# Yukayo/MobGT

Measured on AMD Instinct MI355X. Metric: check-ins/sec (train step), higher is better.
Workload: dtype bf16

## Files before the change

### __graft_entry__.py

```python
import os
import subprocess
import sys

ROOT = os.path.dirname(os.path.abspath(__file__))
if ROOT not in sys.path:
    sys.path.insert(0, ROOT)


def build() -> None:
    from mobgt_amd import _native
    for library in _native.LIBRARIES:
        library.build()
        library.lib()
    from mobgt_amd import _pairbins
    _pairbins.LIBRARY.build()
    _pairbins.LIBRARY.lib()
    from mobgt_amd import _universe
    _universe.LIBRARY.build()
    _universe.LIBRARY.lib()
    from mobgt_amd import _checkins
    _checkins.LIBRARY.build()
    _checkins.LIBRARY.lib()
    from mobgt_amd import _prefixes
    _prefixes.LIBRARY.build()
    _prefixes.LIBRARY.lib()
    from mobgt_amd import _baseline
    _baseline.LIBRARY.build()
    _baseline.LIBRARY.lib()
    from mobgt_amd import _prior
    _prior.LIBRARY.build()
    _prior.LIBRARY.lib()
    from mobgt_amd import _geoprior
    _geoprior.LIBRARY.build()
    _geoprior.LIBRARY.lib()
    from mobgt_amd import _priorfit
    _priorfit.LIBRARY.build()
    _priorfit.LIBRARY.lib()
    from mobgt_amd import _ctxprior
    _ctxprior.LIBRARY.build()
    _ctxprior.LIBRARY.lib()
    subprocess.check_call(["make", "-s", "-C", os.path.join(ROOT, "oracle")])
    import mobgt_amd


def smoke() -> None:
    import numpy as np
    import torch
    from mobgt_amd import ops, synth
    from mobgt_amd.model_fqandtoyo import EncoderLayer
    from oracle import algos_oracle as ao
    from oracle import model_oracle as mo
    assert torch.cuda.is_available(), "smoke() needs cuda:0"
    dev = "cuda:0"
    G, H, T, C = 3, 8, 37, 192
    torch.manual_seed(0)
    layer = EncoderLayer(C, 256, 0.1, 0.1, H).eval()
    sd = {"L." + k: v.detach().clone().requires_grad_(True) for k, v in layer.state_dict().items()}
    rng = np.random.RandomState(0)
    x = torch.from_numpy(rng.standard_normal((G, T, C)).astype(np.float32))
    gy = torch.from_numpy(rng.standard_normal((G, T, C)).astype(np.float32))
    bias = torch.from_numpy((rng.standard_normal((G, H, T, T)) * 0.5).astype(np.float32))
    bias[1, :, :, 30:] = float("-inf")
    xr, br = x.clone().requires_grad_(True), bias.clone().requires_grad_(True)
    ref = mo.encoder_layer_fq(sd, "L", xr, br, H)
    ref.backward(gy)
    layer = layer.to(dev)
    xd, bd = x.to(dev).requires_grad_(True), bias.to(dev).requires_grad_(True)
    out = layer(xd, bd)
    out.backward(gy.to(dev))
    torch.cuda.synchronize()

    def close(name, got, want, tol):
        got, want = got.detach().float().cpu().numpy(), want.detach().numpy()
        scale = float(np.sqrt((want ** 2).mean()))
        err = float(np.abs(got - want).max())
        assert err <= tol * scale, f"{name}: max |err| {err:.3e} vs rms {scale:.3e}"
    close("y", out, ref, 1e-3)
    close("dx", xd.grad, xr.grad, 1e-3)
    close("dbias", bd.grad, br.grad, 1e-3)
    for k, p in layer.named_parameters():
        if k.endswith("linear_k.bias"):
            continue
        if sd["L." + k].grad is not None:
            close("d" + k, p.grad, sd["L." + k].grad, 2e-3)
    layer.act_dtype = torch.bfloat16
    for prm in layer.parameters():
        prm.grad = None
    xb, bb = x.to(dev).requires_grad_(True), bias.to(dev).requires_grad_(True)
    out16 = layer(xb, bb)
    out16.backward(gy.to(dev))
    torch.cuda.synchronize()
    close("y (bf16)", out16, ref, 8e-2)
    close("dx (bf16)", xb.grad, xr.grad, 1e-1)
    close("dbias (bf16)", bb.grad, br.grad, 2e-1)
    trajs = synth.make_batch_of_trajectories(seed=4, G=4, P=50, n_user=8, n_nodes=[17, 3, 9, 30])
    n = np.array([len(t["node_name"]) for t in trajs], dtype=np.int32)
    counts = np.zeros((4, 30, 30), dtype=np.int32)
    for g, t in enumerate(trajs):
        counts[g, :n[g], :n[g]] = t["edge_type"]
    sp = ops.spd_batched(torch.from_numpy(counts).to(dev), torch.from_numpy(n).to(dev), 20)
    for g in range(4):
        k = int(n[g])
        M, path = ao.floyd_warshall(counts[g, :k, :k] != 0)
        assert np.array_equal(sp["spd"][g, :k, :k].cpu().numpy().astype(np.int64), M)
        assert np.array_equal(sp["path"][g, :k, :k].cpu().numpy().astype(np.int64), path)
    print("smoke ok: fused fq EncoderLayer fwd+bwd (f32 and bf16 configurations) and batched SPD match the oracle")


if __name__ == "__main__":
    build()
    if len(sys.argv) > 1 and sys.argv[1] == "smoke":
        smoke()
```

### mobgt_amd/csrc/tokbwd.hip

```cpp
#include "common.h"
#include "mobgt_hip.h"

namespace {

typedef __attribute__((ext_vector_type(4))) float f32x4;

constexpr int TNW = 12, TNT = TNW * 64, TBM = 16;

struct TokBwdParams {
    const float* dout;
    const float* real;
    const float* y4;
    const float* y2; int64_t ld2;
    const float *w4, *w2;
    float *d_nf, *d_add;
    float* dx4; int64_t ldx4;
    float* d_pt;
    float* d_token;
    int G, N;
    float slope4, slope2;
    uint32_t thr_pos, thr_in;
    float keep_pos, keep_in;
    uint64_t seed;
    const uint64_t* seed_dev;
    uint32_t salt_nf, salt_tok, salt_in;
    int n_node_blocks;
};

__device__ __forceinline__ float leaky_grad(float y, float slope) { return y > 0.f ? 1.f : slope; }

#ifdef TB_STAMP
__device__ int* g_tb_dbg = nullptr;
#define TSTAMP_DECL int st_[8] = {}
#define TSTAMP(i) st_[i] = (int)wall_clock64()
#define TSTAMP_DUMP() do { if (g_tb_dbg && threadIdx.x == 0) for (int q_ = 0; q_ < 8; ++q_) g_tb_dbg[blockIdx.x * 8 + q_] = st_[q_]; } while (0)
#else
#define TSTAMP_DECL
#define TSTAMP(i)
#define TSTAMP_DUMP()
#endif

template <int N> constexpr int gemm_ks() { return TNW / ((N + 63) / 64); }
template <int K, int N, int LDA, int LDO>
__device__ __forceinline__ void gemm_kn(const float* __restrict__ A, const float* __restrict__ W, float* __restrict__ out) {
    constexpr int NB = (N + 63) / 64, KS = TNW / NB, NT16 = K / 16, TMAX = (NT16 + KS - 1) / KS;
    static_assert(K % 16 == 0 && N % 32 == 0 && KS >= 1, "shape");
    const int lane = threadIdx.x & 63, wave = threadIdx.x >> 6;
    const int j = lane & 15, q = lane >> 4;
    if (wave >= NB * KS) return;
    const int blk = wave / KS, ks = wave % KS;
    const int t_lo = ks * NT16 / KS, t_hi = (ks + 1) * NT16 / KS;
    const int n0 = 64 * blk;
    const bool col_ok = n0 + 4 * j < N;
    const int cl = col_ok ? n0 + 4 * j : 0;
    f32x4 acc[4];
#pragma unroll
    for (int n = 0; n < 4; ++n) acc[n] = f32x4{0.f, 0.f, 0.f, 0.f};
    f32x4 bw[TMAX][4];
#pragma unroll
    for (int tt = 0; tt < TMAX; ++tt) {
        const int t = min(t_lo + tt, t_hi - 1);
#pragma unroll
        for (int i = 0; i < 4; ++i) bw[tt][i] = *reinterpret_cast<const f32x4*>(W + (int64_t)(16 * t + 4 * q + i) * N + cl);
    }
#pragma unroll
    for (int tt = 0; tt < TMAX; ++tt) {
        if (t_lo + tt < t_hi) {
            const f32x4 a = *reinterpret_cast<const f32x4*>(A + j * LDA + 16 * (t_lo + tt) + 4 * q);
#pragma unroll
            for (int i = 0; i < 4; ++i)
#pragma unroll
                for (int n = 0; n < 4; ++n) acc[n] = __builtin_amdgcn_mfma_f32_16x16x4f32(a[i], bw[tt][i][n], acc[n], 0, 0, 0);
        }
    }
    if (col_ok) {
#pragma unroll
        for (int n = 0; n < 4; ++n)
#pragma unroll
            for (int v = 0; v < 4; ++v) out[(ks * TBM + 4 * q + v) * LDO + n0 + 4 * j + n] = acc[n][v];
    }
}

template <int C, int W2>
__global__ __launch_bounds__(TNT) void token_bwd_chain_kernel(const TokBwdParams p) {
    constexpr int LDA = C + 4, LD2 = W2 + 4;
    __shared__ __attribute__((aligned(16))) float a4[TBM * LDA];
    constexpr int KS4 = gemm_ks<C>(), KS2 = gemm_ks<W2>();
    __shared__ __attribute__((aligned(16))) float t4[(KS4 > KS2 ? KS4 : KS2) * TBM * LDA];
    const int lane = threadIdx.x & 63, wave = threadIdx.x >> 6;
    const int T = p.N + 1;
    const uint64_t seed = (p.thr_pos || p.thr_in) ? p.seed + (p.seed_dev ? *p.seed_dev : 0ull) : 0ull;
    if ((int)blockIdx.x >= p.n_node_blocks) {
        const int g = ((int)blockIdx.x - p.n_node_blocks) * TNW + wave;
        if (g >= p.G) return;
        const int64_t row = (int64_t)g * T;
        const uint32_t h1 = p.thr_pos ? dropout_row_hash(seed, (uint32_t)g ^ p.salt_tok) : 0u;
        const uint32_t h2 = p.thr_in ? dropout_row_hash(seed, (uint32_t)row ^ p.salt_in) : 0u;
        for (int c = lane; c < C; c += 64) {
            float scale = 1.f;
            if (p.thr_pos) scale = dropout_bits16(seed, h1, (uint32_t)c) >= p.thr_pos ? p.keep_pos : 0.f;
            if (p.thr_in) scale *= dropout_bits16(seed, h2, (uint32_t)c) >= p.thr_in ? p.keep_in : 0.f;
            const float d = p.dout[row * C + c] * scale;
            if (d != 0.f) atomicAdd(&p.d_token[c], d);
        }
        return;
    }
    const int64_t R = (int64_t)p.G * p.N;
    const int64_t j0 = (int64_t)blockIdx.x * TBM;
    TSTAMP_DECL;
    TSTAMP(0);
    constexpr int EPT = TBM * C / TNT;
    static_assert(TBM * C % TNT == 0, "flat split");
    float dv[EPT], yv[EPT], rl[EPT];
#pragma unroll
    for (int k = 0; k < EPT; ++k) {
        const int e = threadIdx.x + k * TNT, r = e / C, c = e % C;
        const int64_t jc = min(j0 + r, R - 1);
        const int g = (int)(jc / p.N), n = (int)(jc - (int64_t)g * p.N);
        dv[k] = p.dout[((int64_t)g * T + n + 1) * C + c];
        yv[k] = p.y4[jc * C + c];
        rl[k] = p.real[jc];
    }
#pragma unroll
    for (int k = 0; k < EPT; ++k) {
        const int e = threadIdx.x + k * TNT, r = e / C, c = e % C;
        const int64_t jn = j0 + r;
        const bool on = jn < R;
        const int64_t jc = on ? jn : R - 1;
        const int g = (int)(jc / p.N), n = (int)(jc - (int64_t)g * p.N);
        const int64_t row = (int64_t)g * T + n + 1;
        float scale = 1.f;
        if (p.thr_pos) scale = dropout_bits16(seed, dropout_row_hash(seed, (uint32_t)jc ^ p.salt_nf), (uint32_t)c) >= p.thr_pos ? p.keep_pos : 0.f;
        if (p.thr_in) scale *= dropout_bits16(seed, dropout_row_hash(seed, (uint32_t)row ^ p.salt_in), (uint32_t)c) >= p.thr_in ? p.keep_in : 0.f;
        const float d = on ? dv[k] * scale : 0.f;
        const float dnf = d * rl[k];
        a4[r * LDA + c] = dnf * leaky_grad(yv[k], p.slope4);
        if (on) {
            p.d_add[jn * C + c] = d;
            p.d_nf[jn * C + c] = dnf;
        }
    }
    __syncthreads();
    TSTAMP(1);
    gemm_kn<C, C, LDA, LDA>(a4, p.w4, t4);
    __syncthreads();
    TSTAMP(2);
    for (int e = threadIdx.x; e < TBM * C; e += TNT) {
        const int r = e / C, c = e % C;
        const int64_t jn = j0 + r;
        float v = 0.f;
#pragma unroll
        for (int ks = 0; ks < KS4; ++ks) v += t4[(ks * TBM + r) * LDA + c];
        if (jn < R) p.dx4[jn * p.ldx4 + c] = v;
        if (c < W2) a4[r * LD2 + c] = jn < R ? v * leaky_grad(p.y2[jn * p.ld2 + c], p.slope2) : 0.f;
    }
    __syncthreads();
    TSTAMP(3);
    gemm_kn<W2, W2, LD2, LD2>(a4, p.w2, t4);
    __syncthreads();
    TSTAMP(4);
    for (int e = threadIdx.x; e < TBM * W2; e += TNT) {
        const int r = e / W2, c = e % W2;
        const int64_t jn = j0 + r;
        float v = 0.f;
#pragma unroll
        for (int ks = 0; ks < KS2; ++ks) v += t4[(ks * TBM + r) * LD2 + c];
        if (jn < R) p.d_pt[jn * W2 + c] = v;
    }
    TSTAMP(5);
    TSTAMP_DUMP();
}

}

#ifdef TB_STAMP
extern "C" int mobgt_tokbwd_debug_buffer(int* buf) { return (int)hipMemcpyToSymbol(HIP_SYMBOL(g_tb_dbg), &buf, sizeof(buf)); }
#endif

extern "C" int mobgt_token_bwd_chain(const float* dout, const float* real, const float* y4, const float* y2, int64_t ld_y2,
                                     const float* w4, const float* w2, float* d_nf, float* d_add, float* dx4, int64_t ld_dx4,
                                     float* d_pt, float* d_token, int G, int N, int C, int W2, float slope4, float slope2,
                                     float p_pos, float p_in, uint64_t seed, const uint64_t* seed_dev, uint32_t salt_nf,
                                     uint32_t salt_tok, uint32_t salt_in, void* stream) {
    if (G <= 0 || N <= 0) return MOBGT_EBADDIM;
    if (!(C == 192 && W2 == 160)) return MOBGT_EBADDIM;
    if (!dout || !real || !y4 || !y2 || !w4 || !w2 || !d_nf || !d_add || !dx4 || !d_pt || !d_token || ld_y2 < W2 || ld_dx4 < C)
        return MOBGT_EBADDIM;
    if (((uintptr_t)w4 | (uintptr_t)w2) & 15) return MOBGT_EALIGN;
    TokBwdParams p = {};
    p.dout = dout; p.real = real; p.y4 = y4; p.y2 = y2; p.ld2 = ld_y2; p.w4 = w4; p.w2 = w2; p.d_nf = d_nf; p.d_add = d_add;
    p.dx4 = dx4; p.ldx4 = ld_dx4; p.d_pt = d_pt; p.d_token = d_token; p.G = G; p.N = N; p.slope4 = slope4; p.slope2 = slope2;
    p.thr_pos = p_pos > 0.f ? dropout_threshold(p_pos) : 0u;
    p.thr_in = p_in > 0.f ? dropout_threshold(p_in) : 0u;
    p.keep_pos = p.thr_pos ? 1.f / (1.f - (float)p.thr_pos / 65536.f) : 1.f;
    p.keep_in = p.thr_in ? 1.f / (1.f - (float)p.thr_in / 65536.f) : 1.f;
    p.seed = seed; p.seed_dev = seed_dev; p.salt_nf = salt_nf; p.salt_tok = salt_tok; p.salt_in = salt_in;
    p.n_node_blocks = (int)(((int64_t)G * N + TBM - 1) / TBM);
    const dim3 grid(p.n_node_blocks + (G + TNW - 1) / TNW), block(TNT);
    hipLaunchKernelGGL((token_bwd_chain_kernel<192, 160>), grid, block, 0, (hipStream_t)stream, p);
    return (int)hipGetLastError();
}
```

### mobgt_amd/csrc/wgrad_body.h

```cpp
#pragma once
#include "common.h"
#include "mobgt_hip.h"

namespace mobgt_wgrad {

constexpr int TILE = 32;
constexpr int KSTEP = 32;
constexpr int SHORT_R = 1024;
typedef __attribute__((ext_vector_type(4))) float f32x4;

struct WgradParams {
    const uint16_t* g;  int64_t ldg;
    const uint16_t* x;  int64_t ldx;
    float* dw;  int64_t ldw;
    float* db;
    int R, M, N;
    int tiles_n;
    int k_per_wg;
    int in_f32;
    const float* gmask;
    const float* xmask;
    float mpos, mneg, mzero;
    int db_x;
    const float* out_bias;
    float* gm_out;
};

__device__ __forceinline__ void split_pairs(const uint32_t (&d)[8], bf16x8& even, bf16x8& odd) {
    uint32_t e[4], o[4];
#pragma unroll
    for (int j = 0; j < 4; ++j) {
        e[j] = __builtin_amdgcn_perm(d[2 * j + 1], d[2 * j], 0x05040100u);
        o[j] = __builtin_amdgcn_perm(d[2 * j + 1], d[2 * j], 0x07060302u);
    }
    even = __builtin_bit_cast(bf16x8, e);
    odd = __builtin_bit_cast(bf16x8, o);
}

__device__ __forceinline__ uint32_t pack_pair(const float* p) {
    typedef __attribute__((ext_vector_type(2))) __bf16 bf16x2;
    const float2 v = *reinterpret_cast<const float2*>(p);
    bf16x2 o;
    o[0] = (bf16_t)v.x;
    o[1] = (bf16_t)v.y;
    return __builtin_bit_cast(uint32_t, o);
}

__device__ __forceinline__ uint32_t pack_pair_masked(const float* p, const float* m, float pos, float neg, float zer,
                                                     float* keep = nullptr) {
    typedef __attribute__((ext_vector_type(2))) __bf16 bf16x2;
    float2 v = *reinterpret_cast<const float2*>(p);
    const float2 y = *reinterpret_cast<const float2*>(m);
    v.x *= y.x > 0.f ? pos : (y.x < 0.f ? neg : zer);
    v.y *= y.y > 0.f ? pos : (y.y < 0.f ? neg : zer);
    if (keep) *reinterpret_cast<float2*>(keep) = v;
    bf16x2 o;
    o[0] = (bf16_t)v.x;
    o[1] = (bf16_t)v.y;
    return __builtin_bit_cast(uint32_t, o);
}

struct Slab {
    uint32_t g[8], x[8];
    template <bool F32>
    __device__ __forceinline__ void load_masked(const WgradParams& p, const void* gp, const void* xp, const float* gm, const float* xm,
                                                int r0, int k1, bool m_ok, bool n_ok, float* gkeep = nullptr) {
#pragma unroll
        for (int j = 0; j < 8; ++j) {
            const int r = r0 + j;
            const bool ok = r < k1;
            const float* gq = reinterpret_cast<const float*>(gp) + (int64_t)r * p.ldg;
            const float* xq = reinterpret_cast<const float*>(xp) + (int64_t)r * p.ldx;
            g[j] = !(ok && m_ok) ? 0u : (gm ? pack_pair_masked(gq, gm + (int64_t)r * p.ldg, p.mpos, p.mneg, p.mzero,
                                                               gkeep ? gkeep + (int64_t)r * p.ldg : nullptr) : pack_pair(gq));
            x[j] = !(ok && n_ok) ? 0u : (xm ? pack_pair_masked(xq, xm + (int64_t)r * p.ldx, p.mpos, p.mneg, p.mzero) : pack_pair(xq));
        }
    }
    template <bool GF32, bool XF32>
    __device__ __forceinline__ void load(const void* gp, const void* xp, int64_t ldg, int64_t ldx, int r0, int k1,
                                         bool m_ok, bool n_ok) {
#pragma unroll
        for (int j = 0; j < 8; ++j) {
            const int r = r0 + j;
            const bool ok = r < k1;
            if (GF32) g[j] = ok && m_ok ? pack_pair(reinterpret_cast<const float*>(gp) + (int64_t)r * ldg) : 0u;
            else g[j] = ok && m_ok ? *reinterpret_cast<const uint32_t*>(reinterpret_cast<const uint16_t*>(gp) + (int64_t)r * ldg) : 0u;
            if (XF32) x[j] = ok && n_ok ? pack_pair(reinterpret_cast<const float*>(xp) + (int64_t)r * ldx) : 0u;
            else x[j] = ok && n_ok ? *reinterpret_cast<const uint32_t*>(reinterpret_cast<const uint16_t*>(xp) + (int64_t)r * ldx) : 0u;
        }
    }
};

template <int NWAVE> constexpr int wgrad_lds_floats() { return (NWAVE / 2) * TILE * TILE + NWAVE * TILE; }

template <bool F32, int NWAVE, bool XF32 = F32>
__device__ __forceinline__ void wgrad_body(const WgradParams& p, const int tile, const int split, const int nsplit,
                                           float* __restrict__ lds) {
    float (*part)[TILE * TILE] = reinterpret_cast<float (*)[TILE * TILE]>(lds);
    float (*colpart)[TILE] = reinterpret_cast<float (*)[TILE]>(lds + (NWAVE / 2) * TILE * TILE);
    const int lane = threadIdx.x & 63, wave = threadIdx.x >> 6;
    const int i = lane & 15, kq = lane >> 4;
    const int m0 = (tile / p.tiles_n) * TILE, n0 = (tile % p.tiles_n) * TILE;
    const int k0 = split * p.k_per_wg;
    const int k1 = min(p.R, k0 + p.k_per_wg);
    const bool want_db = p.db != nullptr && (p.db_x ? m0 == 0 : n0 == 0);
    const bool m_ok = m0 + 2 * i < p.M, n_ok = n0 + 2 * i < p.N;
    const void* gp = F32 ? (const void*)(reinterpret_cast<const float*>(p.g) + m0 + 2 * i) : (const void*)(p.g + m0 + 2 * i);
    const void* xp = XF32 ? (const void*)(reinterpret_cast<const float*>(p.x) + n0 + 2 * i) : (const void*)(p.x + n0 + 2 * i);

    f32x4 acc[2][2];
#pragma unroll
    for (int a = 0; a < 2; ++a)
#pragma unroll
        for (int b = 0; b < 2; ++b) acc[a][b] = f32x4{0.f, 0.f, 0.f, 0.f};
    float se = 0.f, so = 0.f;

    const bool masked = F32 && (p.gmask || p.xmask);
    const float* gm = masked && p.gmask ? p.gmask + m0 + 2 * i : nullptr;
    const float* xm = masked && p.xmask ? p.xmask + n0 + 2 * i : nullptr;
    float* gkeep = (masked && gm && p.gm_out && n0 == 0) ? p.gm_out + m0 + 2 * i : nullptr;
    auto fetch = [&](Slab& s_, int r0_) {
        if (masked) s_.template load_masked<F32>(p, gp, xp, gm, xm, r0_, k1, m_ok, n_ok, gkeep);
        else s_.template load<F32, XF32>(gp, xp, p.ldg, p.ldx, r0_, k1, m_ok, n_ok);
    };
    int kb = k0 + wave * KSTEP;
    Slab cur, nxt;
    if (kb < k1) fetch(cur, kb + 8 * kq);
    for (; kb < k1; kb += NWAVE * KSTEP) {
        const int kn = kb + NWAVE * KSTEP;
        if (kn < k1) fetch(nxt, kn + 8 * kq);
        bf16x8 ge, go, xe, xo;
        split_pairs(cur.g, ge, go);
        split_pairs(cur.x, xe, xo);
        acc[0][0] = __builtin_amdgcn_mfma_f32_16x16x32_bf16(ge, xe, acc[0][0], 0, 0, 0);
        acc[0][1] = __builtin_amdgcn_mfma_f32_16x16x32_bf16(ge, xo, acc[0][1], 0, 0, 0);
        acc[1][0] = __builtin_amdgcn_mfma_f32_16x16x32_bf16(go, xe, acc[1][0], 0, 0, 0);
        acc[1][1] = __builtin_amdgcn_mfma_f32_16x16x32_bf16(go, xo, acc[1][1], 0, 0, 0);
        if (want_db) {
#pragma unroll
            for (int j = 0; j < 8; ++j) {
                const uint32_t d = p.db_x ? cur.x[j] : cur.g[j];
                se += bf16_lo(d); so += bf16_hi(d);
            }
        }
        if (kn < k1) cur = nxt;
    }

    if (wave >= NWAVE / 2) {
#pragma unroll
        for (int a = 0; a < 2; ++a)
#pragma unroll
            for (int b = 0; b < 2; ++b)
#pragma unroll
                for (int v = 0; v < 4; ++v) part[wave - NWAVE / 2][(2 * (4 * kq + v) + a) * TILE + 2 * i + b] = acc[a][b][v];
    }
    __syncthreads();
    if (wave < NWAVE / 2) {
#pragma unroll
        for (int a = 0; a < 2; ++a)
#pragma unroll
            for (int b = 0; b < 2; ++b)
#pragma unroll
                for (int v = 0; v < 4; ++v) part[wave][(2 * (4 * kq + v) + a) * TILE + 2 * i + b] += acc[a][b][v];
    }
    if (want_db) {
        se += __shfl_xor(se, 16, 64); se += __shfl_xor(se, 32, 64);
        so += __shfl_xor(so, 16, 64); so += __shfl_xor(so, 32, 64);
        if (kq == 0) { colpart[wave][2 * i] = se; colpart[wave][2 * i + 1] = so; }
    }
    __syncthreads();
    for (int e = threadIdx.x; e < TILE * TILE; e += NWAVE * 64) {
        const int r = e >> 5, c = e & 31;
        float s = 0.f;
#pragma unroll
        for (int w = 0; w < NWAVE / 2; ++w) s += part[w][e];
        if (m0 + r < p.M && n0 + c < p.N) {
            float* dst = p.dw + (int64_t)(m0 + r) * p.ldw + n0 + c;
            if (p.out_bias && split == 0) s += p.out_bias[n0 + c];
            atomicAdd(dst, s);
        }
    }
    {
        const int e = threadIdx.x;
        const int c0 = p.db_x ? n0 : m0;
        if (want_db && e < TILE && c0 + e < (p.db_x ? p.N : p.M)) {
            float t = 0.f;
#pragma unroll
            for (int w = 0; w < NWAVE; ++w) t += colpart[w][e];
            atomicAdd(p.db + c0 + e, t);
        }
    }
}

inline int fill_problem(WgradParams& p, const void* g, int64_t ldg, const void* x, int64_t ldx, float* dw, int64_t ldw, float* db,
                 int64_t R, int M, int N, int target_wgs, int* tiles_out, int* splits_out, int in_f32, int nwave) {
    if (R <= 0 || M <= 0 || N <= 0 || (M & 1) || (N & 1) || (ldg & 1) || (ldx & 1) || R > 0x7fffffff) return MOBGT_EBADDIM;
    if (((uintptr_t)g & (in_f32 == 1 ? 7 : 3)) || ((uintptr_t)x & (in_f32 ? 7 : 3))) return MOBGT_EALIGN;
    p.in_f32 = in_f32;
    p.gmask = p.xmask = nullptr; p.mpos = p.mneg = p.mzero = 1.f; p.db_x = 0; p.out_bias = nullptr; p.gm_out = nullptr;
    p.g = reinterpret_cast<const uint16_t*>(g); p.ldg = ldg;
    p.x = reinterpret_cast<const uint16_t*>(x); p.ldx = ldx;
    p.dw = dw; p.ldw = ldw; p.db = db;
    p.R = (int)R; p.M = M; p.N = N;
    const int tiles_m = (M + TILE - 1) / TILE;
    p.tiles_n = (N + TILE - 1) / TILE;
    const int tiles = tiles_m * p.tiles_n;
    const int slab = nwave * KSTEP;
    int splits = target_wgs / tiles;
    const int max_splits = (int)((R + slab - 1) / slab);
    if (splits > max_splits) splits = max_splits;
    if (splits < 1) splits = 1;
    p.k_per_wg = (int)(((R + splits - 1) / splits + slab - 1) / slab) * slab;
    *splits_out = (int)((R + p.k_per_wg - 1) / p.k_per_wg);
    *tiles_out = tiles;
    return 0;
}


}
```

### mobgt_amd/forms.py

```python
import contextlib
import os
from collections import namedtuple

Form = namedtuple("Form", "name env default doc")

_ROWS = (
    Form("safe_forms", "MOBGT_SAFE_FORMS", False, "no launch waits for peer workgroups: one workgroup per row block, the head as "
         "three launches, the GCN layer by layer (what TrainStep.guarded_step switches to before it re-runs a faulted step)"),
    Form("chain", "MOBGT_NO_CHAIN", True, "out-proj -> LN -> FFN -> LN -> the next layer's QKV in one launch (off: separate launches)"),
    Form("chain_big", "MOBGT_NO_CHAIN_BIG", True, "past 4 096 rows: the 64-row forward chain (off: the library's GEMMs)"),
    Form("chain_bwd", None, True, "the same chain backwards, d(out) -> d(attention out)"),
    Form("ln_gemm", None, True, "dropout+residual+LN as the prologue of the GEMM that consumes it (off: the two-launch form)"),
    Form("ln_gemm_bwd", "MOBGT_LN_GEMM_BWD", False, "the LayerNorm-prologue GEMMs in the backward as well"),
    Form("own_gemm", None, True, "the layer's GEMMs on csrc/gemm.hip (off: through torch)"),
    Form("tail", None, True, "a layer's input-gradient GEMM rides in its grouped weight-gradient launch"),
    Form("defer_tail", "MOBGT_NO_DEFER_TAIL", True, "a layer leaves dx and its weight gradients to the chain_bwd launch of the layer "
         "below (off: it finishes its own backward)"),
    Form("wgrad_big", None, True, "past 4 096 rows: the layer's weight gradients as one launch"),
    Form("skinny_all", "MOBGT_SKINNY_ALL", False, "all three classifier products on csrc/skinny.hip (off: dW / db only)"),
    Form("token_fwd_chain", "MOBGT_NO_TOKEN_FWD_CHAIN", True, "the encoder input's forward as one launch (off: four)"),
    Form("token_bwd_chain", "MOBGT_NO_TOKEN_BWD_CHAIN", True, "the encoder input's backward as one launch, csrc/tokbwd.hip (off: three)"),
    Form("pack_passenger", "MOBGT_NO_PACK_PASSENGER", True, "the layers' weight pack, in the next front launch"),
    Form("front_passengers", "MOBGT_NO_FRONT_PASSENGERS", True, "hop table forward and node-feature indices, in the category GCN's forward"),
    Form("bias_bwd_passenger", "MOBGT_NO_BIAS_BWD_PASSENGER", True, "short batches: the bias tables' backward, in the category GCN's backward"),
    Form("bias_bwd_beside", None, True, "long batches: the bias tables' backward on a side stream (off: where autograd reaches it)"),
    Form("l0_ride", "MOBGT_NO_L0_RIDE", True, "the distance GCN's first product, in the bias assembly's launch"),
    Form("psum_defer", "MOBGT_NO_PSUM_DEFER", True, "split-K partial sums, in the step's one reduction launch into the gradient sinks"),
    Form("small_gcn", "MOBGT_NO_SMALL_GCN", True, "the three-layer category GCN as one launch each way (off: layer by layer)"),
    Form("conv_act", "MOBGT_NO_CONV_ACT", True, "bias + LeakyReLU + dropout in the small GEMM's epilogue (off: launch per product)"),
    Form("dist_gcn_fused", "MOBGT_NO_DIST_GCN_FUSED", True, "the distance GCN on the masked-GEMM launches"),
    Form("sp_gather", None, True, "sparse adjacency, transposed product as a gather (off: the atomic scatter)"),
    Form("stock_front", "MOBGT_NO_STOCK_FRONT", True, "hop table, weight pack and encoder input as one front launch"),
    Form("stock_tail", "MOBGT_NO_STOCK_TAIL", True, "the encoder input's and the wide hop table's backward share one grid at the flush"),
    Form("stock_ln_qkv", "MOBGT_NO_STOCK_LN_QKV", True, "the first layer's norm inside its QKV GEMM"),
    Form("attn_one_pass", "MOBGT_ATTN_TWO_PASS", True, "T > 64, bf16: one-pass backward (off: the two deterministic passes)"),
    Form("ddp_overlap", "MOBGT_DDP_OVERLAP", False, "the backward split into graphs, finished gradient slices all-reduced beside the next"),
    Form("ddp_host_exchange", "MOBGT_DDP_HOST_EXCHANGE", False, "all-reduce issued by the host between backward and optimizer graph"),
    Form("force_comm", "MOBGT_FORCE_COMM", False, "a process group of one rank takes the data-parallel path (tests)"),
)
_BY_NAME = {row.name: row for row in _ROWS}
_OVERRIDES = {}


def _env_set(var):
    v = os.environ.get(var, "")
    if v in ("", "0"):
        return False
    if v == "1":
        return True
    raise ValueError(f"{var}={v!r}: expected unset, '', '0' or '1'")


def on(name):
    row = _BY_NAME[name]
    if name in _OVERRIDES:
        return _OVERRIDES[name]
    if row.env is not None and _env_set(row.env):
        return not row.default
    return row.default


def set(name, value):
    _BY_NAME[name]
    if value is None:
        _OVERRIDES.pop(name, None)
    else:
        _OVERRIDES[name] = bool(value)


@contextlib.contextmanager
def using(**names):
    saved = dict(_OVERRIDES)
    try:
        for name, value in names.items():
            set(name, value)
        yield
    finally:
        _OVERRIDES.clear()
        _OVERRIDES.update(saved)


def table():
    return _ROWS
```

### mobgt_amd/fused_layer.py

```python
import ctypes
from collections import namedtuple

import torch

from . import _lib, forms, ops
from .layer_plan import (BACKWARD_FORMS, BIG_R, FORWARD_FORMS, TAIL_MAX_R, Given, Operands, Tail, plan_backward, plan_forward)
from .ops import _p, _stream, _DT
from .step_state import STEP

_M32 = 0xFFFFFFFF
_TAKES_OUT_DTYPE = {}


def _takes_out_dtype(gemm, *operands):
    if gemm not in _TAKES_OUT_DTYPE:
        try:
            gemm(*operands, out_dtype=torch.float32)
            _TAKES_OUT_DTYPE[gemm] = True
        except Exception:
            _TAKES_OUT_DTYPE[gemm] = False
    return _TAKES_OUT_DTYPE[gemm]


def _split_factor(R, tiles):
    want = max(1, (512 + tiles - 1) // tiles)
    best = 1
    for s in range(1, 257):
        if R % s == 0 and R // s >= 32:
            best = s
            if s >= want:
                break
    return best


def _wgrad_hip(dtype, M, N, R):
    return dtype == torch.bfloat16 and M % 2 == 0 and N % 2 == 0 and (M * N <= _WGRAD_HIP_MN or R <= BIG_R)


_WGRAD_HIP_MN = 131072


def _wgrad_arrays(items):
    n = len(items)
    vp, i64, ci = ctypes.c_void_p, ctypes.c_int64, ctypes.c_int
    return (n, (vp * n)(*[t[0].data_ptr() for t in items]), (i64 * n)(*[t[0].stride(0) for t in items]),
            (vp * n)(*[t[1].data_ptr() for t in items]), (i64 * n)(*[t[1].stride(0) for t in items]),
            (vp * n)(*[t[2].data_ptr() for t in items]), (i64 * n)(*[t[2].shape[1] for t in items]),
            (vp * n)(*[(t[3].data_ptr() if t[3] is not None else None) for t in items]),
            (ci * n)(*[t[0].shape[1] for t in items]), (ci * n)(*[t[1].shape[1] for t in items]))


class _WgradBatch:

    def __init__(self):
        self.items = []

    def add(self, g, x, db=None, sink=None):
        if not _wgrad_hip(g.dtype, g.shape[1], x.shape[1], g.shape[0]):
            return _wgrad(g, x, db, sink=sink)
        dw = sink[:] if sink is not None else ops.zeros_f32((g.shape[1], x.shape[1]), g.device)
        self.items.append((g, x, dw, db))
        return dw

    def flush(self, tail=None):
        it = self.items
        if not it:
            return False
        R = it[0][0].shape[0]
        arr = _wgrad_arrays(it)
        group = arr[:8] + (R,) + arr[8:] + (_DT[it[0][0].dtype],)
        self.items = []
        if tail is not None and R <= TAIL_MAX_R:
            a, w, c = tail
            if (a.dtype == torch.bfloat16 and w.dtype == torch.bfloat16 and c.dtype == torch.float32 and a.shape[1] % 32 == 0
                    and w.shape[1] % 8 == 0 and a.is_contiguous() and w.is_contiguous() and c.is_contiguous()):
                _lib.call("mobgt_layer_backward_tail", *group, _p(a), a.stride(0), _p(w), w.stride(0), _p(c), c.stride(0),
                          a.shape[0], w.shape[1], a.shape[1], _stream())
                return True
        _lib.call("mobgt_linear_wgrad_group", *group, _stream())
        return False


def _join_step_wgrads(wb):
    for g, x, dw, db in wb.items:
        STEP.wgrad_items.append((g, x, None, None, (1.0, 1.0, 1.0), dw[:], db[:] if db is not None else None, False))
    wb.items = []


def _wgrad(g, x, db=None, sink=None):
    if _wgrad_hip(g.dtype, g.shape[1], x.shape[1], g.shape[0]):
        return ops.linear_wgrad(g, x, db=db)[0]
    if db is not None:
        _lib.call("mobgt_colsum", _p(g), _p(db), g.shape[0], g.shape[1], _DT[g.dtype], _stream())
    return _mm_tn_f32(g, x, sink=sink)


def _mm_tn_f32(g, x, sink=None):
    R, M = g.shape
    N = x.shape[1]
    tiles = ((M + 63) // 64) * ((N + 63) // 64)
    s = _split_factor(R, tiles) if (tiles <= 12 or (R >= 4096 and tiles < 256)) else 1
    if s > 1:
        ga, xa = g.view(s, R // s, M).transpose(1, 2), x.view(s, R // s, N)
        if g.dtype != torch.float32 and _takes_out_dtype(torch.bmm, ga[:1], xa[:1]):
            part = torch.bmm(ga, xa, out_dtype=torch.float32)
            parked = ops.defer_partial_sum(part, sink) if sink is not None else None
            return parked if parked is not None else part.sum(0)
        part = torch.bmm(ga, xa)
        return part.float().sum(0) if part.dtype != torch.float32 else part.sum(0)
    if g.dtype == torch.float32:
        return g.t() @ x
    if _takes_out_dtype(torch.mm, g.t(), x):
        return torch.mm(g.t(), x, out_dtype=torch.float32)
    return (g.t() @ x).float()




def _addmm_f32(c, a, b, inplace=False):
    if _takes_out_dtype(torch.addmm, c, a, b):
        if inplace:
            return torch.ops.aten.addmm.dtype_out(c, a, b, torch.float32, out=c)
        return torch.addmm(c, a, b, out_dtype=torch.float32)
    return c + (a @ b).float()


def _k1_fwd(x, y, x1, w, b, z, z32, mean, rstd, R, C, p, seed, seed_dev, salt, act):
    _lib.call("mobgt_dropout_add_ln_fwd", _p(x), _p(y), _p(x1), _p(w), _p(b), _p(z), _p(z32), _p(mean), _p(rstd), R, C,
              p, seed, _p(seed_dev), salt, act, _stream())






def _pending_key(t):
    return (ops.graph_task_id(), t.device.index, t.data_ptr())


def _park_tail(dx1, **work):
    STEP.layer_tails[_pending_key(dx1)] = dict(dx1=dx1[:], **work)
    if STEP.tail_check_task != ops.graph_task_id():
        STEP.tail_check_task = ops.graph_task_id()
        torch.autograd.Variable._execution_engine.queue_callback(_pending_check)


def _take_tail(dout):
    if STEP.layer_tails or STEP.tail_check_task is not None:
        STEP.drop_stale_tails(ops.graph_task_id())
    return STEP.layer_tails.pop(_pending_key(dout), None) if STEP.layer_tails else None


def _complete_pending(pend):
    if pend["kind"] == "preln":
        raise RuntimeError("mobgt fused layer (pre-LN): the parked input gradient of a chained layer found no host "
                           "(was the layer's input used by something else as well?); set MOBGT_NO_DEFER_TAIL=1")
    if pend["kind"] == "big":
        _addmm_f32(pend["dx1"], pend["dqkv"], pend["wqkv"], inplace=True)
        return
    wb = _WgradBatch()
    wb.items = pend["items"]
    if not wb.flush(tail=(pend["dqkv"], pend["wqkv"], pend["dx1"])):
        ops.layer_gemm(pend["dqkv"], pend["wqkv"], None, True, ops.GEMM_ADD, aux_in=pend["dx1"])


def _pending_check():
    tid = ops.graph_task_id()
    STEP.tail_check_task = None
    mine = [k for k in STEP.layer_tails if k[0] == tid or tid == -1]
    if mine:
        left = [STEP.layer_tails.pop(k) for k in mine]
        try:
            for pend in left:
                _complete_pending(pend)
        finally:
            STEP.layer_tails.clear()
        raise RuntimeError("mobgt fused layer: a deferred input gradient was not consumed by the layer below "
                           "(was the layer's input used by something else as well?); set MOBGT_NO_DEFER_TAIL=1")


_CHAIN_WS = {}
_CHAIN_NCL = {}


def chain_workspace(dev, C=192, R=None):
    if forms.on("safe_forms"):
        return None
    idx = dev.index if dev.index is not None else torch.cuda.current_device()
    R = 16 if R is None else int(R)
    ncl = _CHAIN_NCL.get((idx, R))
    if ncl is None:
        ncl = _CHAIN_NCL[idx, R] = _lib.lib().mobgt_chain_cluster_size(R)
    key = (idx, int(C), ncl)
    ws = _CHAIN_WS.get(key)
    if ws is None:
        if torch.cuda.is_current_stream_capturing():
            raise RuntimeError("the chain kernels' workspace must be allocated before graph capture: run one eager step first")
        ws = _CHAIN_WS[key] = torch.zeros(int(_lib.lib().mobgt_chain_ws_bytes()), dtype=torch.uint8, device=dev)
    return ws


def _ln_gemm_fwd(x, y, x1, w, b, z, mean, rstd, R, C, p, seed, seed_dev, salt, weight, bias, epilogue):
    N = weight.shape[0]
    out = torch.empty(R, N, dtype=torch.bfloat16, device=x.device)
    aux = torch.empty(R, N, dtype=torch.bfloat16, device=x.device) if epilogue == ops.GEMM_GELU else None
    _lib.call("mobgt_ln_gemm_fwd", _p(x), _p(y), _p(x1), _p(w), _p(b), _p(z), _p(mean), _p(rstd), R, C, p, seed,
              _p(seed_dev), salt, _p(weight), weight.stride(0), _p(bias), _p(out), N, epilogue,
              _p(aux), N, _stream())
    return (out, aux) if aux is not None else out


def _ln_gemm_bwd(dz, dz32, dres, x1, mean, rstd, w, dx1, dy, dgamma, dbeta, dbias, R, C, p, seed, seed_dev, salt, weight_kn,
                 epilogue, aux_in):
    N = weight_kn.shape[1]
    out = torch.empty(R, N, dtype=torch.bfloat16, device=x1.device)
    _lib.call("mobgt_ln_gemm_bwd", _p(dz), _p(dz32), _p(dres), _p(x1), _p(mean), _p(rstd), _p(w), _p(dx1), _p(dy),
              _p(dgamma), _p(dbeta), _p(dbias), R, C, p, seed, _p(seed_dev), salt, _p(weight_kn),
              weight_kn.stride(0), _p(out), N, epilogue, _p(aux_in), N, _stream())
    return out


def _k1_bwd(dz, dz32, dres, x1, mean, rstd, w, dx1, dy, dgamma, dbeta, dbias, R, C, p, seed, seed_dev, salt, act):
    _lib.call("mobgt_dropout_add_ln_bwd", _p(dz), _p(dz32), _p(dres), _p(x1), _p(mean), _p(rstd), _p(w), _p(dx1), _p(dy),
              _p(dgamma), _p(dbeta), _p(dbias), R, C, p, seed, _p(seed_dev), salt, act,
              _stream())


def _chain_fwd(a, x, packed, sh, n1, norm, nq, outs, stats, plan, cfg):
    p_wo, p_w1, p_w2 = packed
    _lib.call("mobgt_layer_chain_fwd", _p(a), _p(x), _p(p_wo), _p(sh.bo), _p(n1[0]), _p(n1[1]), _p(p_w1), _p(sh.b1), _p(p_w2),
              _p(sh.b2), _p(norm[0]), _p(norm[1]), _p(nq[0]), _p(nq[1]), *[_p(t) for t in outs], _p(stats[2]), _p(stats[3]),
              _p(stats[4]), _p(stats[5]), plan.R, plan.C, plan.F, cfg.p, cfg.seed, _p(cfg.seed_dev), (cfg.salt + 1) & _M32,
              (cfg.salt + 2) & _M32, _p(chain_workspace(x.device, plan.C, plan.R)), _stream())


def _chain_bwd(entry, plan, cfg, sv, dout, norm, sm, pend):
    R, C, F = plan.R, plan.C, plan.F
    bf = dict(dtype=cfg.act_dtype, device=dout.device)
    df, dy, da = torch.empty(R, C, **bf), torch.empty(R, C, **bf), torch.empty(R, C, **bf)
    du = torch.empty(R, F, **bf)
    dx1 = torch.empty(R, C, dtype=torch.float32, device=dout.device)
    w2t, w1t, wot = cfg.packed_t[:3]
    st = sv.stats
    ptrs = [_p(t) for t in (dout, sv.x2, sv.x1, sv.u, st[2], st[3], st[4], st[5], sv.n1w, norm[0], w2t, w1t, wot, df, du, dy, da, dx1,
                            norm[1], norm[2], sm.db2, sm.dn1w, sm.dn1b, sm.dbo)]
    dims = (R, C, F, cfg.p, cfg.seed, _p(cfg.seed_dev), (cfg.salt + 1) & _M32, (cfg.salt + 2) & _M32)
    tail = (_p(pend["dqkv"]), _p(pend["wqt"])) if pend is not None else (None, None)
    if entry == "chain64":
        _lib.call("mobgt_layer_chain_bwd_big", *ptrs, _p(None if plan.db1_in_wgrad else sm.db1), *dims, *tail, _stream())
    else:
        extra = _wgrad_arrays(pend["items"]) if pend is not None and pend["items"] else (0,) + (None,) * 9
        _lib.call("mobgt_layer_chain_bwd_preln" if entry == "preln" else "mobgt_layer_chain_bwd", *ptrs, *dims, *tail, *extra,
                  _p(chain_workspace(dout.device, C, R)), _stream())
    return df, du, dy, da, dx1


class LayerConfig:

    def __init__(self, variant, num_heads, scale, p_drop, p_att, seed, seed_dev, salt, pack, act_dtype):
        self.variant, self.H, self.scale = variant, num_heads, scale
        self.p, self.p_att = float(p_drop), float(p_att)
        self.seed, self.seed_dev, self.salt = int(seed), seed_dev, int(salt) & 0xFFFFFFFF
        self.pack = pack
        self.act_dtype = act_dtype
        self.from_layer = False
        self.next_qkv = None
        self.packed = None
        self.packed_t = None
        self.out_act = self.out_qkv = None
        self.next_norm = None
        self.out_preln = False


_Params = namedtuple("_Params", "wq bq wk bk wv bv wo bo n1w n1b nxw nxb w1 b1 w2 b2 nnw nnb", defaults=(None, None))
_Shadows = namedtuple("_Shadows", "wqkv bqkv wo bo w1 b1 w2 b2")
_Saved = namedtuple("_Saved", "x xa qkv a lse x1 z u h x2 stats s_wqkv s_wo s_w1 s_w2 n1w nxw nnw")
_Sinks = namedtuple("_Sinks", "qkv wo w1 w2 small nx nn")
_SmallGrads = namedtuple("_SmallGrads", "dbqkv dbo db1 db2 dn1w dn1b dnxw dnxb")


def _aligned(*ts):
    return all(t is None or (t.is_contiguous() and t.data_ptr() % 16 == 0) for t in ts)


def _forms_on(names):
    return {name: forms.on(name) for name in names}


def _given(cfg, xa_pre, qkv_pre, p, R, C):
    A, nq = cfg.act_dtype, cfg.next_qkv
    return Given(xa_pre=xa_pre is not None and xa_pre.dtype == A and xa_pre.numel() == R * C,
                 qkv_pre=qkv_pre is not None and qkv_pre.dtype == A and qkv_pre.numel() == 3 * R * C,
                 nx=p.nxw is not None, packed=cfg.packed is not None, n_packed_t=len(cfg.packed_t) if cfg.packed_t is not None else 0,
                 next_qkv=nq is not None and nq[0].dtype == A and tuple(nq[0].shape) == (3 * C, C) and _aligned(nq[0]),
                 next_norm=p.nnw is not None and p.nnw.is_contiguous() and p.nnb is not None, from_layer=bool(cfg.from_layer))


def _operands(cfg, x, xa, sh, p):
    if cfg.act_dtype != torch.bfloat16 or xa is None:
        return Operands(False, False, False, False, False, False, False)
    R, C, F = x.shape[0] * x.shape[1], x.shape[2], sh.w1.shape[0]
    stock = cfg.variant == "stock"
    own_norm = () if stock else (p.nxw, p.nxb)
    return Operands(gemm_qkv=ops.layer_gemm_ok(xa, sh.wqkv), gemm_w1=ops.layer_gemm_ok(xa, sh.w1),
                    chain=cfg.packed is not None and _aligned(x, sh.bo, sh.b1, sh.b2, p.n1w, p.n1b, *own_norm, *cfg.packed),
                    ln_qkv=stock and _aligned(x, sh.wqkv, sh.bqkv, p.nxw, p.nxb), ln_ffn=_aligned(x, sh.w1, sh.b1, sh.w2, sh.wo),
                    packed_t=cfg.packed_t is not None and _aligned(*cfg.packed_t), wgrad_hip=_wgrad_hip(cfg.act_dtype, F, C, R))


def _input_act(cfg, x, xa_pre, given, R, C):
    A = cfg.act_dtype
    if cfg.variant == "stock":
        if given.nx:
            return torch.empty(R, C, dtype=A, device=x.device)
        return xa_pre.view(R, C) if given.xa_pre else None
    if A == torch.float32:
        return x.view(R, C)
    return xa_pre.view(R, C) if given.xa_pre else x.view(R, C).to(A)


def _find_sinks(plan, p, C):
    sq, sk, sv = ops.grad_sink(p.wq), ops.grad_sink(p.wk), ops.grad_sink(p.wv)
    s_qkv = None
    if sq is not None and sk is not None and sv is not None and sq.is_contiguous() \
            and sk.data_ptr() == sq.data_ptr() + 4 * sq.numel() and sv.data_ptr() == sk.data_ptr() + 4 * sk.numel():
        s_qkv = torch.as_strided(sq, (3 * C, C), (C, 1))
    weights = (s_qkv, ops.grad_sink(p.wo), ops.grad_sink(p.w1), ops.grad_sink(p.w2))
    preln = plan.body == "preln_chain"
    chain = [ops.grad_sink(t) for t in (p.bq, p.bk, p.bv, p.bo, p.b1, p.b2, p.n1w, p.n1b) + (() if preln else (p.nxw, p.nxb))]
    small = None
    if all(t is not None and t.is_contiguous() for t in chain) and \
            all(chain[j + 1].data_ptr() == chain[j].data_ptr() + 4 * chain[j].numel() for j in range(len(chain) - 1)):
        small = torch.as_strided(chain[0], (sum(t.numel() for t in chain),), (1,))
    nx = (ops.grad_sink(p.nxw), ops.grad_sink(p.nxb)) if preln and p.nxw is not None else (None, None)
    nn = (ops.grad_sink(p.nnw), ops.grad_sink(p.nnb)) if preln and plan.chain_next else (None, None)
    return _Sinks(*weights, small, nx, nn)


def _small_grads(sinks, C, F, n, dev):
    sizes = [3 * C, C, F, C, C, C, C, C][:n]
    block = sinks.small if sinks.small is not None else ops.zeros_f32((sum(sizes),), dev)
    views, o = [], 0
    for size in sizes:
        views.append(block[o:o + size])
        o += size
    return views


def _norm_grads(pair, have, C, dev):
    if not have:
        return None, None
    return tuple(s[:] if s is not None else ops.zeros_f32((C,), dev) for s in pair)


def _forward_chain(plan, cfg, x, a, stats, sh, p):
    R, C, F = plan.R, plan.C, plan.F
    stock, nxt = plan.body == "preln_chain", plan.chain_next
    f32, bf = dict(dtype=torch.float32, device=x.device), dict(dtype=cfg.act_dtype, device=x.device)
    x1, x2 = torch.empty(R, C, **f32), torch.empty(R, C, **f32)
    z, u, h = torch.empty(R, C, **bf), torch.empty(R, F, **bf), torch.empty(R, F, **bf)
    out = None if stock else torch.empty(R, C, **f32)
    out_a = torch.empty(R, C, **bf) if nxt or not stock else None
    qkv_next = torch.empty(R, 3 * C, **bf) if nxt else None
    norm = (p.nxw, p.nxb) if not stock else (p.nnw, p.nnb) if nxt else (None, None)
    _chain_fwd(a, x, cfg.packed, sh, (p.n1w, p.n1b), norm, cfg.next_qkv if nxt else (None, None),
               (x1, z, u, h, x2, out, out_a, qkv_next), stats, plan, cfg)
    if not stock:
        cfg.out_act, cfg.out_qkv = out_a, qkv_next
    elif nxt:
        cfg.out_act, cfg.out_qkv, cfg.out_preln = out_a, qkv_next, True
    return (x2 if stock else out), x1, z, u, h, x2


def _forward_launches(plan, cfg, x, a, stats, sh, p):
    R, C, A, own = plan.R, plan.C, cfg.act_dtype, plan.own
    act = _DT[A]
    seed, sd, salt = cfg.seed, cfg.seed_dev, cfg.salt
    f32 = dict(dtype=torch.float32, device=x.device)
    y = ops.layer_gemm(a.view(R, C), sh.wo, sh.bo) if own else torch.addmm(sh.bo, a.view(R, C), sh.wo.t())
    x1 = torch.empty(R, C, **f32)
    z = torch.empty(R, C, dtype=A, device=x.device)
    if plan.ln_gemm:
        u, h = _ln_gemm_fwd(x, y, x1, p.n1w, p.n1b, z, stats[2], stats[3], R, C, cfg.p, seed, sd, salt + 1, sh.w1, sh.b1,
                            ops.GEMM_GELU)
        f = ops.layer_gemm(h, sh.w2, sh.b2)
    elif own:
        _k1_fwd(x, y, x1, p.n1w, p.n1b, z, None, stats[2], stats[3], R, C, cfg.p, seed, sd, salt + 1, act)
        u, h = ops.layer_gemm(z, sh.w1, sh.b1, epilogue=ops.GEMM_GELU)
        f = ops.layer_gemm(h, sh.w2, sh.b2)
    else:
        _k1_fwd(x, y, x1, p.n1w, p.n1b, z, None, stats[2], stats[3], R, C, cfg.p, seed, sd, salt + 1, act)
        u = torch.addmm(sh.b1, z, sh.w1.t())
        h = torch.empty_like(u)
        _lib.call("mobgt_gelu_fwd", _p(u), _p(h), u.numel(), act, _stream())
        f = torch.addmm(sh.b2, h, sh.w2.t())
    x2 = torch.empty(R, C, **f32)
    if plan.variant == "stock":
        _k1_fwd(x1, f, x2, None, None, None, None, None, None, R, C, cfg.p, seed, sd, salt + 2, act)
        out = x2
    else:
        out = torch.empty(R, C, **f32)
        out_a = torch.empty(R, C, dtype=A, device=x.device) if A != torch.float32 else None
        _k1_fwd(x1, f, x2, p.nxw, p.nxb, out_a, out, stats[4], stats[5], R, C, cfg.p, seed, sd, salt + 2, act)
        cfg.out_act = out_a
    return out, x1, z, u, h, x2


def _backward_launches(plan, bp, cfg, wb, dout, sv, sm, sinks):
    R, C, F, A, own = plan.R, plan.C, plan.F, cfg.act_dtype, plan.own
    act, dev, st = _DT[A], dout.device, sv.stats
    seed, sd, salt = cfg.seed, cfg.seed_dev, cfg.salt
    db1_in_wgrad = plan.db1_in_wgrad
    df = torch.empty(R, C, dtype=A, device=dev)
    du = None
    if plan.variant == "stock":
        dx2 = dout
        _k1_bwd(None, None, dout, sv.x2, None, None, None, None, df, None, None, sm.db2, R, C, cfg.p, seed, sd, salt + 2, act)
    else:
        dx2 = torch.empty(R, C, dtype=torch.float32, device=dev)
        if bp.ln_gemm_bwd and db1_in_wgrad:
            du = _ln_gemm_bwd(None, dout, None, sv.x2, st[4], st[5], sv.nxw, dx2, df, sm.dnxw, sm.dnxb, sm.db2, R, C, cfg.p,
                              seed, sd, salt + 2, sv.s_w2, ops.GEMM_GELU_BWD, sv.u)
        else:
            _k1_bwd(None, dout, None, sv.x2, st[4], st[5], sv.nxw, dx2, df, sm.dnxw, sm.dnxb, sm.db2, R, C, cfg.p, seed, sd,
                    salt + 2, act)
    dw2 = wb.add(df, sv.h, sink=sinks.w2)
    if du is not None:
        pass
    elif own and db1_in_wgrad:
        du = ops.layer_gemm(df, sv.s_w2, None, True, ops.GEMM_GELU_BWD, aux_in=sv.u)
    else:
        dh = df @ sv.s_w2
        du = torch.empty_like(sv.u)
        _lib.call("mobgt_gelu_bwd_colsum", _p(dh), _p(sv.u), _p(du), _p(None if db1_in_wgrad else sm.db1), R, F, act,
                  _stream())
    dz = ops.layer_gemm(du, sv.s_w1, None, True) if own else du @ sv.s_w1
    dw1 = wb.add(du, sv.z, db=sm.db1 if db1_in_wgrad else None, sink=sinks.w1)
    dx1 = torch.empty(R, C, dtype=torch.float32, device=dev)
    dy = torch.empty(R, C, dtype=A, device=dev)
    if bp.ln_gemm_bwd:
        da = _ln_gemm_bwd(dz, None, dx2, sv.x1, st[2], st[3], sv.n1w, dx1, dy, sm.dn1w, sm.dn1b, sm.dbo, R, C, cfg.p, seed, sd,
                          salt + 1, sv.s_wo, ops.GEMM_BIAS, None)
    else:
        _k1_bwd(dz, None, dx2, sv.x1, st[2], st[3], sv.n1w, dx1, dy, sm.dn1w, sm.dn1b, sm.dbo, R, C, cfg.p, seed, sd, salt + 1, act)
        da = ops.layer_gemm(dy, sv.s_wo, None, True) if own else dy @ sv.s_wo
    dwo = wb.add(dy, sv.a.view(R, C), sink=sinks.wo)
    return da, dx1, dw2, dw1, dwo


def _finish_dx(plan, bp, cfg, sv, sm, dqkv2, dx1, items):
    R, C = plan.R, plan.C
    if bp.dx == "below":
        kind = "preln" if bp.entry == "preln" else "layer" if bp.wgrads == "below" else "big"
        _park_tail(dx1, dqkv=dqkv2, wqkv=sv.s_wqkv, wqt=cfg.packed_t[3], items=items, R=R, kind=kind)
    elif bp.dx == "norm":
        dz0 = ops.layer_gemm(dqkv2, sv.s_wqkv, None, True) if plan.own else dqkv2 @ sv.s_wqkv
        dx = torch.empty(R, C, dtype=torch.float32, device=dx1.device)
        _k1_bwd(dz0, None, dx1, sv.x.view(R, C), sv.stats[0], sv.stats[1], sv.nxw, dx, None, sm.dnxw, sm.dnxb, None, R, C, 0.0,
                cfg.seed, cfg.seed_dev, cfg.salt, _DT[cfg.act_dtype])
        return dx
    elif bp.dx == "addmm_out":
        torch.addmm(dx1, dqkv2, sv.s_wqkv, out=dx1)
    elif bp.dx == "own_gemm":
        ops.layer_gemm(dqkv2, sv.s_wqkv, None, True, ops.GEMM_ADD, aux_in=dx1)
    elif bp.dx == "addmm_f32":
        _addmm_f32(dx1, dqkv2, sv.s_wqkv, inplace=True)
    return dx1


class _FusedLayerFn(torch.autograd.Function):

    @staticmethod
    def forward(ctx, x, token, cfg, shadows, xa_pre, qkv_pre, *params):
        p, sh = _Params(*params), _Shadows(*shadows)
        G, T, C = x.shape
        R, F, A = G * T, sh.w1.shape[0], cfg.act_dtype
        x = x.contiguous()
        given = _given(cfg, xa_pre, qkv_pre, p, R, C)
        xa = _input_act(cfg, x, xa_pre, given, R, C)
        plan = plan_forward(cfg.variant, A == torch.bfloat16, R, C, F, any(ctx.needs_input_grad), given, _operands(cfg, x, xa, sh, p),
                            _forms_on(FORWARD_FORMS))
        stats = torch.empty(6, R, dtype=torch.float32, device=x.device)
        seed, sd, salt = cfg.seed, cfg.seed_dev, cfg.salt
        if plan.norm_launch:
            _k1_fwd(x, None, None, p.nxw, p.nxb, xa, None, stats[0], stats[1], R, C, 0.0, seed, sd, salt, _DT[A])
        if plan.qkv == "pre":
            qkv = qkv_pre.view(G, T, 3 * C)
        elif plan.qkv == "ln_gemm":
            qkv = _ln_gemm_fwd(x, None, None, p.nxw, p.nxb, xa, stats[0], stats[1], R, C, 0.0, seed, sd, salt, sh.wqkv, sh.bqkv,
                               ops.GEMM_BIAS).view(G, T, 3 * C)
        elif plan.qkv == "own":
            qkv = ops.layer_gemm(xa, sh.wqkv, sh.bqkv).view(G, T, 3 * C)
        else:
            qkv = torch.addmm(sh.bqkv, xa, sh.wqkv.t()).view(G, T, 3 * C)
        q, k, v = qkv[..., :C], qkv[..., C:2 * C], qkv[..., 2 * C:]
        a, lse = ops._attn_fwd(q, k, v, cfg.pack, cfg.scale, cfg.p_att, seed ^ (salt * 0x9E3779B1), sd)
        cfg.out_qkv = None
        body = _forward_launches if plan.body == "launches" else _forward_chain
        out, x1, z, u, h, x2 = body(plan, cfg, x, a, stats, sh, p)
        ctx.plan, ctx.cfg, ctx.shapes = plan, cfg, (G, T, C)
        ctx.chain_bwd, ctx.stock_chain = plan.chain_bwd, plan.body == "preln_chain"
        ctx.sinks = _find_sinks(plan, p, C)
        ctx.save_for_backward(x, xa, qkv, a, lse, x1, z, u, h, x2, stats, sh.wqkv, sh.wo, sh.w1, sh.w2, p.n1w, p.nxw,
                              p.nnw if plan.chain_next else None)
        return out.view(G, T, C)

    @staticmethod
    def backward(ctx, dout):
        cfg, plan, sinks = ctx.cfg, ctx.plan, ctx.sinks
        G, T, C = ctx.shapes
        R, F, A, dev = plan.R, plan.F, cfg.act_dtype, dout.device
        sv = _Saved(*ctx.saved_tensors)
        busy = getattr(ctx, "_mobgt_pending", None)
        if busy is not None:
            busy.done()
        preln = plan.body == "preln_chain"
        dout = dout.contiguous().view(R, C).float()
        if preln:
            sm = _SmallGrads(*_small_grads(sinks, C, F, 6, dev), *_norm_grads(sinks.nx, sv.nxw is not None, C, dev))
            dnn = _norm_grads(sinks.nn, sv.nnw is not None, C, dev)
        else:
            sm, dnn = _SmallGrads(*_small_grads(sinks, C, F, 8, dev)), (None, None)
        pend = _take_tail(dout)
        bp = plan_backward(plan, _forms_on(BACKWARD_FORMS), STEP.wgrad_on,
                           Tail(pend["kind"], pend["R"], bool(pend["items"])) if pend is not None else None,
                           sum(_wgrad_hip(A, m, n, R) for m, n in ((C, F), (F, C), (C, C), (3 * C, C))),
                           all(k is not None for k in sinks[:4]), sinks.small is not None, R * max(3 * C, F) * 2 < (1 << 31))
        if pend is not None and not bp.host:
            _complete_pending(pend)
            pend = None
        wb = _WgradBatch()
        if bp.entry is None:
            da, dx1, dw2, dw1, dwo = _backward_launches(plan, bp, cfg, wb, dout, sv, sm, sinks)
        else:
            norm = (sv.nnw,) + dnn if preln else (sv.nxw, sm.dnxw, sm.dnxb)
            df, du, dy, da, dx1 = _chain_bwd(bp.entry, plan, cfg, sv, dout, norm, sm, pend)
            if bp.db1_colsum:
                _lib.call("mobgt_colsum", _p(du), _p(sm.db1), R, F, _DT[A], _stream())
            three = [(df, sv.h, None, sinks.w2), (du, sv.z, sm.db1 if plan.db1_in_wgrad else None, sinks.w1),
                     (dy, sv.a.view(R, C), None, sinks.wo)]
            if bp.wgrads != "big":
                dw2, dw1, dwo = [wb.add(g_, x_, db=db_, sink=k_) for g_, x_, db_, k_ in three]
        dqkv = torch.empty(G, T, 3 * C, dtype=A, device=dev)
        q, k, v = sv.qkv[..., :C], sv.qkv[..., C:2 * C], sv.qkv[..., 2 * C:]
        ops._attn_bwd(q, k, v, sv.a, sv.lse, da.view(G, T, C), dqkv[..., :C], dqkv[..., C:2 * C], dqkv[..., 2 * C:], cfg.pack,
                      cfg.scale, cfg.p_att, cfg.seed ^ (cfg.salt * 0x9E3779B1), cfg.seed_dev)
        dqkv2 = dqkv.view(R, 3 * C)
        items = []
        if bp.wgrads == "big":
            four = three + [(dqkv2, sv.xa.view(R, C), sm.dbqkv, sinks.qkv)]
            assert ops.layer_wgrad_big_ok(four)
            dw2, dw1, dwo, dwqkv = ops.layer_wgrad_big(four, R)
        else:
            dwqkv = wb.add(dqkv2, sv.xa, db=sm.dbqkv, sink=sinks.qkv)
        if bp.wgrads == "below":
            items = [(g_, x_, dw_[:], db_[:] if db_ is not None else None) for g_, x_, dw_, db_ in wb.items]
            wb.items = []
        elif bp.wgrads == "step":
            _join_step_wgrads(wb)
        else:
            rode = wb.flush(tail=(dqkv2, sv.s_wqkv, dx1) if bp.dx == "tail" else None)
            assert rode == (bp.dx == "tail")
        dx = _finish_dx(plan, bp, cfg, sv, sm, dqkv2, dx1, items)
        return (dx.view(G, T, C), None, None, None, None, None, dwqkv[:C], sm.dbqkv[:C], dwqkv[C:2 * C], sm.dbqkv[C:2 * C],
                dwqkv[2 * C:], sm.dbqkv[2 * C:], dwo, sm.dbo, sm.dn1w, sm.dn1b, sm.dnxw, sm.dnxb, dw1, sm.db1, dw2, sm.db2) \
            + (dnn if plan.variant == "stock" else ())


def fused_encoder_layer(x, pack, cfg, shadows, params, xa_pre=None, qkv_pre=None):
    cfg.out_act = cfg.out_qkv = None
    cfg.out_preln = False
    out = _FusedLayerFn.apply(x, pack.token, cfg, shadows, xa_pre, qkv_pre, *params)
    if cfg.out_preln:
        out._mobgt_preln = True
    if cfg.out_act is not None:
        out._mobgt_act = cfg.out_act
    if cfg.out_qkv is not None:
        out._mobgt_qkv = cfg.out_qkv
        out._mobgt_from_layer = True
    return out
```

### mobgt_amd/layer_plan.py

```python
from collections import namedtuple

from . import _lib

CHAIN_SHAPES = ((128, 1024), (192, 1024), (256, 1024))
BIG_R = _lib.CONSTANTS["MOBGT_CHAIN_BIG_ROWS"]
TAIL_MAX_R = 1024
DEFER_MAX_R = 4096

FORWARD_FORMS = ("own_gemm", "ln_gemm", "stock_ln_qkv", "chain", "chain_big", "chain_bwd")
BACKWARD_FORMS = ("ln_gemm_bwd", "wgrad_big", "defer_tail", "tail")

Given = namedtuple("Given", "xa_pre qkv_pre nx packed n_packed_t next_qkv next_norm from_layer")
Operands = namedtuple("Operands", "gemm_qkv gemm_w1 chain ln_qkv ln_ffn packed_t wgrad_hip")

LayerPlan = namedtuple("LayerPlan", "variant bf16 R C F qkv norm_launch own body ln_gemm chain_next chain_bwd below_hosts chained_in "
                                    "db1_in_wgrad")
Tail = namedtuple("Tail", "kind R items")
BackwardPlan = namedtuple("BackwardPlan", "entry host host_items db1_colsum ln_gemm_bwd wgrads dx")


def plan_forward(variant, bf16, R, C, F, need_bwd, given, ok, on):
    stock = variant == "stock"
    chained_in = stock and not given.nx
    if chained_in and not (given.xa_pre and given.qkv_pre):
        raise RuntimeError("mobgt fused layer (pre-LN): a chained input without its normed copy / qkv")
    own = bool(on["own_gemm"] and ok.gemm_qkv and ok.gemm_w1 and C % 32 == 0 and F % 32 == 0)
    ln_fits = on["ln_gemm"] and C % 32 == 0 and C <= 256
    if given.qkv_pre and (not stock or chained_in):
        qkv = "pre"
    elif (stock and bf16 and not given.qkv_pre and on["own_gemm"] and ok.gemm_qkv and ln_fits and ok.ln_qkv and on["stock_ln_qkv"]):
        qkv = "ln_gemm"
    else:
        qkv = "own" if own else "torch"
    chain_fits = bool(bf16 and given.packed and on["chain"] and (C, F) in CHAIN_SHAPES and ok.chain)
    if stock:
        bwd_ok = on["chain_bwd"] and given.n_packed_t > 3 and ok.packed_t
        body = "preln_chain" if (own and chain_fits and (bwd_ok or not need_bwd) and ok.wgrad_hip) else "launches"
        chain_bwd = False
    else:
        body = "chain" if ((own or (R > BIG_R and on["chain_big"])) and chain_fits) else "launches"
        chain_bwd = bool(body == "chain" and on["chain_bwd"] and given.n_packed_t >= 3 and ok.packed_t and (R <= BIG_R or on["chain_big"]))
    if chained_in and body != "preln_chain":
        raise RuntimeError("mobgt fused layer (pre-LN): the layer below chained into this one, which cannot run its chain kernels")
    return LayerPlan(
        variant=variant, bf16=bool(bf16), R=R, C=C, F=F, qkv=qkv, norm_launch=stock and not chained_in and qkv != "ln_gemm", own=own,
        body=body, ln_gemm=bool(body == "launches" and own and bf16 and ln_fits and ok.ln_ffn),
        chain_next=bool(given.next_qkv and (body == "chain" or (body == "preln_chain" and given.next_norm))), chain_bwd=chain_bwd,
        below_hosts=bool(given.from_layer and given.qkv_pre and chain_bwd and given.n_packed_t > 3),
        chained_in=chained_in, db1_in_wgrad=bool(ok.wgrad_hip))


def plan_backward(plan, on, wgrad_on, tail, n_hip, sinks, small_sink, big_fits):
    R, stock = plan.R, plan.variant == "stock"
    step = bool(stock and wgrad_on and R <= DEFER_MAX_R and sinks)
    if plan.body == "preln_chain":
        host = bool(tail is not None and tail.kind == "preln" and plan.chain_next and tail.R == R)
        return BackwardPlan("preln", host, False, False, False, "step" if step and n_hip else "own", "below" if plan.chained_in else "norm")
    chain = plan.chain_bwd and (plan.db1_in_wgrad or R > BIG_R)
    host = bool(chain and tail is not None and tail.kind != "preln" and tail.R == R)
    host_items = bool(host and tail.items)
    entry = None if not chain else "chain64" if (R > BIG_R and not host_items) else "chain16"
    big = bool(chain and R > BIG_R and on["wgrad_big"] and plan.bf16 and not plan.db1_in_wgrad and big_fits)
    n_batch = 0 if big else n_hip
    may_defer = on["defer_tail"] and plan.below_hosts and not stock and on["tail"]
    defer = bool(may_defer and plan.own and n_batch == 4 and R <= DEFER_MAX_R and small_sink and sinks)
    big_defer = bool(not defer and may_defer and R > BIG_R)
    wgrads = "big" if big else "below" if defer else "step" if step and n_batch else "own"
    if defer or big_defer:
        dx = "below"
    elif wgrads == "own" and plan.own and not stock and on["tail"] and n_batch and R <= TAIL_MAX_R:
        dx = "tail"
    else:
        dx = "norm" if stock else "addmm_out" if not plan.bf16 else "own_gemm" if plan.own else "addmm_f32"
    return BackwardPlan(entry, host, host_items, entry == "chain16" and not plan.db1_in_wgrad,
                        bool(entry is None and on["ln_gemm_bwd"] and (plan.ln_gemm if plan.body == "launches" else plan.own)), wgrads, dx)
```

### mobgt_amd/model.py

```python
import math
import weakref

import torch
import torch.nn as nn
import torch.nn.functional as F

from . import forms, layer_plan, ops
from .step_state import STEP


def init_bert_params(module, n_layers):
    if isinstance(module, nn.Linear):
        module.weight.data.normal_(mean=0.0, std=0.02 / math.sqrt(n_layers))
        if module.bias is not None:
            module.bias.data.zero_()
    if isinstance(module, nn.Embedding):
        module.weight.data.normal_(mean=0.0, std=0.02)


def no_grad_row0(weight):
    return torch.cat([weight[:1].detach(), weight[1:]], dim=0)


def hop_table_from(edge_weight, edge_dis_weight, H, D, fp16_roundtrip=False):
    if edge_weight.is_cuda and edge_weight.dtype == torch.float32 and edge_dis_weight.dtype == torch.float32:
        from . import ops
        return ops.hop_table(edge_weight, edge_dis_weight, H, D, fp16_roundtrip)
    W = edge_dis_weight.reshape(-1, H, H)[:D]
    enc = no_grad_row0(edge_weight)
    if fp16_roundtrip:
        return torch.matmul(enc.half().float().unsqueeze(0), W.half().float()).half().float()
    return torch.matmul(enc.unsqueeze(0), W)


class FeedForwardNetwork(nn.Module):

    def __init__(self, hidden_size, ffn_size, dropout_rate):
        super().__init__()
        self.layer1 = nn.Linear(hidden_size, ffn_size)
        self.gelu = nn.GELU()
        self.layer2 = nn.Linear(ffn_size, hidden_size)

    def forward(self, x):
        return self.layer2(self.gelu(self.layer1(x)))


_layer_counter = [0]


class MultiHeadAttention(nn.Module):

    def __init__(self, hidden_size, attention_dropout_rate, num_heads):
        super().__init__()
        self.num_heads = num_heads
        self.att_size = att_size = hidden_size // num_heads
        self.scale = att_size ** -0.5
        self.linear_q = nn.Linear(hidden_size, num_heads * att_size)
        self.linear_k = nn.Linear(hidden_size, num_heads * att_size)
        self.linear_v = nn.Linear(hidden_size, num_heads * att_size)
        self.att_dropout = nn.Dropout(attention_dropout_rate)
        self.output_layer = nn.Linear(num_heads * att_size, hidden_size)
        _layer_counter[0] += 1
        self.set_layer_index(_layer_counter[0])
        self._pack_cache = None
        self.seed_dev = None

    def set_layer_index(self, index):
        self._layer_index = int(index)
        self._seed_salt = (self._layer_index * 0x9E3779B97F4A7C15) & 0x7FFFFFFFFFFFFFFF

    def fuse_qkv_storage(self):
        ws = [self.linear_q.weight, self.linear_k.weight, self.linear_v.weight]
        bs = [self.linear_q.bias, self.linear_k.bias, self.linear_v.bias]
        C = ws[0].shape[0]
        fw = getattr(self, "_wqkv", None)
        ok = fw is not None and fw.device == ws[0].device and all(
            w.data_ptr() == fw.data_ptr() + i * C * w.shape[1] * 4 for i, w in enumerate(ws)) and all(
            b.data_ptr() == self._bqkv.data_ptr() + i * C * 4 for i, b in enumerate(bs))
        if not ok:
            with torch.no_grad():
                fw = torch.cat([w.detach().float() for w in ws], dim=0).contiguous()
                fb = torch.cat([b.detach().float() for b in bs], dim=0).contiguous()
                for i, (w, b) in enumerate(zip(ws, bs)):
                    w.data = fw[i * C:(i + 1) * C]
                    b.data = fb[i * C:(i + 1) * C]
            self._wqkv, self._bqkv = fw, fb
        return self._wqkv, self._bqkv

    def _packed(self, attn_bias, G, T, ref):
        if isinstance(attn_bias, ops.PackedBias):
            return attn_bias
        if attn_bias is None:
            attn_bias = torch.zeros(1, 1, T, T, device=ref.device)
        cache = MultiHeadAttention._shared_cache
        src = cache.get("src")
        grad_mode = attn_bias.requires_grad and torch.is_grad_enabled()
        if (src is None or src() is not attn_bias or cache.get("key") != (attn_bias._version, G, T, self.num_heads, grad_mode)
                or cache["pack"].spent):
            cache["pack"] = ops.pack_bias(attn_bias, G, self.num_heads, T)
            cache["src"] = weakref.ref(attn_bias)
            cache["key"] = (attn_bias._version, G, T, self.num_heads, grad_mode)
        return cache["pack"]

    _shared_cache = {}

    def _masked_forward(self, q, k, v, attn_bias, mask):
        G, Tq = q.shape[0], q.shape[1]
        H, d = self.num_heads, self.att_size
        qh = self.linear_q(q).float().view(G, -1, H, d).transpose(1, 2) * self.scale
        kh = self.linear_k(k).float().view(G, -1, H, d).transpose(1, 2).transpose(2, 3)
        vh = self.linear_v(v).float().view(G, -1, H, d).transpose(1, 2)
        s = torch.matmul(qh, kh)
        if attn_bias is not None:
            if isinstance(attn_bias, ops.PackedBias):
                attn_bias = attn_bias.dense()
            s = s + attn_bias.float()
        s = s.masked_fill(mask.unsqueeze(1), 0)
        p = self.att_dropout(torch.softmax(s, dim=3))
        x = torch.matmul(p, vh).transpose(1, 2).contiguous().view(G, Tq, H * d)
        return self.output_layer(x.to(self.output_layer.weight.dtype))

    def forward(self, q, k, v, attn_bias=None, mask=None):
        if mask is not None:
            x = self._masked_forward(q, k, v, attn_bias, mask)
            assert x.size() == q.size()
            return x
        orig_q_size = q.size()
        G, T = q.shape[0], q.shape[1]
        pack = self._packed(attn_bias, G, T, q)
        p_drop = self.att_dropout.p if self.training else 0.0
        seed = self._seed_salt
        if p_drop > 0 and self.seed_dev is None:
            seed = (seed + int(torch.randint(0, 2 ** 31 - 1, (1,)).item())) & 0x7FFFFFFFFFFFFFFF
        if q is k and k is v:
            w = torch.cat([self.linear_q.weight, self.linear_k.weight, self.linear_v.weight], dim=0)
            b = torch.cat([self.linear_q.bias, self.linear_k.bias, self.linear_v.bias], dim=0)
            x = ops.attention_qkv(F.linear(q, w, b), pack, self.scale, p_drop, seed, self.seed_dev)
        else:
            x = ops.attention(self.linear_q(q), self.linear_k(k), self.linear_v(v), pack, self.scale, p_drop, seed,
                              self.seed_dev)
        x = self.output_layer(x)
        assert x.size() == orig_q_size
        return x


def fused_layer_forward(layer, variant, x, attn_bias, n1, nx, next_layer=None):
    from .fused_layer import LayerConfig, fused_encoder_layer
    mha = layer.self_attention
    G, T, C = x.shape
    pack = mha._packed(attn_bias, G, T, x)
    wqkv, bqkv = mha.fuse_qkv_storage()
    act = getattr(layer, "act_dtype", torch.float32)
    amp = x.is_cuda and torch.is_autocast_enabled("cuda")
    if amp:
        act = torch.bfloat16
    masters = (wqkv, bqkv, mha.output_layer.weight, mha.output_layer.bias, layer.ffn.layer1.weight, layer.ffn.layer1.bias,
               layer.ffn.layer2.weight, layer.ffn.layer2.bias)
    if act == torch.float32:
        shadows = tuple(m.detach() for m in masters)
    else:
        sh = getattr(layer, "_shadows", None)
        if sh is None or sh[0].device != x.device or sh[0].dtype != act:
            sh = tuple(torch.empty_like(m, dtype=act) for m in masters)
            layer._shadows = sh
            layer._shadow_fresh = False
            layer._shadow_ver = None
        if not getattr(layer, "_shadow_fresh", False) or act != getattr(layer, "act_dtype", torch.float32):
            ver = _weights_version(layer)
            if ((getattr(layer, "_shadow_ver", None) != ver or not _may_skip_shadow_copy(layer))
                    and not getattr(layer, "_shadow_external", False)):
                torch._foreach_copy_(list(sh), [m.detach() for m in masters])
                layer._shadow_ver = ver
                layer._packed_ver = None
        layer._shadow_fresh = False
        shadows = sh
    training = layer.training
    p = layer.self_attention_dropout.p if training else 0.0
    p_att = mha.att_dropout.p if training else 0.0
    seed = mha._seed_salt
    if (p > 0 or p_att > 0) and mha.seed_dev is None:
        seed = (seed + int(torch.randint(0, 2 ** 31 - 1, (1,)).item())) & 0x7FFFFFFFFFFFFFFF
    cfg = LayerConfig(variant, mha.num_heads, mha.scale, p, p_att, seed, mha.seed_dev, mha._layer_index * 8, pack, act)
    cfg.from_layer = bool(getattr(x, "_mobgt_from_layer", False)) and not getattr(layer, "_mobgt_cut", False)
    nxt = next_layer
    stock = variant == "stock"
    if (nxt is not None and act != torch.float32 and not amp and getattr(nxt, "fused", False)
            and getattr(nxt, "act_dtype", None) == act and getattr(nxt, "_packed_fresh", False)
            and nxt._packed[0].device == x.device):
        if not stock:
            cfg.next_qkv = (nxt._packed[0], nxt._shadows[1])
        else:
            bwd_ok = (not torch.is_grad_enabled()) or (getattr(nxt, "_packed_t_fresh", False) and getattr(layer, "_packed_t_fresh", False))
            if forms.on("defer_tail") and not getattr(nxt, "_mobgt_cut", False) and getattr(layer, "_packed_fresh", False) and bwd_ok:
                cfg.next_qkv = (nxt._packed[0], nxt._shadows[1])
                cfg.next_norm = (nxt.self_attention_norm.weight, nxt.self_attention_norm.bias)
    if getattr(layer, "_packed_fresh", False) is True and act != torch.float32 and not amp:
        cfg.packed = layer._packed[1:]
        if getattr(layer, "_packed_t_fresh", False):
            cfg.packed_t = layer._packed_t
    layer._packed_fresh = layer._packed_t_fresh = False
    chained_in = (stock and not amp and getattr(x, "_mobgt_preln", False) and getattr(x, "_mobgt_qkv", None) is not None
                  and getattr(x, "_mobgt_act", None) is not None and not getattr(layer, "_mobgt_cut", False))
    params = (mha.linear_q.weight, mha.linear_q.bias, mha.linear_k.weight, mha.linear_k.bias, mha.linear_v.weight,
              mha.linear_v.bias, mha.output_layer.weight, mha.output_layer.bias, n1.weight, n1.bias,
              None if chained_in else nx.weight, None if chained_in else nx.bias,
              layer.ffn.layer1.weight, layer.ffn.layer1.bias, layer.ffn.layer2.weight, layer.ffn.layer2.bias)
    if stock:
        nn_ = getattr(cfg, "next_norm", None)
        params = params + ((nn_[0], nn_[1]) if nn_ is not None else (None, None))
    if amp:
        with torch.autocast("cuda", enabled=False):
            out = fused_encoder_layer(x.float(), pack, cfg, shadows, params, xa_pre=getattr(x, "_mobgt_act", None))
    else:
        out = fused_encoder_layer(x.float(), pack, cfg, shadows, params, xa_pre=getattr(x, "_mobgt_act", None),
                                  qkv_pre=getattr(x, "_mobgt_qkv", None))
    if act != torch.float32 and out.requires_grad:
        note_pending_backward(layer, out)
    return out


def take_pending_pack():
    jobs, STEP.weight_pack = STEP.weight_pack, []
    return jobs


def flush_pending_pack():
    jobs = take_pending_pack()
    if jobs:
        _launch_pack(jobs)


def _launch_pack(jobs):
    import ctypes
    from . import _lib
    from .ops import _stream
    for o in range(0, len(jobs), 96):
        part = jobs[o:o + 96]
        n = len(part)
        vp, ci = ctypes.c_void_p, ctypes.c_int
        _lib.call("mobgt_pack_mfma_b", n, (vp * n)(*[j[0].data_ptr() for j in part]), (vp * n)(*[j[1].data_ptr() for j in part]),
                  (ci * n)(*[j[2] for j in part]), (ci * n)(*[j[3] for j in part]),
                  (ci * n)(*[j[4] for j in part]), _stream())


class _PendingBackward:
    __slots__ = ("pending", "__weakref__")

    def __init__(self, pending):
        self.pending = pending
        pending.add(id(self))
        weakref.finalize(self, pending.discard, id(self))

    def done(self):
        self.pending.discard(id(self))


def note_pending_backward(layer, out):
    fn = getattr(out, "grad_fn", None)
    if fn is None:
        return
    pend = layer.__dict__.setdefault("_pending_bwd", set())
    try:
        fn._mobgt_pending = _PendingBackward(pend)
    except Exception:
        pass


def _may_skip_shadow_copy(layer):
    return bool(getattr(layer, "_pending_bwd", None)) or bool(getattr(layer, "_weights_frozen", False))


def _weights_version(layer):
    mha = layer.self_attention
    ps = (mha.linear_q.weight, mha.linear_k.weight, mha.linear_v.weight, mha.linear_q.bias, mha.linear_k.bias, mha.linear_v.bias,
          mha.output_layer.weight, mha.output_layer.bias, layer.ffn.layer1.weight, layer.ffn.layer1.bias, layer.ffn.layer2.weight,
          layer.ffn.layer2.bias)
    return tuple((p._version, p.data_ptr()) for p in ps)


def refresh_shadows(layers, defer_pack=False, rows=None):
    dst, src = [], []
    for layer in layers:
        if getattr(layer, "act_dtype", torch.float32) == torch.float32 or not layer.fused:
            continue
        if getattr(layer, "_shadow_external", False):
            layer._shadow_fresh = True
            continue
        mha = layer.self_attention
        wqkv, bqkv = mha.fuse_qkv_storage()
        masters = (wqkv, bqkv, mha.output_layer.weight, mha.output_layer.bias, layer.ffn.layer1.weight, layer.ffn.layer1.bias,
                   layer.ffn.layer2.weight, layer.ffn.layer2.bias)
        sh = getattr(layer, "_shadows", None)
        ver = _weights_version(layer)
        if sh is None or sh[0].device != wqkv.device or sh[0].dtype != layer.act_dtype:
            sh = tuple(torch.empty_like(m, dtype=layer.act_dtype) for m in masters)
            layer._shadows = sh
            layer._shadow_ver = None
        if getattr(layer, "_shadow_ver", None) != ver or not _may_skip_shadow_copy(layer):
            dst += list(sh)
            src += [m.detach() for m in masters]
            layer._shadow_ver = ver
            layer._packed_ver = None
        layer._shadow_fresh = True
    if dst:
        torch._foreach_copy_(dst, src)
    pack_layer_weights(layers, defer=defer_pack, rows=rows)


def pack_layer_weights(layers, defer=False, rows=None):
    flush_pending_pack()
    if not forms.on("chain"):
        return
    want_t = torch.is_grad_enabled() and forms.on("chain_bwd")
    big = rows is not None and rows > layer_plan.BIG_R
    qkv0_only = big and not forms.on("chain_big")
    if big and not forms.on("chain_big"):
        want_t = False
    jobs = []
    for li, layer in enumerate(layers):
        layer._packed_fresh = layer._packed_t_fresh = False
        sh = getattr(layer, "_shadows", None)
        if (sh is None or not getattr(layer, "fused", False) or not getattr(layer, "_shadow_fresh", False)
                or not (hasattr(layer, "ffn_norm2") or hasattr(layer, "self_attention_norm")) or sh[0].dtype != torch.bfloat16
                or not sh[0].is_cuda):
            continue
        C, F = sh[2].shape[0], sh[4].shape[0]
        if (C, F) not in layer_plan.CHAIN_SHAPES or not all(sh[i].is_contiguous() for i in (0, 2, 4, 6)):
            continue
        pk = getattr(layer, "_packed", None)
        if pk is None or pk[0].device != sh[0].device:
            pk = tuple(torch.empty_like(sh[i]) for i in (0, 2, 4, 6))
            layer._packed = pk
            layer._packed_ver = None
        want_t_l = bool(want_t and any(p.requires_grad for p in layer.parameters()))
        pt = getattr(layer, "_packed_t", None)
        if want_t_l and (pt is None or pt[0].device != sh[0].device):
            pt = tuple(torch.empty_like(sh[i]) for i in (6, 4, 2, 0))
            layer._packed_t = pt
            layer._packed_ver = None
        ver = None if getattr(layer, "_shadow_external", False) else getattr(layer, "_shadow_ver", None)
        have = getattr(layer, "_packed_ver", None)
        what = "qkv" if qkv0_only else "all"
        reuse = ver is not None and have is not None and have[0] == ver and have[1] == what and (have[2] or not want_t_l)
        if qkv0_only:
            if li == 0:
                if not reuse:
                    jobs.append((sh[0], pk[0], sh[0].shape[0], sh[0].shape[1], 0))
                    layer._packed_ver = (ver, what, False)
                layer._packed_fresh = "qkv"
            continue
        if not reuse:
            for d, i in zip(pk, (0, 2, 4, 6)):
                jobs.append((sh[i], d, sh[i].shape[0], sh[i].shape[1], 0))
            if want_t_l:
                for d, i in zip(pt, (6, 4, 2, 0)):
                    jobs.append((sh[i], d, sh[i].shape[1], sh[i].shape[0], 1))
            layer._packed_ver = (ver, what, want_t_l)
        layer._packed_fresh = True
        layer._packed_t_fresh = want_t_l
    small = sum(j[2] * j[3] for j in jobs) <= (8 << 20)
    if defer and jobs and len(jobs) <= 96 and small and forms.on("pack_passenger"):
        STEP.weight_pack.extend(jobs)
    else:
        _launch_pack(jobs)


def sync_external_shadows(model):
    for layer in getattr(model, "layers", []):
        layer._shadow_ver = layer._packed_ver = None
    ref = model.__dict__.get("_shadow_sync")
    fn = ref() if ref is not None else None
    if fn is not None:
        fn()


class EncoderLayer(nn.Module):
    fused = True
    act_dtype = torch.float32

    def __init__(self, hidden_size, ffn_size, dropout_rate, attention_dropout_rate, num_heads):
        super().__init__()
        self.self_attention_norm = nn.LayerNorm(hidden_size)
        self.self_attention = MultiHeadAttention(hidden_size, attention_dropout_rate, num_heads)
        self.self_attention_dropout = nn.Dropout(dropout_rate)
        self.ffn_norm = nn.LayerNorm(hidden_size)
        self.ffn = FeedForwardNetwork(hidden_size, ffn_size, dropout_rate)
        self.ffn_dropout = nn.Dropout(dropout_rate)

    def forward(self, x, attn_bias=None, mask=None, next_layer=None):
        if self.fused and x.is_cuda and mask is None:
            return fused_layer_forward(self, "stock", x, attn_bias, self.ffn_norm, self.self_attention_norm, next_layer=next_layer)
        y = self.self_attention_norm(x)
        y = self.self_attention(y, y, y, attn_bias, mask=mask)
        y = self.self_attention_dropout(y)
        x = x + y.to(x.dtype)
        y = self.ffn_norm(x)
        y = self.ffn(y)
        y = self.ffn_dropout(y)
        return x + y.to(x.dtype)


class Graphormer(nn.Module):

    def __init__(self, n_layers, num_heads, hidden_dim, dropout_rate, intput_dropout_rate, weight_decay, ffn_dim,
                 dataset_name, warmup_updates, tot_updates, peak_lr, end_lr, edge_type, multi_hop_max_dist,
                 attention_dropout_rate, num_class=1, bias_dtype=torch.float32, act_dtype=torch.float32, fused_layers=True,
                 num_atoms=512 * 9 + 1, **_unused):
        super().__init__()
        self.num_heads = num_heads
        self.atom_encoder = nn.Embedding(num_atoms, hidden_dim, padding_idx=0)
        self.edge_encoder = nn.Embedding(512 * 3 + 1, num_heads, padding_idx=0)
        self.edge_type = edge_type
        if self.edge_type == "multi_hop":
            self.edge_dis_encoder = nn.Embedding(128 * num_heads * num_heads, 1)
        self.rel_pos_encoder = nn.Embedding(512, num_heads, padding_idx=0)
        self.in_degree_encoder = nn.Embedding(512, hidden_dim, padding_idx=0)
        self.out_degree_encoder = nn.Embedding(512, hidden_dim, padding_idx=0)
        self.input_dropout = nn.Dropout(intput_dropout_rate)
        self.layers = nn.ModuleList([EncoderLayer(hidden_dim, ffn_dim, dropout_rate, attention_dropout_rate, num_heads)
                                     for _ in range(n_layers)])
        for li, layer in enumerate(self.layers):
            layer.act_dtype, layer.fused = act_dtype, fused_layers
            layer.self_attention.set_layer_index(li + 1)
        self.final_ln = nn.LayerNorm(hidden_dim)
        self.downstream_out_proj = nn.Linear(hidden_dim, num_class)
        self.graph_token = nn.Embedding(1, hidden_dim)
        self.graph_token_virtual_distance = nn.Embedding(1, num_heads)
        self.dataset_name = dataset_name
        self.warmup_updates, self.tot_updates = warmup_updates, tot_updates
        self.peak_lr, self.end_lr, self.weight_decay = peak_lr, end_lr, weight_decay
        self.multi_hop_max_dist = multi_hop_max_dist
        self.hidden_dim = hidden_dim
        self.bias_dtype = bias_dtype
        self.apply(lambda module: init_bert_params(module, n_layers=n_layers))

    def _hop_depth(self, batched_data):
        D = batched_data.edge_input.shape[3]
        if self.multi_hop_max_dist > 0:
            D = min(D, self.multi_hop_max_dist)
        if self.edge_type != "multi_hop":
            raise NotImplementedError("only edge_type='multi_hop' is used by MobGT (README.md:62)")
        return D

    def assemble_bias(self, batched_data, hop=None):
        H = self.num_heads
        edge_input = batched_data.edge_input
        D = self._hop_depth(batched_data)
        if hop is None:
            hop = hop_table_from(self.edge_encoder.weight, self.edge_dis_encoder.weight, H, D)
        rel = self.rel_pos_encoder.weight
        return ops.build_bias(batched_data.attn_bias, batched_data.rel_pos, None, edge_input, rel, None, hop,
                              self.graph_token_virtual_distance.weight, D, dtype=self.bias_dtype)

    def validate_batch(self, batched_data):
        if getattr(batched_data, "_mobgt_validated", None) is self or not batched_data.x.is_cuda:
            return
        if torch.cuda.is_current_stream_capturing():
            return
        lim = [("x", batched_data.x, self.atom_encoder.num_embeddings), ("in_degree", batched_data.in_degree, self.in_degree_encoder.num_embeddings),
               ("rel_pos", batched_data.rel_pos, self.rel_pos_encoder.num_embeddings),
               ("edge_input", batched_data.edge_input, self.edge_encoder.num_embeddings),
               ("y", batched_data.y, self.downstream_out_proj.out_features)]
        mx = torch.stack([t.max().long() if t.numel() else torch.zeros((), dtype=torch.long, device=t.device) for _, t, _ in lim]).tolist()
        mn = int(batched_data.y.min()) if batched_data.y.numel() else 0
        for (name, _, n), m in zip(lim, mx):
            if m >= n:
                raise IndexError(f"batch.{name} has index {m}, out of range for a table of {n} rows")
        if mn < 0:
            raise IndexError(f"batch.y has the negative class {mn}")
        try:
            batched_data._mobgt_validated = self
        except AttributeError:
            pass

    def index_limits(self):
        return dict(x=self.atom_encoder.num_embeddings - 1, y=self.downstream_out_proj.out_features - 1,
                    edge=self.edge_encoder.num_embeddings, deg=self.in_degree_encoder.num_embeddings)

    def forward(self, batched_data, perturb=None):
        self.validate_batch(batched_data)
        x = batched_data.x
        in_degree = out_degree = batched_data.in_degree
        n_graph = x.size(0)
        if x.shape[2] != 1:
            raise NotImplementedError("MobGT items have one feature column (wrapper.py:37)")
        xi = x.reshape(x.shape[0], x.shape[1])
# ... 60 lines not shown
```

### mobgt_amd/ops.py

```python
import contextlib
import ctypes
import math

import torch

from . import _lib, forms
from ._lib import F32, BF16, I64, I32, I16, U8, check
from .step_state import STEP

_DT = {torch.float32: F32, torch.bfloat16: BF16}
BIAS_LONG_PAIRS, HOP_DMAX, TOPK_MAX = _lib.LIBRARY.constants("BIAS_LONG_PAIRS", "HOP_DMAX", "TOPK_MAX_K")
SKINNY_MAX_G, SKINNY_MAX_K, SKINNY_MFMA_MAX_K, SKINNY_MFMA_K_STEP = _lib.LIBRARY.constants(
    "SKINNY_MAX_G", "SKINNY_MAX_K", "SKINNY_MFMA_MAX_K", "SKINNY_MFMA_K_STEP")
_IT = {torch.int64: I64, torch.int32: I32, torch.int16: I16, torch.uint8: U8}


def _stream():
    return ctypes.c_void_p(torch.cuda.current_stream().cuda_stream)


def _p(t):
    return ctypes.c_void_p(t.data_ptr()) if t is not None else ctypes.c_void_p(0)


def _require_cuda(*ts):
    for t in ts:
        if t is not None and not t.is_cuda:
            raise RuntimeError("mobgt_amd ops run on the GPU only (there is no CPU fallback); got a CPU tensor")




def _ws_word(ws, off):
    return ws.view(torch.int32)[off // 4:off // 4 + 1]


def _scrub_exchange_area(ws, fault_off):
    ws[fault_off + 4:].zero_()
    torch.cuda.synchronize()


def peer_wait_faults(reset=True):
    from . import fused_layer
    lib = _lib.lib()
    dev = torch.cuda.current_device()
    torch.cuda.synchronize(dev)
    out = {}
    for key, ws in fused_layer._CHAIN_WS.items():
        if key[0] != dev:
            continue
        off = int(lib.mobgt_chain_ws_fault_offset())
        w = _ws_word(ws, off)
        n = int(w.item())
        if n:
            out["chain"] = out.get("chain", 0) + n
            if reset:
                w.zero_()
                _scrub_exchange_area(ws, off)
    ws = _HEAD_WS.get(dev)
    if ws is not None:
        off = int(lib.mobgt_head_chain_ws_fault_offset())
        w = _ws_word(ws, off)
        n = int(w.item())
        if n:
            out["head"] = n
            if reset:
                w.zero_()
                _scrub_exchange_area(ws, off)
    c = ctypes.c_uint32(0)
    _lib.call("mobgt_small_gcn_faults", 1 if reset else 0, ctypes.byref(c))
    if c.value:
        out["small_gcn"] = int(c.value)
    return out


def set_peer_wait_limit(rounds=0, gcn_ticks=0):
    from . import fused_layer
    lib = _lib.lib()
    dev = torch.cuda.current_device()
    rounds = int(rounds) & 0xFFFFFFFF
    rounds = rounds - (1 << 32) if rounds >= (1 << 31) else rounds
    for key, ws in fused_layer._CHAIN_WS.items():
        if key[0] == dev:
            _ws_word(ws, int(lib.mobgt_chain_ws_limit_offset())).fill_(int(rounds))
    ws = _HEAD_WS.get(dev)
    if ws is not None:
        _ws_word(ws, int(lib.mobgt_head_chain_ws_limit_offset())).fill_(int(rounds))
    _lib.call("mobgt_small_gcn_set_wait_limit", int(gcn_ticks))
    torch.cuda.synchronize()


class ZeroArena:

    def __init__(self, device, n=1 << 20):
        self.buf = torch.zeros(n, dtype=torch.float32, device=device)
        self.off = 0

    def reset(self):
        self.buf.zero_()
        self.off = 0

    def take(self, n):
        n4 = (n + 3) // 4 * 4
        if self.off + n4 > self.buf.numel():
            return None
        t = self.buf[self.off:self.off + n]
        self.off += n4
        return t


def set_zero_arena(arena):
    STEP.zero_arena = arena


def zeros_f32(shape, device):
    n = 1
    for d in (shape if isinstance(shape, (tuple, list, torch.Size)) else (shape,)):
        n *= int(d)
    a = STEP.zero_arena
    if a is not None and a.buf.device == torch.device(device):
        t = a.take(n)
        if t is not None:
            return t.view(shape)
    return torch.zeros(shape, dtype=torch.float32, device=device)


def set_grad_sinks(params, views):
    import weakref
    STEP.grad_sinks = {p.data_ptr(): (weakref.ref(p), v) for p, v in zip(params, views)} if params is not None else {}


def sink_census_begin():
    STEP.sink_census.update(on=True, cur={}, max={})


def sink_census_pass():
    c = STEP.sink_census
    for k, n in c["cur"].items():
        if n > c["max"].get(k, 0):
            c["max"][k] = n
    c["cur"] = {}


def sink_census_end():
    sink_census_pass()
    c = STEP.sink_census
    out, c["on"], c["max"] = c["max"], False, {}
    return out


def grad_sink(param):
    c = STEP.sink_census
    if c["on"]:
        c["cur"][id(param)] = c["cur"].get(id(param), 0) + 1
    e = STEP.grad_sinks.get(param.data_ptr())
    if e is not None and e[0]() is param and e[1].shape == param.shape:
        return e[1]
    return None


def round_up(x, m):
    return (x + m - 1) // m * m


class PackedBias:

    def __init__(self, G, H, T, dtype, device):
        self.G, self.H, self.T = G, H, T
        self.ld = round_up(T, 64)
        self.dtype = dtype
        self.bias = torch.empty(G, H, T, self.ld, dtype=dtype, device=device)
        self.bias_t = torch.empty(G, H, T, self.ld, dtype=dtype, device=device)
        self.dbias = None
        self.n_use = 0
        self.n_bwd = 0
        self.needs_grad = False
        self.token = None
        self.spent = False

    def dense(self):
        return self.bias[..., : self.T].float()

    @property
    def sliced(self):
        return self.dtype == torch.bfloat16

    def grad_buffer(self):
        if self.dbias is None:
            shape = (self.G, self.H, self.T, self.ld)
            if self.sliced:
                self.dbias = torch.empty((max(self.n_use, 1),) + shape, dtype=torch.bfloat16, device=self.bias.device)
            else:
                self.dbias = torch.zeros(shape, dtype=torch.float32, device=self.bias.device)
        return self.dbias

    def next_grad_slice(self):
        buf = self.grad_buffer()
        i = self.n_bwd
        self.n_bwd += 1
        if not self.sliced:
            return buf, 1 if i > 0 else 0
        if i >= buf.shape[0]:
            raise RuntimeError("PackedBias: more attention backward passes than forward uses of this bias")
        return buf[i], 0

    def grad_total(self):
        if self.dbias is None:
            return None
        if self.sliced:
            return self.dbias[: max(self.n_bwd, 1), ..., : self.T].float().sum(0)
        return self.dbias[..., : self.T]


class _PackFn(torch.autograd.Function):
    @staticmethod
    def forward(ctx, src, pack):
        G, H, T = pack.G, pack.H, pack.T
        s = src.expand(G, H, T, T)
        st = s.stride()
        _lib.call("mobgt_bias_pack", _p(s), _DT[s.dtype], st[0], st[1], st[2], st[3], _p(pack.bias), _p(pack.bias_t),
                  _DT[pack.dtype], G, H, T, pack.ld, _stream())
        ctx.pack = pack
        ctx.src_shape = src.shape
        ctx.src_dtype = src.dtype
        ctx.set_materialize_grads(False)
        return zeros_f32((1,), src.device)

    @staticmethod
    def backward(ctx, _g):
        pack = ctx.pack
        pack.spent = True
        if pack.dbias is None:
            return torch.zeros(ctx.src_shape, dtype=ctx.src_dtype, device=pack.bias.device), None
        g = pack.grad_total()
        if tuple(ctx.src_shape) != tuple(g.shape):
            g = g.sum_to_size(ctx.src_shape)
        return g.to(ctx.src_dtype), None


def pack_bias(attn_bias, G, H, T, dtype=None):
    _require_cuda(attn_bias)
    if attn_bias.dtype not in _DT:
        attn_bias = attn_bias.float()
    if attn_bias.dim() == 3:
        attn_bias = attn_bias.unsqueeze(1)
    pack = PackedBias(G, H, T, dtype or attn_bias.dtype, attn_bias.device)
    pack.needs_grad = attn_bias.requires_grad and torch.is_grad_enabled()
    pack.token = _PackFn.apply(attn_bias, pack)
    return pack




def front_deferral(on):
    STEP.front_on = bool(on) and forms.on("front_passengers")


def take_front_jobs():
    hop, ni = STEP.front_hop, STEP.front_ni
    STEP.front_hop = STEP.front_ni = None
    return hop, ni


def flush_front():
    hop, ni = take_front_jobs()
    if hop is not None:
        _lib.call("mobgt_hop_table_fwd", *hop[0], _stream())
    if ni is not None:
        _lib.call("mobgt_node_index", *ni[0], _stream())


def _bias_bwd_alloc(shapes, dev, sinks=(None, None, None, None)):
    return tuple(None if sh is None else (k[:] if (k is not None and tuple(k.shape) == tuple(sh)) else zeros_f32(sh, dev))
                 for sh, k in zip(shapes, sinks))


def take_bias_bwd_job():
    job, STEP.bias_bwd_job = STEP.bias_bwd_job, None
    if job is None or not forms.on("bias_bwd_passenger"):
        return None
    pack = job["pack"]()
    if pack is None or pack.dbias is None or not pack.sliced or pack.n_use < 1 or pack.n_bwd < pack.n_use:
        return None
    G, N, H, D_in, D, F, n_rel, n_poi, n_edge, ld, idx_dt, edge_dt = job["args"]
    if not (idx_dt == I16 and edge_dt == U8 and H == 8 and 0 < D <= HOP_DMAX and F == 1 and G * (N + 1) * (N + 1) < BIAS_LONG_PAIRS
            and job["idx"][3] is not None):
        return None
    return job


def bias_bwd_job_args(job):
    pack = job["pack"]()
    outs = _bias_bwd_alloc(job["shapes"], pack.bias.device, job.get("sinks", (None,) * 4))
    attn_bias, rel_pos, poi_pos, edge_input = job["idx"]
    n_sl = max(pack.n_bwd, 1) if pack.sliced else 1
    stride = pack.dbias.stride(0) if pack.sliced else 0
    args = [_p(pack.dbias), _DT[pack.dbias.dtype], n_sl, stride, _p(attn_bias), _p(rel_pos), _p(poi_pos), _p(edge_input),
            _p(outs[0]), _p(outs[1]), _p(outs[2]), _p(outs[3]), *job["args"]]
    return outs, args


class _BuildBiasFn(torch.autograd.Function):
    @staticmethod
    def forward(ctx, rel_table, poi_table, hop_table, vdist, pack, attn_bias, rel_pos, poi_pos, edge_input, D, sinks=(None,) * 4):
        G, N = rel_pos.shape[:2]
        H = rel_table.shape[1]
        has_edge = edge_input is not None and D > 0
        D_in = edge_input.shape[3] if has_edge else 0
        F = edge_input.shape[4] if has_edge else 1
# ... 901 lines not shown
    STEP.token_fwd_on = bool(on) and forms.on("token_fwd_chain") and not _NAN_TRACE["on"]


def flush_token_fwd():
    for k in ("gather", "f2", "f4"):
        rec = STEP.token_fwd.pop(k, None)
        if rec is not None:
            rec["launch"]()


class _GatherMultiFn(torch.autograd.Function):

    @staticmethod
    def forward(ctx, spec, out_widths, n, *args):
        tables, idx = args[:n], args[n:]
        R = idx[0].numel()
        dev = tables[0].device
        outs = [torch.empty(R, w, dtype=torch.float32, device=dev) for w in out_widths]
        ci, i64, vp = ctypes.c_int, ctypes.c_int64, ctypes.c_void_p

        def launch():
            _lib.call("mobgt_embed_gather_multi",
                n, _ptr_array(tables), None, _ptr_array(idx), (i64 * n)(*[sp[3] for sp in spec]),
                (ci * n)(*[t.shape[1] for t in tables]), (ci * n)(*[sp[1] for sp in spec]), (ci * n)(*[int(sp[2]) for sp in spec]),
                (vp * n)(*[outs[sp[0]].data_ptr() for sp in spec]), (i64 * n)(*[outs[sp[0]].stride(0) for sp in spec]), R,
                _IT[idx[0].dtype], 0, None, 0, _stream())
        if STEP.token_fwd_on and "gather" not in STEP.token_fwd and len(outs) == 3 and all(i_.dtype == idx[0].dtype for i_ in idx):
            STEP.token_fwd["gather"] = dict(launch=launch, tables=tables, idx=idx, spec=spec, outs=outs, R=R)
        else:
            launch()
        ctx.idx, ctx.spec, ctx.n = idx, spec, n
        ctx.ptrs = [t.data_ptr() for t in tables]
        ctx.shapes = [t.shape for t in tables]
        ctx.sinks = [grad_sink(t) for t in tables]
        return tuple(outs)

    @staticmethod
    def backward(ctx, *douts):
        n, spec = ctx.n, ctx.spec
        dev = ctx.idx[0].device
        R = ctx.idx[0].numel()
        gbuf = []
        for g in douts:
            if g is not None and (g.stride(1) != 1 or g.stride(0) % 4 or g.data_ptr() % 16 or g.dtype != torch.float32):
                g = g.float().contiguous()
            gbuf.append(g)
        grads = [(ctx.sinks[t][:] if ctx.sinks[t] is not None else zeros_f32(tuple(sh), dev))
                 if (ctx.needs_input_grad[3 + t] and gbuf[spec[t][0]] is not None) else None for t, sh in enumerate(ctx.shapes)]
        jobs = [t for t in range(n) if grads[t] is not None]
        if jobs:
            m = len(jobs)
            ci, i64, vp = ctypes.c_int, ctypes.c_int64, ctypes.c_void_p
            extra, extra_job = None, 0
            for k, t in enumerate(jobs):
                pend = _ROW0_PENDING.pop(ctx.ptrs[t], None)
                if pend is not None:
                    extra, extra_job = pend, k
            _lib.call("mobgt_embed_gather_multi",
                m, None, (vp * m)(*[grads[t].data_ptr() for t in jobs]), (vp * m)(*[ctx.idx[t].data_ptr() for t in jobs]),
                (i64 * m)(*[spec[t][3] for t in jobs]), (ci * m)(*[ctx.shapes[t][1] for t in jobs]),
                (ci * m)(*[spec[t][1] for t in jobs]), None, (vp * m)(*[gbuf[spec[t][0]].data_ptr() for t in jobs]),
                (i64 * m)(*[gbuf[spec[t][0]].stride(0) for t in jobs]), R, _IT[ctx.idx[0].dtype], 1, _p(extra), extra_job,
                _stream())
        return (None, None, None, *grads, *([None] * n))


def embed_gather_multi(jobs, out_widths):
    n = len(jobs)
    tabs = [j[0].float().contiguous() for j in jobs]
    idx = [j[1].contiguous().reshape(-1) for j in jobs]
    _require_cuda(*tabs, *idx)
    spec = tuple((int(j[2]), int(j[3]), int(j[4]), -1 if j[5] is None else int(j[5])) for j in jobs)
    for k, sp in enumerate(spec):
        assert sp[2] != 2 or (k > 0 and tabs[k].shape[1] == tabs[k - 1].shape[1] and not tabs[k].requires_grad
                              and (k < 4 or any(s_[2] != 2 for s_ in spec[k - 3:k]))), "fold job (at most three per gather)"
    return list(_GatherMultiFn.apply(spec, tuple(out_widths), n, *tabs, *idx))


class _JoinColsFn(torch.autograd.Function):

    @staticmethod
    def forward(ctx, whole, part):
        ctx.w = part.shape[1]
        return whole.detach().view_as(whole)

    @staticmethod
    def backward(ctx, g):
        return g, g[:, :ctx.w]


def join_cols(whole, part):
    return _JoinColsFn.apply(whole, part)


class _GradientTailLossFn(torch.autograd.Function):
    @staticmethod
    def forward(ctx, logits, targets, alpha, target_offset):
        logits = logits.float().contiguous()
        G, V = logits.shape
        dlogits = torch.empty_like(logits)
        loss = torch.empty((), dtype=torch.float32, device=logits.device)
        _lib.call("mobgt_gradient_tail_loss", _p(logits), _p(targets.long().contiguous()), int(target_offset), _p(dlogits),
                  _p(loss), G, V, float(alpha), _stream())
        ctx.save_for_backward(dlogits)
        return loss

    @staticmethod
    def backward(ctx, g):
        (dlogits,) = ctx.saved_tensors
        if g.data_ptr() == unit_grad(g.device).data_ptr():
            return dlogits, None, None, None
        return dlogits * g, None, None, None


class _StockTokensFn(torch.autograd.Function):
    @staticmethod
    def forward(ctx, x, din, dout, atom, indeg, outdeg, gtok, p, seed, seed_dev, salt, padding_idx):
        G, N = x.shape
        C = atom.shape[1]
        y = torch.empty(G, N + 1, C, dtype=torch.float32, device=atom.device)
        tok = (_p(x), _p(din), _p(dout), _IT[x.dtype], _IT[din.dtype], _p(atom), _p(indeg), _p(outdeg), _p(gtok), _p(y),
               G, N, C, atom.shape[0], indeg.shape[0], outdeg.shape[0], p, seed, _p(seed_dev), salt)
        hop, ni = take_front_jobs() if STEP.front_on else (None, None)
        if ni is not None:
            _lib.call("mobgt_node_index", *ni[0], _stream())
        jobs = []
        if STEP.front_on:
            from .model import take_pending_pack
            jobs = take_pending_pack()
        if hop is not None or jobs:
            import ctypes
            vp, ci = ctypes.c_void_p, ctypes.c_int
            for o in range(96, len(jobs), 96):
                from .model import _launch_pack
                _launch_pack(jobs[o:o + 96])
            part = jobs[:96]
            nj = len(part)
            pack = ((vp * nj)(*[j[0].data_ptr() for j in part]), (vp * nj)(*[j[1].data_ptr() for j in part]), (ci * nj)(*[j[2] for j in part]),
                    (ci * nj)(*[j[3] for j in part]), (ci * nj)(*[j[4] for j in part])) if nj else (None, None, None, None, None)
            hargs = [1] + hop[0] if hop is not None else [0, None, None, None, 0, 0, 0, 0]
            _lib.call("mobgt_stock_front_fwd", *tok, nj, *pack, *hargs, _stream())
        else:
            _lib.call("mobgt_stock_tokens_fwd", *tok, _stream())
        ctx.idx = (x, din, dout)
        ctx.misc = (p, seed, seed_dev, salt, padding_idx, [t.shape for t in (atom, indeg, outdeg, gtok)])
        ptrs = [t.data_ptr() for t in (atom, indeg, outdeg, gtok)]
        ctx.sinks = [grad_sink(t) if ptrs.count(t.data_ptr()) == 1 else None for t in (atom, indeg, outdeg, gtok)]
        return y

    @staticmethod
    def backward(ctx, dy):
        x, din, dout = ctx.idx
        p, seed, seed_dev, salt, padding_idx, shapes = ctx.misc
        G, N = x.shape
        dy = dy.contiguous()
        C = dy.shape[2]
        grads = [None if not need else (k[:] if (k is not None and tuple(k.shape) == tuple(sh)) else zeros_f32(tuple(sh), dy.device))
                 for need, k, sh in zip(ctx.needs_input_grad[3:7], ctx.sinks, shapes)]
        args = [_p(dy), _p(x), _p(din), _p(dout), _IT[x.dtype], _IT[din.dtype], _p(grads[0]), _p(grads[1]), _p(grads[2]),
                _p(grads[3]), G, N, C, shapes[0][0], shapes[1][0], shapes[2][0], int(padding_idx), p, seed, _p(seed_dev), salt]
        in_sinks = all((not need) or (k is not None and tuple(k.shape) == tuple(sh))
                       for need, k, sh in zip(ctx.needs_input_grad[3:7], ctx.sinks, shapes))
        if STEP.wgrad_on and in_sinks and STEP.wgrad_stock_tok is None and forms.on("stock_tail"):
            STEP.wgrad_stock_tok = (args, (dy, x, din, dout, seed_dev, grads))
            return (None, None, None, *[g_[:] if g_ is not None else None for g_ in grads], None, None, None, None, None)
        _lib.call("mobgt_stock_tokens_bwd", *args, _stream())
        return (None, None, None, *grads, None, None, None, None, None)


def stock_tokens_ok(x, atom, indeg, outdeg, gtok):
    return (x.is_cuda and x.dim() == 2 and x.dtype in _IT and atom.shape[1] % 4 == 0
            and all(t.dtype == torch.float32 and t.is_contiguous() and t.data_ptr() % 16 == 0 for t in (atom, indeg, outdeg, gtok)))


def stock_tokens(x, in_degree, out_degree, atom, indeg, outdeg, graph_token, p, training, salt, padding_idx=0):
    _require_cuda(x, atom)
    assert in_degree.dtype == out_degree.dtype and in_degree.dtype in _IT and in_degree.dtype != torch.uint8 and x.dtype != torch.uint8
    if not training:
        p = 0.0
    seed, seed_dev = _DROPOUT_STATE["seed"], _DROPOUT_STATE["seed_dev"]
    if seed_dev is None and p > 0:
        seed = (seed + int(torch.randint(0, 2 ** 31 - 1, (1,)).item())) & 0x7FFFFFFFFFFFFFFF
    return _StockTokensFn.apply(x.contiguous(), in_degree.contiguous(), out_degree.contiguous(), atom, indeg, outdeg, graph_token,
                                float(p), int(seed), seed_dev, int(salt) & 0xFFFFFFFF, int(padding_idx))


class _TokenLayerNormFn(torch.autograd.Function):
    @staticmethod
    def forward(ctx, enc, weight, bias, eps):
        enc = enc.contiguous()
        G, T, C = enc.shape
        y = torch.empty(G, C, dtype=torch.float32, device=enc.device)
        stat = torch.empty(2, G, dtype=torch.float32, device=enc.device)
        _lib.call("mobgt_token_ln_fwd", _p(enc), _p(weight), _p(bias), _p(y), _p(stat[0]), _p(stat[1]), G, T, C, float(eps),
                  _stream())
        ctx.save_for_backward(enc, weight, stat)
        ctx.sinks = (grad_sink(weight), grad_sink(bias))
        return y

    @staticmethod
    def backward(ctx, dy):
        enc, weight, stat = ctx.saved_tensors
        G, T, C = enc.shape
        denc = torch.empty_like(enc)
        dg, db = (k[:] if k is not None else zeros_f32((C,), enc.device) for k in ctx.sinks)
        _lib.call("mobgt_token_ln_bwd", _p(dy.contiguous()), _p(enc), _p(stat[0]), _p(stat[1]), _p(weight), _p(denc), _p(dg), _p(db),
                  G, T, C, _stream())
        return denc, dg, db, None


def token_layer_norm_ok(enc, weight):
    return (enc.is_cuda and enc.dim() == 3 and enc.dtype == torch.float32 and weight.dtype == torch.float32
            and enc.shape[2] <= 1024)


def token_layer_norm(enc, weight, bias, eps=1e-5):
    _require_cuda(enc, weight, bias)
    return _TokenLayerNormFn.apply(enc, weight.contiguous(), bias.contiguous(), eps)


class _CrossEntropyFn(torch.autograd.Function):
    @staticmethod
    def forward(ctx, logits, targets, ignore_index):
        logits = logits.float().contiguous()
        G, V = logits.shape
        dlogits = torch.empty_like(logits)
        loss = torch.empty((), dtype=torch.float32, device=logits.device)
        _lib.call("mobgt_cross_entropy", _p(logits), _p(targets.long().contiguous()), int(ignore_index), _p(dlogits), _p(loss), G, V,
                  _stream())
        ctx.save_for_backward(dlogits)
        return loss

    @staticmethod
    def backward(ctx, g):
        (dlogits,) = ctx.saved_tensors
        if g.data_ptr() == unit_grad(g.device).data_ptr():
            return dlogits, None, None
        return dlogits * g, None, None


def cross_entropy_ok(logits, targets):
    return (logits.is_cuda and logits.dim() == 2 and 0 < logits.shape[0] <= 4095 and logits.shape[1] <= 10240
            and targets.numel() == logits.shape[0])


def cross_entropy(logits, targets, ignore_index=-100):
    _require_cuda(logits, targets)
    return _CrossEntropyFn.apply(logits, targets.reshape(-1), ignore_index)


_UNIT = {}


def unit_grad(device):
    device = torch.device(device)
    key = (device.type, device.index if device.index is not None else (torch.cuda.current_device() if device.type == "cuda" else 0))
    t = _UNIT.get(key)
    if t is None:
        t = torch.ones((), dtype=torch.float32, device=device)
        _UNIT[key] = t
    return t


def gradient_tail_loss(logits, targets, alpha=0.25, target_offset=0):
    _require_cuda(logits, targets)
    return _GradientTailLossFn.apply(logits, targets[: logits.shape[0]].reshape(-1), alpha, target_offset)


class OutRef:

    def __init__(self, t):
        self.t = t.detach()


def register_token_chain(nf, x4, w2_width, w4, slope4, w2, slope2):
    STEP.token_chain = None
    if not forms.on("token_bwd_chain"):
        return
    if (nf.is_cuda and nf.dtype == torch.float32 and x4.dtype == torch.float32 and nf.dim() == 2 and nf.is_contiguous()
            and x4.is_contiguous() and tuple(nf.shape) == tuple(x4.shape) and nf.shape[1] == 192 and w2_width == 160
            and tuple(w4.shape) == (192, 192) and tuple(w2.shape) == (160, 160) and w4.is_contiguous() and w2.is_contiguous()
            and w4.dtype == torch.float32 and w2.dtype == torch.float32):
        STEP.token_chain = dict(nf_ptr=nf.data_ptr(), nf=nf.detach(), x4=x4.detach(), w4=w4.detach(), slope4=float(slope4),
                                w2=w2.detach(), slope2=float(slope2))


def _token_park_linear(g, w, y):
    pend = STEP.token_pending.get(g.data_ptr())
    if pend is None:
        return None
    ent = pend["ent"]
    if pend["stage"] == 1 and w.data_ptr() == ent["w4"].data_ptr() and y is not None and y.data_ptr() == ent["nf_ptr"]:
        del STEP.token_pending[g.data_ptr()]
        dx4 = torch.empty_like(ent["x4"])
        pend.update(stage=2, dx4=dx4)
        STEP.token_pending[dx4.data_ptr()] = pend
        return dx4
    if pend["stage"] == 2 and w.data_ptr() == ent["w2"].data_ptr() and y is not None and y.data_ptr() == ent["x4"].data_ptr():
        del STEP.token_pending[g.data_ptr()]
        G, N, C, p_pos, p_in, seed, seed_dev, salts = pend["misc"]
        W2 = ent["w2"].shape[0]
        d_pt = torch.empty(G * N, W2, dtype=torch.float32, device=g.device)
        dx4 = pend["dx4"]
        _lib.call("mobgt_token_bwd_chain", _p(pend["dout"]), _p(pend["real"]), _p(ent["nf"]), _p(ent["x4"]), ent["x4"].stride(0),
                  _p(ent["w4"]), _p(ent["w2"]), _p(pend["d_nf"]), _p(pend["d_add"]), _p(dx4), dx4.stride(0),
                  _p(d_pt), _p(pend["d_tok"]), G, N, C, W2, ent["slope4"], ent["slope2"], p_pos, p_in, seed,
                  _p(seed_dev), salts[0], salts[1], salts[2], _stream())
        return d_pt
    return None


class _LinearSplitKFn(torch.autograd.Function):

    @staticmethod
    def forward(ctx, x, w, b, bf16_wgrad, slope, out=None):
        ctx.bf16_wgrad = bf16_wgrad
        ctx.slope = slope
        if _small_linear(x, w) & 1:
            rec, gat = STEP.token_fwd, STEP.token_fwd.get("gather") if STEP.token_fwd_on else None
            stage = None
            if gat is not None and slope is not None and b is not None and x.dtype == torch.float32 and w.dtype == torch.float32:
                if ("f2" not in rec and out is not None and x.data_ptr() == gat["outs"][0].data_ptr()
                        and out.t.data_ptr() == gat["outs"][1].data_ptr()):
                    stage = "f2"
                elif ("f2" in rec and "f4" not in rec and out is None
                        and x.data_ptr() == gat["outs"][1].data_ptr() and x.is_contiguous()):
                    stage = "f4"
            if stage is not None:
                y = out.t if out is not None else torch.empty(x.shape[0], w.shape[0], dtype=torch.float32, device=x.device)
                rec[stage] = dict(launch=lambda: small_gemm(x, w, b, True, leaky=slope, out=y), x=x, w=w, b=b, slope=slope, y=y)
            else:
                y = small_gemm(x, w, b, True, leaky=slope, out=out.t if out is not None else None)
            if out is not None:
                y = y.view_as(y)
        else:
            y = torch.addmm(b, x, w.t())
            if slope is not None:
                y = torch.nn.functional.leaky_relu(y, slope)
        ctx.save_for_backward(x, w, y if slope is not None else None)
        ctx.sinks = (grad_sink(w), grad_sink(b) if b is not None else None)
        return y

    @staticmethod
    def backward(ctx, g):
        x, w, y = ctx.saved_tensors
        k_w, k_b = ctx.sinks

        def dst(sink, shape):
            return sink[:] if sink is not None else zeros_f32(shape, g.device)
        if y is None or y.is_contiguous():
            g = g.contiguous()
        R = x.shape[0]
        hip_wgrad = (ctx.bf16_wgrad and g.dtype == torch.float32 and x.dtype == torch.float32 and g.shape[1] % 2 == 0
                     and x.shape[1] % 2 == 0 and R <= 4096 and g.data_ptr() % 8 == 0 and x.data_ptr() % 8 == 0)
        if y is not None:
            mv = act_mask_values(ctx.slope, 0.0)
            if (hip_wgrad and R <= 64 and small_gemm_ok(g, w) and y.is_contiguous() and y.data_ptr() % 8 == 0
                    and max(w.shape) <= 512):
                db = dst(k_b, (g.shape[1],))
                dw = linear_wgrad_masked(g, x, g_mask=y, mask_vals=mv, db=db, leaf=True, dw=dst(k_w, tuple(w.shape)))
                dx = _token_park_linear(g, w, y) if STEP.wgrad_on else None
                return (dx if dx is not None else small_gemm(g, w, a_mask=(y, *mv))), dw, (db[:] if STEP.wgrad_on else db), None, None, None
            if (STEP.wgrad_on and hip_wgrad and g.stride(1) == 1 and y.stride() == g.stride() and g.data_ptr() % 8 == 0
                    and y.data_ptr() % 8 == 0 and g.stride(0) % 2 == 0 and small_gemm_ok(g, w) and R <= _SMALL_ROWS
                    and max(w.shape) <= 512):
                db = dst(k_b, (g.shape[1],))
                dw = linear_wgrad_masked(g, x, g_mask=y, mask_vals=mv, db=db, leaf=True, dw=dst(k_w, tuple(w.shape)))
                dx = _token_park_linear(g, w, y)
                return (dx if dx is not None else small_gemm(g, w, a_mask=(y, *mv))), dw, db[:], None, None, None
            if (hip_wgrad and g.stride(1) == 1 and y.stride() == g.stride() and g.data_ptr() % 8 == 0 and y.data_ptr() % 8 == 0
                    and g.stride(0) % 2 == 0):
                gm = torch.empty_strided(g.shape, g.stride(), dtype=torch.float32, device=g.device)
                db = zeros_f32((g.shape[1],), g.device)
                dw = linear_wgrad_masked(g, x, g_mask=y, mask_vals=mv, db=db, g_out=gm)
                dx = small_gemm(gm, w) if (small_gemm_ok(gm, w) and R <= _SMALL_ROWS and max(w.shape) <= 512) else gm @ w
                return dx, dw, db, None, None, None
            g = torch.ops.aten.leaky_relu_backward(g, y, ctx.slope, True).contiguous()
        if hip_wgrad:
            dw, db = linear_wgrad(g, x, with_bias=True, leaf=True, dw=dst(k_w, tuple(w.shape)), db=dst(k_b, (g.shape[1],)))
            return (small_gemm(g, w) if _small_linear(g, w) & 2 else g @ w), dw, db, None, None, None
        s = max((c for c in (16, 8, 4, 2) if R % c == 0 and R // c >= 16), default=1)
        if s > 1:
            dw = torch.bmm(g.view(s, R // s, -1).transpose(1, 2), x.view(s, R // s, -1)).sum(0)
        else:
            dw = g.t() @ x
        return g @ w, dw, colsum(g), None, None, None


_SMALL_LINEAR = 1
_SMALL_ROWS = 4096


def _small_linear(x, w):
    ok = (x.is_cuda and x.dtype == torch.float32 and w.dtype == torch.float32 and x.dim() == 2 and x.shape[0] <= _SMALL_ROWS
          and max(w.shape) <= 512 and x.stride(1) == 1 and w.is_contiguous())
    if not ok:
        return 0
    return _SMALL_LINEAR if x.shape[0] <= 64 else (_SMALL_LINEAR & 1)


def linear_splitk(x, weight, bias, bf16_wgrad=False, slope=None, out=None):
    shape = x.shape
    x2 = x.reshape(-1, shape[-1]).contiguous()
    if out is not None and not (_small_linear(x2, weight) & 1 and out.shape == (x2.shape[0], weight.shape[0])):
        out = None
    y = _LinearSplitKFn.apply(x2, weight, bias, bf16_wgrad, slope, OutRef(out) if out is not None else None)
    return y if out is not None else y.view(*shape[:-1], weight.shape[0])


_DROPOUT_STATE = {"seed_dev": None, "seed": 0x5DEECE66D}


def set_dropout_state(seed_dev=None, seed=None):
    _DROPOUT_STATE["seed_dev"] = seed_dev
    if seed is not None:
        _DROPOUT_STATE["seed"] = int(seed)


class _DropoutFn(torch.autograd.Function):
    @staticmethod
    def forward(ctx, x, p, seed, seed_dev, salt):
        x = x.contiguous()
        y = torch.empty_like(x)
        row = x.shape[-1] if x.dim() > 1 else x.numel()
        _lib.call("mobgt_dropout", _p(x), _p(y), x.numel(), row, p, seed, _p(seed_dev), salt, _stream())
        ctx.misc = (p, seed, seed_dev, salt, row)
        return y

    @staticmethod
    def backward(ctx, g):
        p, seed, seed_dev, salt, row = ctx.misc
        g = g.contiguous()
        dx = torch.empty_like(g)
        _lib.call("mobgt_dropout", _p(g), _p(dx), g.numel(), row, p, seed, _p(seed_dev), salt, _stream())
        return dx, None, None, None, None


def dropout(x, p, training, salt):
    if not training or p <= 0.0:
        return x
    _require_cuda(x)
    seed, seed_dev = _DROPOUT_STATE["seed"], _DROPOUT_STATE["seed_dev"]
    if seed_dev is None:
        seed = (seed + int(torch.randint(0, 2 ** 31 - 1, (1,)).item())) & 0x7FFFFFFFFFFFFFFF
    return _DropoutFn.apply(x.float(), float(p), int(seed), seed_dev, int(salt) & 0xFFFFFFFF)


class _BiasActFn(torch.autograd.Function):
    @staticmethod
    def forward(ctx, x, bias, slope, p_drop, seed, seed_dev, salt, yt=None):
        x = x.contiguous()
        R, C = x.shape
        y = torch.empty_like(x)
        _lib.call("mobgt_bias_act_fwd_t", _p(x), _p(bias), _p(y), _p(yt.t if yt is not None else None),
                  yt.t.stride(0) if yt is not None else 0, R, C, slope, p_drop, seed, _p(seed_dev), salt,
                  _stream())
        ctx.save_for_backward(y)
        ctx.misc = (slope, p_drop, seed, seed_dev, salt, bias is not None)
        return y

    @staticmethod
    def backward(ctx, dy):
        (y,) = ctx.saved_tensors
        slope, p_drop, seed, seed_dev, salt, has_bias = ctx.misc
        R, C = y.shape
        dx = torch.empty_like(y)
        db = zeros_f32((C,), y.device) if has_bias else None
        _lib.call("mobgt_bias_act_bwd", _p(dy.contiguous()), _p(y), _p(dx), _p(db), R, C, slope, p_drop, seed, _p(seed_dev),
                  salt, _stream())
        return dx, db, None, None, None, None, None, None


def dropout_seed(p_drop):
    seed, seed_dev = _DROPOUT_STATE["seed"], _DROPOUT_STATE["seed_dev"]
    if seed_dev is None and p_drop > 0:
        seed = (seed + int(torch.randint(0, 2 ** 31 - 1, (1,)).item())) & 0x7FFFFFFFFFFFFFFF
    return int(seed), seed_dev


def bias_act(x, bias, slope, p_drop, training, salt, yt=None):
    _require_cuda(x)
    if not training:
        p_drop = 0.0
    seed, seed_dev = _DROPOUT_STATE["seed"], _DROPOUT_STATE["seed_dev"]
    if seed_dev is None and p_drop > 0:
        seed = (seed + int(torch.randint(0, 2 ** 31 - 1, (1,)).item())) & 0x7FFFFFFFFFFFFFFF
    return _BiasActFn.apply(x.float(), bias, float(slope), float(p_drop), int(seed), seed_dev, int(salt) & 0xFFFFFFFF,
                            OutRef(yt) if yt is not None else None)


class _HeadActFn(torch.autograd.Function):
    @staticmethod
    def forward(ctx, u, w, b, eps, slope, p_drop, seed, seed_dev, salt):
        u, w, b = u.contiguous(), w.contiguous(), b.contiguous()
        R, C = u.shape
        out = torch.empty_like(u)
        stats = torch.empty(2, R, dtype=torch.float32, device=u.device)
        _lib.call("mobgt_head_act_fwd", _p(u), _p(w), _p(b), _p(out), _p(stats[0]), _p(stats[1]), R, C, eps, slope, p_drop,
                  seed, _p(seed_dev), salt, _stream())
        ctx.save_for_backward(u, w, b, stats)
        ctx.misc = (eps, slope, p_drop, seed, seed_dev, salt)
        return out

    @staticmethod
    def backward(ctx, dout):
        u, w, b, stats = ctx.saved_tensors
        eps, slope, p_drop, seed, seed_dev, salt = ctx.misc
        R, C = u.shape
        du = torch.empty_like(u)
        dg, db = zeros_f32((C,), u.device), zeros_f32((C,), u.device)
        _lib.call("mobgt_head_act_bwd", _p(dout.contiguous()), _p(u), _p(w), _p(b), _p(stats[0]), _p(stats[1]), _p(du),
                  _p(dg), _p(db), R, C, eps, slope, p_drop, seed, _p(seed_dev), salt, _stream())
        return du, dg, db, None, None, None, None, None, None


def head_act(u, ln_weight, ln_bias, eps, slope, p_drop, training, salt):
    _require_cuda(u, ln_weight, ln_bias)
    if not training:
        p_drop = 0.0
    seed, seed_dev = _DROPOUT_STATE["seed"], _DROPOUT_STATE["seed_dev"]
    if seed_dev is None and p_drop > 0:
        seed = (seed + int(torch.randint(0, 2 ** 31 - 1, (1,)).item())) & 0x7FFFFFFFFFFFFFFF
    return _HeadActFn.apply(u.float(), ln_weight, ln_bias, float(eps), float(slope), float(p_drop), int(seed), seed_dev,
                            int(salt) & 0xFFFFFFFF)


class _HeadChainFn(torch.autograd.Function):

    @staticmethod
    def forward(ctx, enc, table, user, offset, w3, b3, ln_w, ln_b, eps, slope, p_drop, seed, seed_dev, salt, bf16_wgrad):
        G, T, C = enc.shape
        U = table.shape[1]
        W = C + U
        dev = enc.device
        x3, u3, out = (torch.empty(G, W, dtype=torch.float32, device=dev) for _ in range(3))
        stats = torch.empty(2, G, dtype=torch.float32, device=dev)
        _lib.call("mobgt_head_chain_fwd", _p(enc), _p(user), _IT[user.dtype], offset, _p(table), table.shape[0], _p(w3), _p(b3),
                  _p(ln_w), _p(ln_b), _p(x3), _p(u3), _p(out), _p(stats[0]), _p(stats[1]), G, T, C, U,
                  eps, slope, p_drop, seed, _p(seed_dev), salt, _p(_head_chain_ws(dev)), _stream())
        ctx.save_for_backward(x3, u3, stats, w3, ln_w, ln_b)
        ctx.user = user
        ctx.misc = (G, T, C, U, offset, tuple(table.shape), eps, slope, p_drop, seed, seed_dev, salt, bf16_wgrad)
        ctx.sink = grad_sink(table)
        ctx.psinks = (grad_sink(w3), grad_sink(b3), grad_sink(ln_w), grad_sink(ln_b))
        return out

    @staticmethod
    def backward(ctx, dout):
        x3, u3, stats, w3, ln_w, ln_b = ctx.saved_tensors
        G, T, C, U, offset, tshape, eps, slope, p_drop, seed, seed_dev, salt, bf16_wgrad = ctx.misc
        dev = dout.device
        dout = dout.contiguous()
        du3 = torch.empty_like(u3)
        denc = torch.empty(G, T, C, dtype=torch.float32, device=dev)
        dtable = ctx.sink[:] if ctx.sink is not None else zeros_f32(tshape, dev)
        k_w3, k_b3, k_g, k_beta = ctx.psinks
        dg = k_g[:] if k_g is not None else zeros_f32((C + U,), dev)
        dbeta = k_beta[:] if k_beta is not None else zeros_f32((C + U,), dev)
        _lib.call("mobgt_head_chain_bwd", _p(dout), _p(u3), _p(stats[0]), _p(stats[1]), _p(ctx.user), _IT[ctx.user.dtype], offset,
                  tshape[0], _p(w3), _p(ln_w), _p(ln_b), _p(du3), _p(denc), _p(dtable), _p(dg), _p(dbeta),
                  G, T, C, U, eps, slope, p_drop, seed, _p(seed_dev), salt, _stream())
        if bf16_wgrad:
            dw, db = linear_wgrad(du3, x3, with_bias=True, leaf=True, dw=k_w3[:] if k_w3 is not None else None,
                                  db=k_b3[:] if k_b3 is not None else None)
        else:
            dw, db = du3.t() @ x3, colsum(du3)
        return denc, dtable, None, None, dw, db, dg, dbeta, None, None, None, None, None, None, None


_HEAD_WS = {}


def _head_chain_ws(dev):
    key = dev.index if dev.index is not None else torch.cuda.current_device()
    ws = _HEAD_WS.get(key)
    if ws is None:
        if torch.cuda.is_current_stream_capturing():
            raise RuntimeError("the head kernel's workspace must be allocated before graph capture: run one eager step first")
        ws = _HEAD_WS[key] = torch.zeros(int(_lib.lib().mobgt_head_chain_ws_bytes()), dtype=torch.uint8, device=dev)
    return ws


def head_chain_ok(enc, table, user, w3):
    W = enc.shape[-1] + table.shape[1]
    return (enc.is_cuda and enc.dim() == 3 and enc.dtype == torch.float32 and table.dtype == torch.float32 and table.is_contiguous()
            and W in (320, 384) and tuple(w3.shape) == (W, W) and w3.dtype == torch.float32 and w3.is_contiguous()
            and user.dtype in (torch.int64, torch.int32) and user.numel() == enc.shape[0] and enc.shape[0] <= 160
            and enc.shape[-1] % 16 == 0 and table.shape[1] % 16 == 0 and not forms.on("safe_forms"))


def head_chain(enc, user_table, user, user_offset, w3, b3, ln_weight, ln_bias, eps, slope, p_drop, training, salt, bf16_wgrad=False):
    _require_cuda(enc, user_table, user, w3)
    if not training:
        p_drop = 0.0
    seed, seed_dev = _DROPOUT_STATE["seed"], _DROPOUT_STATE["seed_dev"]
    if seed_dev is None and p_drop > 0:
        seed = (seed + int(torch.randint(0, 2 ** 31 - 1, (1,)).item())) & 0x7FFFFFFFFFFFFFFF
    return _HeadChainFn.apply(enc.contiguous(), user_table, user.reshape(-1).contiguous(), int(user_offset), w3, b3.contiguous(),
                              ln_weight.contiguous(), ln_bias.contiguous(), float(eps), float(slope), float(p_drop), int(seed),
                              seed_dev, int(salt) & 0xFFFFFFFF, bool(bf16_wgrad))


class _HeadInputFn(torch.autograd.Function):
    @staticmethod
    def forward(ctx, enc, table, user, offset):
        G, T, C = enc.shape
        U = table.shape[1]
        x3 = torch.empty(G, C + U, dtype=torch.float32, device=enc.device)
        _lib.call("mobgt_head_input_fwd", _p(enc), _p(user), _IT[user.dtype], offset, _p(table), table.shape[0], _p(x3),
                  G, T, C, U, _stream())
        ctx.user, ctx.misc = user, (G, T, C, U, offset, table.shape)
        ctx.sink = grad_sink(table)
        return x3

    @staticmethod
    def backward(ctx, dx3):
        G, T, C, U, offset, tshape = ctx.misc
        dx3 = dx3.contiguous()
        denc = torch.empty(G, T, C, dtype=torch.float32, device=dx3.device)
        dtable = ctx.sink[:] if ctx.sink is not None else zeros_f32(tuple(tshape), dx3.device)
        _lib.call("mobgt_head_input_bwd", _p(dx3), _p(ctx.user), _IT[ctx.user.dtype], offset, _p(denc), _p(dtable),
                  tshape[0], G, T, C, U, _stream())
        return denc, dtable, None, None


def head_input(enc, user_table, user, user_offset=0):
    _require_cuda(enc, user_table, user)
    assert enc.dtype == torch.float32 and user_table.dtype == torch.float32 and user.dtype in (torch.int64, torch.int32)
    assert user_table.is_contiguous()
    return _HeadInputFn.apply(enc.contiguous(), user_table, user.reshape(-1).contiguous(), int(user_offset))


def _token_fwd_fused(nf, real, add, token, pe0, out, out16, qkv_w, qkv, G, N, C, p_pos, p_in, seed, seed_dev, salts):
    gat, f2, f4 = (STEP.token_fwd.get(k) for k in ("gather", "f2", "f4"))
    ok = (gat is not None and f2 is not None and f4 is not None and C == 192 and gat["R"] == G * N and len(gat["outs"]) == 3
          and nf.data_ptr() == f4["y"].data_ptr() and add.data_ptr() == gat["outs"][2].data_ptr()
          and tuple(f2["w"].shape) == (160, 160) and tuple(f4["w"].shape) == (192, 192)
          and gat["outs"][0].shape[1] == 160 and gat["outs"][1].shape[1] == 192 and gat["outs"][2].shape[1] == 192
          and all(t.is_contiguous() for t in (f2["w"], f2["b"], f4["w"], f4["b"], *gat["outs"]))
          and (pe0.dim() == 1 or pe0.shape[0] >= 1))
    if not ok:
        flush_token_fwd()
        return False
    tables, idx, spec = gat["tables"], gat["idx"], gat["spec"]
    n = len(tables)
    ci = ctypes.c_int
    rc = (_lib.lib().mobgt_token_fwd_chain(
        n, _ptr_array(tables), _ptr_array(idx), (ci * n)(*[t.shape[1] for t in tables]), (ci * n)(*[sp[1] for sp in spec]),
        (ci * n)(*[int(sp[2]) for sp in spec]), (ci * n)(*[sp[0] for sp in spec]), _IT[idx[0].dtype],
        _p(gat["outs"][0]), _p(gat["outs"][1]), _p(gat["outs"][2]), _p(f4["y"]), 160,
        _p(f2["w"]), _p(f2["b"]), float(f2["slope"]), _p(f4["w"]), _p(f4["b"]), float(f4["slope"]),
        _p(real), _p(token), _p(pe0), _p(out), _p(out16), _p(qkv_w[0].t), _p(qkv_w[1].t), _p(qkv), G, N, C, p_pos, p_in, seed,
        _p(seed_dev), salts[0], salts[1], salts[2], _stream()))
    if rc == _lib.CONSTANTS["MOBGT_EBADDIM"]:
        flush_token_fwd()
        return False
    check(rc, "mobgt_token_fwd_chain")
    STEP.token_fwd = {}
    STEP.token_fwd_fused_calls += 1
    return True


class _AssembleTokensFn(torch.autograd.Function):
    @staticmethod
    def forward(ctx, nf, real, add, token, pe0, p_pos, p_in, seed, seed_dev, salts, side, row0_via_gather=False, qkv_w=None, tok_sink=None):
        ctx.tok_sink = tok_sink
        ctx.pe_ptr = pe0.data_ptr() if (row0_via_gather and pe0.dim() == 2 and pe0.shape[0] > 1) else None
        ctx.nf_ptr = nf.data_ptr()
        G, N, C = nf.shape
        nf, add, real = nf.contiguous(), add.contiguous(), real.contiguous()
        shapes = (token.shape, pe0.shape)
        token = token.reshape(-1).contiguous()
        pe0 = pe0.contiguous() if pe0.dim() == 2 and pe0.shape[0] > 1 else pe0.reshape(-1).contiguous()
        out = torch.empty(G, N + 1, C, dtype=torch.float32, device=nf.device)
        out16 = torch.empty(G, N + 1, C, dtype=torch.bfloat16, device=nf.device) if side is not None else None
        if qkv_w is not None and out16 is not None and C in (192, 256):
            qkv = torch.empty(G * (N + 1), 3 * C, dtype=torch.bfloat16, device=nf.device)
            if not _token_fwd_fused(nf, real, add, token, pe0, out, out16, qkv_w, qkv, G, N, C, p_pos, p_in, seed, seed_dev, salts):
                _lib.call("mobgt_assemble_tokens_qkv", _p(nf), _p(real), _p(add), _p(token), _p(pe0), _p(out), _p(out16),
                          _p(qkv_w[0].t), _p(qkv_w[1].t), _p(qkv), G, N, C, p_pos, p_in, seed,
                          _p(seed_dev), salts[0], salts[1], salts[2], _stream())
            side.append(out16)
            side.append(qkv)
        else:
            flush_token_fwd()
            _lib.call("mobgt_assemble_tokens_fwd", _p(nf), _p(real), _p(add), _p(token), _p(pe0), _p(out), _p(out16), G, N, C,
                      p_pos, p_in, seed, _p(seed_dev), salts[0], salts[1], salts[2], _stream())
            if side is not None:
                side.append(out16)
        ctx.save_for_backward(real)
        ctx.misc = (G, N, C, p_pos, p_in, seed, seed_dev, salts, shapes)
        return out

    @staticmethod
    def backward(ctx, dout):
        (real,) = ctx.saved_tensors
        G, N, C, p_pos, p_in, seed, seed_dev, salts, (tshape, pshape) = ctx.misc
        dout = dout.contiguous()
        d_nf = torch.empty(G, N, C, dtype=torch.float32, device=dout.device)
        d_add = torch.empty(G, N, C, dtype=torch.float32, device=dout.device)
        k_tok = ctx.tok_sink
        if ctx.pe_ptr is not None:
            d_tok = k_tok.view(-1)[:] if (k_tok is not None and k_tok.numel() == C) else zeros_f32((C,), dout.device)
            d_pe = None
        elif len(pshape) == 2 and pshape[0] > 1:
            d_pe = zeros_f32(tuple(pshape), dout.device)
            d_tok = d_pe[0]
        else:
            d_tok = zeros_f32((C,), dout.device)
            d_pe = d_tok.view(pshape)
        ent = STEP.token_chain
        if (ent is not None and ent["nf_ptr"] == ctx.nf_ptr and STEP.wgrad_on and C == ent["nf"].shape[1]
                and G * N == ent["nf"].shape[0] and forms.on("token_bwd_chain")):
            STEP.token_pending[d_nf.data_ptr()] = dict(stage=1, ent=ent, dout=dout, real=real, d_nf=d_nf, d_add=d_add, d_tok=d_tok,
                                                       misc=(G, N, C, p_pos, p_in, seed, seed_dev, salts))
        else:
            _lib.call("mobgt_assemble_tokens_bwd", _p(dout), _p(real), _p(d_nf), _p(d_add), _p(d_tok), G, N, C, p_pos, p_in, seed,
                      _p(seed_dev), salts[0], salts[1], salts[2], _stream())
        if ctx.pe_ptr is not None:
            _ROW0_PENDING[ctx.pe_ptr] = d_tok
            return d_nf, None, d_add, d_tok.view(tshape), None, None, None, None, None, None, None, None, None, None
        return d_nf, None, d_add, d_tok.view(tshape), d_pe, None, None, None, None, None, None, None, None, None


def assemble_tokens(nf, real, add, token, pe0, p_pos, p_in, training, salts=(0x1001, 0x1002, 0x1003), bf16_copy=False,
                    pe_row0_via_gather=False, first_qkv=None):
    _require_cuda(nf, add, token, pe0)
    if not training:
        p_pos = p_in = 0.0
    seed, seed_dev = _DROPOUT_STATE["seed"], _DROPOUT_STATE["seed_dev"]
    if seed_dev is None and (p_pos > 0 or p_in > 0):
        seed = (seed + int(torch.randint(0, 2 ** 31 - 1, (1,)).item())) & 0x7FFFFFFFFFFFFFFF
    side = [] if bf16_copy else None
    out = _AssembleTokensFn.apply(nf.float(), real.float(), add.float(), token.float(), pe0.float(), float(p_pos),
                                  float(p_in), int(seed), seed_dev, tuple(int(s) & 0xFFFFFFFF for s in salts), side,
                                  bool(pe_row0_via_gather and pe0.requires_grad and torch.is_grad_enabled()),
                                  (OutRef(first_qkv[0]), OutRef(first_qkv[1])) if (first_qkv is not None and bf16_copy) else None,
                                  grad_sink(token) if token.is_contiguous() else None)
    if side:
        out._mobgt_act = side[0]
        if len(side) > 1:
            out._mobgt_qkv = side[1]
    return out


def small_gemm(a, b, bias=None, b_is_nk=False, out=None, out_dtype=torch.float32, leaky=None, drop=None, a_mask=None, ct=None,
               k_b=None):
    _require_cuda(a, b)
    assert a.dtype == torch.float32 and b.dtype == torch.float32 and a.dim() == 2 and b.dim() == 2
    assert a.stride(1) == 1 and b.stride(1) == 1
    pre = STEP.front_sgemm.get("done")
    if pre is not None:
        if (pre["key"] == (a.data_ptr(), b.data_ptr(), bias.data_ptr() if bias is not None else 0, leaky, k_b,
                           ct[0].data_ptr() if ct else 0) and drop is None and a_mask is None and out is None and not b_is_nk):
            del STEP.front_sgemm["done"]
            return pre["c"]
    M, K = a.shape
    N = b.shape[0] if b_is_nk else b.shape[1]
    assert (b.shape[1] if b_is_nk else b.shape[0]) == (K if k_b is None else k_b) and (k_b is None or (not b_is_nk and k_b <= K))
    if bias is not None:
        assert bias.dtype == torch.float32 and bias.numel() == N and bias.is_contiguous()
    only_t = ct is not None and ct[2]
    c = None if only_t else (out if out is not None else torch.empty(M, N, dtype=out_dtype, device=a.device))
    if leaky is None and a_mask is None and ct is None and k_b is None:
        _lib.call("mobgt_small_gemm_f32", _p(a), a.stride(0), _p(b), b.stride(0), int(b_is_nk), _p(bias), _p(c), c.stride(0),
                  _DT[c.dtype], M, N, K, _stream())
        return c
    y, pos, neg, zer = a_mask if a_mask is not None else (None, 1.0, 1.0, 1.0)
    if y is not None:
        assert y.dtype == torch.float32 and y.shape == a.shape and y.stride(1) == 1 and y.stride(0) == a.stride(0)
    p_drop, seed, seed_dev, salt = drop if drop is not None else (0.0, 0, None, 0)
    _lib.call("mobgt_small_gemm_f32_act", _p(a), a.stride(0), _p(y), float(pos), float(neg), float(zer), _p(b), b.stride(0),
              int(b_is_nk), _p(bias), int(leaky is not None), float(leaky or 0.0), float(p_drop),
              int(seed), _p(seed_dev), int(salt) & 0xFFFFFFFF, _p(c), c.stride(0) if c is not None else N,
              _DT[c.dtype] if c is not None else F32, _p(ct[0] if ct else None),
              ct[0].stride(0) if ct else 0, _p(ct[1] if ct else None), M, N, K, int(k_b or 0),
              _stream())
    return c


def front_small_gemm(a, b, bias, leaky, k_b, ct):
    STEP.front_sgemm = {}
    if (not forms.on("l0_ride") or not (a.is_cuda and a.dtype == torch.float32 and b.dtype == torch.float32
            and a.is_contiguous() and b.is_contiguous() and bias is not None and bias.is_contiguous())):
        return False
    M, K = a.shape
    N = b.shape[1]
    c = torch.empty(M, N, dtype=torch.float32, device=a.device)
    rc = _lib.lib().mobgt_front_sgemm_job(_p(a), a.stride(0), _p(b), b.stride(0), _p(bias), 1, float(leaky), _p(c), c.stride(0),
                                          _p(ct), ct.stride(0) if ct is not None else 0, M, N, K, int(k_b))
    if rc != 0:
        return False
    STEP.front_sgemm["job"] = dict(key=(a.data_ptr(), b.data_ptr(), bias.data_ptr(), leaky, k_b, ct.data_ptr() if ct is not None else 0),
                                   c=c, args=(a, b, bias, leaky, k_b, ct))
    return True


def front_small_gemm_flush():
    job = STEP.front_sgemm.pop("job", None)
    if job is None:
        return
    if _lib.lib().mobgt_front_sgemm_pending():
        _lib.call("mobgt_front_sgemm_job", None, 0, None, 0, None, 0, 0.0, None, 0, None, 0, 0, 0, 0, 0)
        a, b, bias, leaky, k_b, ct = job["args"]
        job["c"] = small_gemm(a, b, bias, leaky=leaky, k_b=k_b, ct=(ct, None, False) if ct is not None else None)
    STEP.front_sgemm["done"] = job


def graph_task_id():
    fn = getattr(torch._C, "_current_graph_task_id", None)
    return int(fn()) if fn is not None else -1


def drop_parked():
    if "job" in STEP.front_sgemm:
        _lib.call("mobgt_front_sgemm_job", None, 0, None, 0, None, 0, 0.0, None, 0, None, 0, 0, 0, 0, 0)
    STEP.drop_parked(graph_task_id())


def act_mask_values(slope, p_drop):
    if p_drop and p_drop > 0.0:
        thr = int(p_drop * 65536.0 + 0.5)
        ik = 1.0 / (1.0 - thr / 65536.0)
        return ik, slope * ik, 0.0
    return 1.0, slope, slope


@contextlib.contextmanager
def recording_wgrads(on=True):
    STEP.wgrad_on = bool(on)
    try:
        yield
        flush_deferred_wgrads()
    except BaseException:
        drop_parked()
        raise
    finally:
        STEP.wgrad_on = False


def defer_partial_sum(part, dst):
    if not (STEP.wgrad_on and dst is not None and part.dtype == torch.float32 and dst.dtype == torch.float32
            and part.is_contiguous() and dst.is_contiguous() and part.dim() == 3 and dst.numel() == part[0].numel()
            and dst.numel() % 4 == 0 and part.data_ptr() % 16 == 0 and dst.data_ptr() % 16 == 0
            and forms.on("psum_defer")):
        return None
    STEP.wgrad_psum.append((part, dst))
    return dst[:]


def layer_wgrad_big(items, R):
    lib = _lib.lib()
    n = len(items)
    vp, i64, ci = ctypes.c_void_p, ctypes.c_int64, ctypes.c_int
    tiles = sum(lib.mobgt_layer_wgrad_big_tiles(g.shape[1], x.shape[1]) for g, x, _, _ in items)
    S = lib.mobgt_layer_wgrad_big_splits(R, tiles)
    dev = items[0][0].device
    parts = [torch.empty(S, g.shape[1], x.shape[1], dtype=torch.float32, device=dev) for g, x, _, _ in items]
    _lib.call("mobgt_layer_wgrad_big", n, (vp * n)(*[t[0].data_ptr() for t in items]), (i64 * n)(*[t[0].stride(0) for t in items]),
              (vp * n)(*[t[1].data_ptr() for t in items]), (i64 * n)(*[t[1].stride(0) for t in items]),
              (vp * n)(*[q.data_ptr() for q in parts]),
              (vp * n)(*[(t[2].data_ptr() if t[2] is not None else None) for t in items]),
              (ci * n)(*[t[0].shape[1] for t in items]), (ci * n)(*[t[1].shape[1] for t in items]), R, S,
              _stream())
    outs = []
    for part, (_, _, _, sink) in zip(parts, items):
        parked = defer_partial_sum(part, sink) if sink is not None else None
        outs.append(parked if parked is not None else part.sum(0))
    return outs


def layer_wgrad_big_ok(items):
    return (1 <= len(items) <= 4 and all(
        g.dtype == torch.bfloat16 and x.dtype == torch.bfloat16 and g.dim() == 2 and x.dim() == 2 and g.shape[0] == x.shape[0]
        and g.stride(1) == 1 and x.stride(1) == 1 and g.shape[1] % 8 == 0 and x.shape[1] % 8 == 0 and g.stride(0) % 8 == 0
        and x.stride(0) % 8 == 0 and g.data_ptr() % 16 == 0 and x.data_ptr() % 16 == 0
        and g.shape[0] * g.stride(0) * 2 < (1 << 31) and x.shape[0] * x.stride(0) * 2 < (1 << 31) for g, x, _, _ in items))


def _wgrad_defer(g, x, g_mask, x_mask, mask_vals, dw, db, db_of_x):
    STEP.wgrad_items.append((g, x, g_mask, x_mask, tuple(float(v) for v in mask_vals), dw, db, bool(db_of_x)))
    return dw[:]


def step_state_leftovers():
    return STEP.leftovers()


def flush_deferred_wgrads():
    if STEP.token_pending:
        stages = [p_["stage"] for p_ in STEP.token_pending.values()]
        raise RuntimeError(f"a parked encoder-input backward chain was never completed (stages {stages}): gradients of this "
                           "step are invalid -- set MOBGT_NO_TOKEN_BWD_CHAIN=1 and report")
    items, hop, psum, tok, wide = STEP.wgrad_items, STEP.wgrad_hop, STEP.wgrad_psum, STEP.wgrad_stock_tok, STEP.wgrad_hop_wide
    STEP.wgrad_items, STEP.wgrad_hop, STEP.wgrad_psum, STEP.wgrad_stock_tok, STEP.wgrad_hop_wide = [], None, [], None, None
    for o in range(0, len(psum), 48):
        part = psum[o:o + 48]
        n = len(part)
        _lib.call("mobgt_partial_sum_multi", n, (ctypes.c_void_p * n)(*[p_[0].data_ptr() for p_ in part]),
                  (ctypes.c_void_p * n)(*[p_[1].data_ptr() for p_ in part]),
                  (ctypes.c_int * n)(*[p_[0].shape[0] for p_ in part]),
                  (ctypes.c_int64 * n)(*[p_[1].numel() for p_ in part]), _stream())
    if tok is not None and wide is not None:
        dtab, ew, dw_, d_ew, d_dw, D, E, rt = wide
        _lib.call("mobgt_stock_tail_bwd", *tok[0], _p(dtab), _p(ew), _p(dw_), _p(d_ew), _p(d_dw), D, E, 8, rt, _stream())
    elif tok is not None:
        _lib.call("mobgt_stock_tokens_bwd", *tok[0], _stream())
    elif wide is not None:
        _hop_table_bwd(wide)
    vp, i64, ci, cf = ctypes.c_void_p, ctypes.c_int64, ctypes.c_int, ctypes.c_float
    if hop is not None and not items:
        _hop_table_bwd(hop)
        hop = None
    for o in range(0, len(items), 32):
        part = items[o:o + 32]
        n = len(part)
        if hop is not None:
            dtab, ew, dw_, d_ew, d_dw, D, E, rt = hop
            hop_args = [1, _p(dtab), _p(ew), _p(dw_), _p(d_ew), _p(d_dw), D, E, rt]
            hop = None
        else:
            hop_args = [0, None, None, None, None, None, 0, 0, 0]
        ptr = lambda t: t.data_ptr() if t is not None else None
        mv = []
        for it in part:
            mv += list(it[4])
        _lib.call("mobgt_linear_wgrad_multi_hop",
            n, (vp * n)(*[ptr(it[0]) for it in part]), (i64 * n)(*[it[0].stride(0) for it in part]),
            (vp * n)(*[ptr(it[1]) for it in part]), (i64 * n)(*[it[1].stride(0) for it in part]),
            (vp * n)(*[ptr(it[2]) for it in part]), (vp * n)(*[ptr(it[3]) for it in part]), (cf * (3 * n))(*mv),
            (vp * n)(*[ptr(it[5]) for it in part]), (i64 * n)(*[it[5].stride(0) for it in part]),
            (vp * n)(*[ptr(it[6]) for it in part]), (ci * n)(*[int(it[7]) for it in part]),
            (i64 * n)(*[it[0].shape[0] for it in part]), (ci * n)(*[it[0].shape[1] for it in part]),
            (ci * n)(*[it[1].shape[1] for it in part]), (ci * n)(*[1 if it[0].dtype == torch.float32 else 0 for it in part]),
            *hop_args, _stream())


def linear_wgrad_masked(g, x, g_mask=None, x_mask=None, mask_vals=(1.0, 1.0, 1.0), db=None, db_of_x=False, dw=None, g_out=None,
                        leaf=False):
    _require_cuda(g, x)
    R, M = g.shape
    N = x.shape[1]
    assert g.dtype == torch.float32 and x.dtype == torch.float32 and g.stride(1) == 1 and x.stride(1) == 1
    for m, t in ((g_mask, g), (x_mask, x)):
        assert m is None or (m.dtype == torch.float32 and m.shape == t.shape and m.stride() == t.stride())
    if dw is None:
        dw = zeros_f32((M, N), g.device)
    assert dw.dim() == 2 and dw.stride(1) == 1
    assert g_out is None or (g_mask is not None and g_out.shape == g.shape and g_out.stride() == g.stride())
    if leaf and STEP.wgrad_on and g_out is None and M % 2 == 0 and N % 2 == 0:
        return _wgrad_defer(g, x, g_mask, x_mask, mask_vals, dw, db, db_of_x)
    _lib.call("mobgt_linear_wgrad_masked", _p(g), g.stride(0), _p(x), x.stride(0), _p(g_mask), _p(x_mask), float(mask_vals[0]),
              float(mask_vals[1]), float(mask_vals[2]), _p(g_out), _p(dw), dw.stride(0), _p(db), int(db_of_x),
              R, M, N, _stream())
    return dw


def small_gemm_ok(a, b):
    return (a.is_cuda and a.dtype == torch.float32 and b.dtype == torch.float32 and a.dim() == 2 and b.dim() == 2
            and a.stride(1) == 1 and b.stride(1) == 1)


GEMM_BIAS, GEMM_GELU, GEMM_GELU_BWD, GEMM_ADD = (_lib.CONSTANTS["MOBGT_GEMM_" + n] for n in ("BIAS", "GELU", "GELU_BWD", "ADD"))


def layer_gemm_ok(a, b, b_is_kn=False):
    if a.dtype != torch.bfloat16 or b.dtype != torch.bfloat16 or a.dim() != 2 or b.dim() != 2:
        return False
    M, K = a.shape
    N = b.shape[1] if b_is_kn else b.shape[0]
    if (b.shape[0] if b_is_kn else b.shape[1]) != K:
        return False
    return (K % 32 == 0 and N % 8 == 0 and a.stride(1) == 1 and b.stride(1) == 1 and a.stride(0) % 8 == 0
            and b.stride(0) % (2 if b_is_kn else 8) == 0 and a.data_ptr() % 16 == 0 and b.data_ptr() % 16 == 0
            and M <= 4096)


def layer_gemm(a, b, bias=None, b_is_kn=False, epilogue=GEMM_BIAS, aux_in=None):
    _require_cuda(a, b)
    M, K = a.shape
    N = b.shape[1] if b_is_kn else b.shape[0]
    dev = a.device
    aux_out = None
    if epilogue == GEMM_ADD:
        assert aux_in.dtype == torch.float32 and aux_in.shape == (M, N) and aux_in.is_contiguous()
        c = aux_in
    else:
        c = torch.empty(M, N, dtype=torch.bfloat16, device=dev)
        if epilogue == GEMM_GELU:
            aux_out = torch.empty(M, N, dtype=torch.bfloat16, device=dev)
        elif epilogue == GEMM_GELU_BWD:
            assert aux_in.dtype == torch.bfloat16 and aux_in.shape == (M, N) and aux_in.is_contiguous()
    if bias is not None:
        assert bias.dtype == torch.bfloat16 and bias.numel() == N and bias.is_contiguous()
    _lib.call("mobgt_layer_gemm", _p(a), a.stride(0), _p(b), b.stride(0), int(b_is_kn), _p(bias), _p(c), N, epilogue,
              _p(aux_in), _p(aux_out), M, N, K, _stream())
    return (c, aux_out) if epilogue == GEMM_GELU else c


_NAN_TRACE = {"flags": None, "names": [], "on": False}


def nan_trace_enable(device, slots=256):
    _NAN_TRACE.update(flags=torch.zeros(slots, dtype=torch.float32, device=device), names=[], on=True)


def trace_nan(name, t, grad=True):
    if not _NAN_TRACE["on"] or t is None:
        return t
    names, flags = _NAN_TRACE["names"], _NAN_TRACE["flags"]
    if name not in names:
        names.append(name)
        if grad:
            names.append("d/" + name)
    i = names.index(name)
    flags[i:i + 1].copy_(torch.isnan(t.detach()).any().float().reshape(1))
    if grad and t.requires_grad:
        j = names.index("d/" + name)
        def _hook(g, j=j):
            flags[j:j + 1].copy_(torch.isnan(g).any().float().reshape(1))
            return None
        t.register_hook(_hook)
    return t


def nan_trace_report():
    f = _NAN_TRACE["flags"].cpu().tolist()
    return [(n, bool(f[i])) for i, n in enumerate(_NAN_TRACE["names"])]


def linear_wgrad(g, x, with_bias=False, db=None, out_bias=None, leaf=False, dw=None):
    _require_cuda(g)
    R, M = g.shape
    N = x.shape[1]
    assert g.dtype == x.dtype and g.dtype in (torch.bfloat16, torch.float32) and g.stride(1) == 1 and x.stride(1) == 1
    if dw is None:
        dw = zeros_f32((M, N), g.device)
    assert dw.dim() == 2 and dw.stride(1) == 1
    if out_bias is not None:
        assert db is None and not with_bias and out_bias.dtype == torch.float32 and out_bias.numel() == N
        _lib.call("mobgt_linear_wgrad_bias", _p(g), g.stride(0), _p(x), x.stride(0), _p(out_bias.contiguous()), _p(dw), dw.stride(0), R, M, N,
                  _DT[g.dtype], _stream())
        return dw, None
    if db is None and with_bias:
        db = zeros_f32((M,), g.device)
# ... 15 lines not shown
```

### mobgt_amd/step_state.py

```python
import contextlib
from collections import namedtuple

PARKED, CARRIED, SWITCH = "parked", "carried", "switch"
Field = namedtuple("Field", "name scope new doc")
_none = type(None)

FIELDS = (
    Field("zero_arena", SWITCH, _none, "TrainStep._prologue sets the step's ZeroArena; ops.zeros_f32 carves from it"),
    Field("grad_sinks", CARRIED, dict, "TrainStep (ops.set_grad_sinks): parameter address -> (weak parameter, gradient view); ops.grad_sink reads"),
    Field("sink_census", SWITCH, lambda: {"on": False, "cur": {}, "max": {}}, "train.used_parameters' dry run counts ops.grad_sink requests per forward"),
    Field("bias_bwd_job", PARKED, _none, "_BuildBiasFn.forward parks; the category GCN's backward launch, the side stream or its own backward takes"),
    Field("front_on", SWITCH, bool, "the model's forward (ops.front_deferral) around the hop table and the node indices"),
    Field("front_hop", PARKED, _none, "_HopTableFn.forward parks; the category GCN's / stock front's forward launch or ops.flush_front takes"),
    Field("front_ni", PARKED, _none, "ops.node_index parks; the same launches take"),
    Field("token_fwd_on", SWITCH, bool, "model_fqandtoyo.node_features (ops.token_fwd_deferral)"),
    Field("token_fwd", PARKED, dict, "'gather' / 'f2' / 'f4': _GatherMultiFn / _LinearSplitKFn.forward record; _AssembleTokensFn launches them as one"),
    Field("token_fwd_fused_calls", CARRIED, int, "how often mobgt_token_fwd_chain took the three records (a counter for tests)"),
    Field("token_chain", CARRIED, _none, "ops.register_token_chain: the encoder-input chain of the forward that just ran; its backward reads it"),
    Field("token_pending", PARKED, dict, "_AssembleTokensFn.backward parks under a gradient's address; FuseEmbeddings-4 / -2's backward re-park / launch"),
    Field("front_sgemm", PARKED, dict, "'job': ops.front_small_gemm parks, the bias assembly's launch takes; 'done': its result until ops.small_gemm asks"),
    Field("wgrad_on", SWITCH, bool, "ops.recording_wgrads around the trainer's backward"),
    Field("wgrad_items", PARKED, list, "leaf weight gradients (ops.linear_wgrad*, fused layers) for ops.flush_deferred_wgrads' grouped launch"),
    Field("wgrad_hop", PARKED, _none, "_HopTableFn.backward parks; rides in the flush's first grouped launch"),
    Field("wgrad_hop_wide", PARKED, _none, "_HopTableFn.backward past 256 edge ids; shares the flush's stock tail launch"),
    Field("wgrad_stock_tok", PARKED, _none, "_StockTokensFn.backward parks; the flush's stock tail launch takes"),
    Field("wgrad_psum", PARKED, list, "ops.defer_partial_sum: split-K partial sums for the flush's one reduction launch"),
    Field("layer_tails", PARKED, dict, "(graph task, device, address of dx1) -> a fused layer's tail; the chain launch of the layer below takes"),
    Field("tail_check_task", PARKED, _none, "graph task whose end-of-backward check (fused_layer._pending_check) is queued"),
    Field("weight_pack", PARKED, list, "model.pack_layer_weights(defer=True) parks; the category GCN's / stock front's forward launch takes"),
    Field("gcn_prelaunched", PARKED, dict, "modelGNN.prelaunch_small_gcn: id(module) -> (key, result); that module's forward adopts it"),
)


class StepState:
    def __init__(self):
        for f in FIELDS:
            setattr(self, f.name, f.new())

    def leftovers(self):
        held = {f.name: getattr(self, f.name) for f in FIELDS if f.scope == PARKED}
        return {k: sorted(map(str, v)) if isinstance(v, dict) else len(v) if isinstance(v, list) else type(v).__name__
                for k, v in held.items() if v is not None and v != [] and v != {}}

    def drop_stale_tails(self, task_id):
        if self.tail_check_task != task_id:
            self.tail_check_task = None
        for k in [k for k in self.layer_tails if k[0] != task_id]:
            del self.layer_tails[k]

    def drop_parked(self, task_id=-1):
        self.drop_stale_tails(task_id)
        for f in FIELDS:
            if f.scope == PARKED and f.name not in ("layer_tails", "tail_check_task"):
                setattr(self, f.name, f.new())

    @contextlib.contextmanager
    def keeping_carried(self):
        saved = {f.name: getattr(self, f.name) for f in FIELDS if f.scope == CARRIED}
        try:
            yield
        finally:
            for k, v in saved.items():
                setattr(self, k, v)


STEP = StepState()
```

Baseline: 26950.

## Fuse first encoder layer's backward tail into token backward chain kernel

Adds a new native library whose kernel runs the first encoder layer's deferred tail (the dqkv x Wqkv^T bf16 MFMA that feeds dx1, plus up to four weight-gradient items) inside the token backward chain launch. Previously the tail ran as a separate launch before the token chain. The aim is fewer kernel launches and less round-tripping of dx1 through memory in the backward pass. It adds eligibility checks and a new code path that is only taken under graph capture, or when an eager flag is set, for small row counts.

```diff
diff --git a/__graft_entry__.py b/__graft_entry__.py
--- a/__graft_entry__.py
+++ b/__graft_entry__.py
@@ -39,6 +39,9 @@
     from mobgt_amd import _ctxprior
     _ctxprior.LIBRARY.build()
     _ctxprior.LIBRARY.lib()
+    from mobgt_amd import _tokhost
+    _tokhost.LIBRARY.build()
+    _tokhost.LIBRARY.lib()
     subprocess.check_call(["make", "-s", "-C", os.path.join(ROOT, "oracle")])
     import mobgt_amd
 
diff --git a/include/mobgt_tokhost.h b/include/mobgt_tokhost.h
--- /dev/null
+++ b/include/mobgt_tokhost.h
@@ -0,0 +1,30 @@
+#ifndef MOBGT_TOKHOST_H
+#define MOBGT_TOKHOST_H
+#include <stdint.h>
+
+#ifdef __cplusplus
+extern "C" {
+#endif
+
+#define MOBGT_TOKHOST_EBADDIM (-1)
+#define MOBGT_TOKHOST_EALIGN (-2)
+
+#define MOBGT_TOKHOST_ABI_VERSION 1
+int mobgt_tokhost_abi_version(void);
+
+#define MOBGT_TOKHOST_MAX_WG 4
+#define MOBGT_TOKHOST_MAX_ROWS 1024
+
+int mobgt_tokhost_token_bwd_chain(const float* dout, const float* real, const float* y4, const float* y2, int64_t ld_y2,
+                                  const float* w4, const float* w2, float* d_nf, float* d_add, float* dx4, int64_t ld_dx4,
+                                  float* d_pt, float* d_token, int G, int N, int C, int W2, float slope4, float slope2, float p_pos,
+                                  float p_in, uint64_t seed, const uint64_t* seed_dev, uint32_t salt_nf, uint32_t salt_tok,
+                                  uint32_t salt_in, const void* tail_dqkv, const void* tail_wqkv_t, float* dx1, int n_wg,
+                                  const void* const* wg_g, const int64_t* wg_ldg, const void* const* wg_x, const int64_t* wg_ldx,
+                                  float* const* wg_dw, const int64_t* wg_ldw, float* const* wg_db, const int* wg_M, const int* wg_N,
+                                  void* stream);
+
+#ifdef __cplusplus
+}
+#endif
+#endif
diff --git a/mobgt_amd/_tokhost.py b/mobgt_amd/_tokhost.py
--- /dev/null
+++ b/mobgt_amd/_tokhost.py
@@ -0,0 +1,15 @@
+from ._native import Library, NativeError
+
+
+class MobgtTokhostError(NativeError):
+    pass
+
+
+LIBRARY = Library("mobgt_tokhost.h", "csrc_tokhost", "libmobgt_tokhost.so", "MOBGT_TOKHOST_", error=MobgtTokhostError,
+                  missing="the first encoder layer's tail is hosted on the device only (MOBGT_NO_L0_TOKEN_HOST=1 does without).",
+                  errors={"EBADDIM": "size outside the supported limits, null buffer or inconsistent tail",
+                          "EALIGN": "pointer violates the documented alignment"})
+lib, launch = LIBRARY.lib, LIBRARY.launch
+SIGNATURES, CONSTANTS, ABI_VERSION = LIBRARY.SIGNATURES, LIBRARY.CONSTANTS, LIBRARY.ABI_VERSION
+MAX_WG, MAX_ROWS = LIBRARY.constants("MAX_WG", "MAX_ROWS")
+EBADDIM, EALIGN = LIBRARY.constants("EBADDIM", "EALIGN")
diff --git a/mobgt_amd/csrc/tokbwd.hip b/mobgt_amd/csrc/tokbwd.hip
--- a/mobgt_amd/csrc/tokbwd.hip
+++ b/mobgt_amd/csrc/tokbwd.hip
@@ -1,177 +1,6 @@
-#include "common.h"
-#include "mobgt_hip.h"
+#include "tokbwd_body.h"
 
-namespace {
-
-typedef __attribute__((ext_vector_type(4))) float f32x4;
-
-constexpr int TNW = 12, TNT = TNW * 64, TBM = 16;
-
-struct TokBwdParams {
-    const float* dout;
-    const float* real;
-    const float* y4;
-    const float* y2; int64_t ld2;
-    const float *w4, *w2;
-    float *d_nf, *d_add;
-    float* dx4; int64_t ldx4;
-    float* d_pt;
-    float* d_token;
-    int G, N;
-    float slope4, slope2;
-    uint32_t thr_pos, thr_in;
-    float keep_pos, keep_in;
-    uint64_t seed;
-    const uint64_t* seed_dev;
-    uint32_t salt_nf, salt_tok, salt_in;
-    int n_node_blocks;
-};
-
-__device__ __forceinline__ float leaky_grad(float y, float slope) { return y > 0.f ? 1.f : slope; }
-
-#ifdef TB_STAMP
-__device__ int* g_tb_dbg = nullptr;
-#define TSTAMP_DECL int st_[8] = {}
-#define TSTAMP(i) st_[i] = (int)wall_clock64()
-#define TSTAMP_DUMP() do { if (g_tb_dbg && threadIdx.x == 0) for (int q_ = 0; q_ < 8; ++q_) g_tb_dbg[blockIdx.x * 8 + q_] = st_[q_]; } while (0)
-#else
-#define TSTAMP_DECL
-#define TSTAMP(i)
-#define TSTAMP_DUMP()
-#endif
-
-template <int N> constexpr int gemm_ks() { return TNW / ((N + 63) / 64); }
-template <int K, int N, int LDA, int LDO>
-__device__ __forceinline__ void gemm_kn(const float* __restrict__ A, const float* __restrict__ W, float* __restrict__ out) {
-    constexpr int NB = (N + 63) / 64, KS = TNW / NB, NT16 = K / 16, TMAX = (NT16 + KS - 1) / KS;
-    static_assert(K % 16 == 0 && N % 32 == 0 && KS >= 1, "shape");
-    const int lane = threadIdx.x & 63, wave = threadIdx.x >> 6;
-    const int j = lane & 15, q = lane >> 4;
-    if (wave >= NB * KS) return;
-    const int blk = wave / KS, ks = wave % KS;
-    const int t_lo = ks * NT16 / KS, t_hi = (ks + 1) * NT16 / KS;
-    const int n0 = 64 * blk;
-    const bool col_ok = n0 + 4 * j < N;
-    const int cl = col_ok ? n0 + 4 * j : 0;
-    f32x4 acc[4];
-#pragma unroll
-    for (int n = 0; n < 4; ++n) acc[n] = f32x4{0.f, 0.f, 0.f, 0.f};
-    f32x4 bw[TMAX][4];
-#pragma unroll
-    for (int tt = 0; tt < TMAX; ++tt) {
-        const int t = min(t_lo + tt, t_hi - 1);
-#pragma unroll
-        for (int i = 0; i < 4; ++i) bw[tt][i] = *reinterpret_cast<const f32x4*>(W + (int64_t)(16 * t + 4 * q + i) * N + cl);
-    }
-#pragma unroll
-    for (int tt = 0; tt < TMAX; ++tt) {
-        if (t_lo + tt < t_hi) {
-            const f32x4 a = *reinterpret_cast<const f32x4*>(A + j * LDA + 16 * (t_lo + tt) + 4 * q);
-#pragma unroll
-            for (int i = 0; i < 4; ++i)
-#pragma unroll
-                for (int n = 0; n < 4; ++n) acc[n] = __builtin_amdgcn_mfma_f32_16x16x4f32(a[i], bw[tt][i][n], acc[n], 0, 0, 0);
-        }
-    }
-    if (col_ok) {
-#pragma unroll
-        for (int n = 0; n < 4; ++n)
-#pragma unroll
-            for (int v = 0; v < 4; ++v) out[(ks * TBM + 4 * q + v) * LDO + n0 + 4 * j + n] = acc[n][v];
-    }
-}
-
-template <int C, int W2>
-__global__ __launch_bounds__(TNT) void token_bwd_chain_kernel(const TokBwdParams p) {
-    constexpr int LDA = C + 4, LD2 = W2 + 4;
-    __shared__ __attribute__((aligned(16))) float a4[TBM * LDA];
-    constexpr int KS4 = gemm_ks<C>(), KS2 = gemm_ks<W2>();
-    __shared__ __attribute__((aligned(16))) float t4[(KS4 > KS2 ? KS4 : KS2) * TBM * LDA];
-    const int lane = threadIdx.x & 63, wave = threadIdx.x >> 6;
-    const int T = p.N + 1;
-    const uint64_t seed = (p.thr_pos || p.thr_in) ? p.seed + (p.seed_dev ? *p.seed_dev : 0ull) : 0ull;
-    if ((int)blockIdx.x >= p.n_node_blocks) {
-        const int g = ((int)blockIdx.x - p.n_node_blocks) * TNW + wave;
-        if (g >= p.G) return;
-        const int64_t row = (int64_t)g * T;
-        const uint32_t h1 = p.thr_pos ? dropout_row_hash(seed, (uint32_t)g ^ p.salt_tok) : 0u;
-        const uint32_t h2 = p.thr_in ? dropout_row_hash(seed, (uint32_t)row ^ p.salt_in) : 0u;
-        for (int c = lane; c < C; c += 64) {
-            float scale = 1.f;
-            if (p.thr_pos) scale = dropout_bits16(seed, h1, (uint32_t)c) >= p.thr_pos ? p.keep_pos : 0.f;
-            if (p.thr_in) scale *= dropout_bits16(seed, h2, (uint32_t)c) >= p.thr_in ? p.keep_in : 0.f;
-            const float d = p.dout[row * C + c] * scale;
-            if (d != 0.f) atomicAdd(&p.d_token[c], d);
-        }
-        return;
-    }
-    const int64_t R = (int64_t)p.G * p.N;
-    const int64_t j0 = (int64_t)blockIdx.x * TBM;
-    TSTAMP_DECL;
-    TSTAMP(0);
-    constexpr int EPT = TBM * C / TNT;
-    static_assert(TBM * C % TNT == 0, "flat split");
-    float dv[EPT], yv[EPT], rl[EPT];
-#pragma unroll
-    for (int k = 0; k < EPT; ++k) {
-        const int e = threadIdx.x + k * TNT, r = e / C, c = e % C;
-        const int64_t jc = min(j0 + r, R - 1);
-        const int g = (int)(jc / p.N), n = (int)(jc - (int64_t)g * p.N);
-        dv[k] = p.dout[((int64_t)g * T + n + 1) * C + c];
-        yv[k] = p.y4[jc * C + c];
-        rl[k] = p.real[jc];
-    }
-#pragma unroll
-    for (int k = 0; k < EPT; ++k) {
-        const int e = threadIdx.x + k * TNT, r = e / C, c = e % C;
-        const int64_t jn = j0 + r;
-        const bool on = jn < R;
-        const int64_t jc = on ? jn : R - 1;
-        const int g = (int)(jc / p.N), n = (int)(jc - (int64_t)g * p.N);
-        const int64_t row = (int64_t)g * T + n + 1;
-        float scale = 1.f;
-        if (p.thr_pos) scale = dropout_bits16(seed, dropout_row_hash(seed, (uint32_t)jc ^ p.salt_nf), (uint32_t)c) >= p.thr_pos ? p.keep_pos : 0.f;
-        if (p.thr_in) scale *= dropout_bits16(seed, dropout_row_hash(seed, (uint32_t)row ^ p.salt_in), (uint32_t)c) >= p.thr_in ? p.keep_in : 0.f;
-        const float d = on ? dv[k] * scale : 0.f;
-        const float dnf = d * rl[k];
-        a4[r * LDA + c] = dnf * leaky_grad(yv[k], p.slope4);
-        if (on) {
-            p.d_add[jn * C + c] = d;
-            p.d_nf[jn * C + c] = dnf;
-        }
-    }
-    __syncthreads();
-    TSTAMP(1);
-    gemm_kn<C, C, LDA, LDA>(a4, p.w4, t4);
-    __syncthreads();
-    TSTAMP(2);
-    for (int e = threadIdx.x; e < TBM * C; e += TNT) {
-        const int r = e / C, c = e % C;
-        const int64_t jn = j0 + r;
-        float v = 0.f;
-#pragma unroll
-        for (int ks = 0; ks < KS4; ++ks) v += t4[(ks * TBM + r) * LDA + c];
-        if (jn < R) p.dx4[jn * p.ldx4 + c] = v;
-        if (c < W2) a4[r * LD2 + c] = jn < R ? v * leaky_grad(p.y2[jn * p.ld2 + c], p.slope2) : 0.f;
-    }
-    __syncthreads();
-    TSTAMP(3);
-    gemm_kn<W2, W2, LD2, LD2>(a4, p.w2, t4);
-    __syncthreads();
-    TSTAMP(4);
-    for (int e = threadIdx.x; e < TBM * W2; e += TNT) {
-        const int r = e / W2, c = e % W2;
-        const int64_t jn = j0 + r;
-        float v = 0.f;
-#pragma unroll
-        for (int ks = 0; ks < KS2; ++ks) v += t4[(ks * TBM + r) * LD2 + c];
-        if (jn < R) p.d_pt[jn * W2 + c] = v;
-    }
-    TSTAMP(5);
-    TSTAMP_DUMP();
-}
-
-}
+using namespace mobgt_tokbwd;
 
 #ifdef TB_STAMP
 extern "C" int mobgt_tokbwd_debug_buffer(int* buf) { return (int)hipMemcpyToSymbol(HIP_SYMBOL(g_tb_dbg), &buf, sizeof(buf)); }
@@ -182,21 +11,8 @@
                                      float* d_pt, float* d_token, int G, int N, int C, int W2, float slope4, float slope2,
                                      float p_pos, float p_in, uint64_t seed, const uint64_t* seed_dev, uint32_t salt_nf,
                                      uint32_t salt_tok, uint32_t salt_in, void* stream) {
-    if (G <= 0 || N <= 0) return MOBGT_EBADDIM;
-    if (!(C == 192 && W2 == 160)) return MOBGT_EBADDIM;
-    if (!dout || !real || !y4 || !y2 || !w4 || !w2 || !d_nf || !d_add || !dx4 || !d_pt || !d_token || ld_y2 < W2 || ld_dx4 < C)
-        return MOBGT_EBADDIM;
-    if (((uintptr_t)w4 | (uintptr_t)w2) & 15) return MOBGT_EALIGN;
-    TokBwdParams p = {};
-    p.dout = dout; p.real = real; p.y4 = y4; p.y2 = y2; p.ld2 = ld_y2; p.w4 = w4; p.w2 = w2; p.d_nf = d_nf; p.d_add = d_add;
-    p.dx4 = dx4; p.ldx4 = ld_dx4; p.d_pt = d_pt; p.d_token = d_token; p.G = G; p.N = N; p.slope4 = slope4; p.slope2 = slope2;
-    p.thr_pos = p_pos > 0.f ? dropout_threshold(p_pos) : 0u;
-    p.thr_in = p_in > 0.f ? dropout_threshold(p_in) : 0u;
-    p.keep_pos = p.thr_pos ? 1.f / (1.f - (float)p.thr_pos / 65536.f) : 1.f;
-    p.keep_in = p.thr_in ? 1.f / (1.f - (float)p.thr_in / 65536.f) : 1.f;
-    p.seed = seed; p.seed_dev = seed_dev; p.salt_nf = salt_nf; p.salt_tok = salt_tok; p.salt_in = salt_in;
-    p.n_node_blocks = (int)(((int64_t)G * N + TBM - 1) / TBM);
-    const dim3 grid(p.n_node_blocks + (G + TNW - 1) / TNW), block(TNT);
-    hipLaunchKernelGGL((token_bwd_chain_kernel<192, 160>), grid, block, 0, (hipStream_t)stream, p);
-    return (int)hipGetLastError();
+    TokBwdParams p;
+    const int rc = fill_params(p, dout, real, y4, y2, ld_y2, w4, w2, d_nf, d_add, dx4, ld_dx4, d_pt, d_token, G, N, C, W2, slope4, slope2,
+                               p_pos, p_in, seed, seed_dev, salt_nf, salt_tok, salt_in);
+    return rc ? rc : launch_plain(p, stream);
 }
diff --git a/mobgt_amd/csrc/tokbwd_body.h b/mobgt_amd/csrc/tokbwd_body.h
--- /dev/null
+++ b/mobgt_amd/csrc/tokbwd_body.h
@@ -0,0 +1,322 @@
+#pragma once
+#include "common.h"
+#include "mobgt_hip.h"
+#include "wgrad_body.h"
+
+namespace mobgt_tokbwd {
+namespace {
+
+typedef __attribute__((ext_vector_type(4))) float f32x4;
+
+constexpr int TNW = 12, TNT = TNW * 64, TBM = 16;
+constexpr int TAIL_NW = 8;
+constexpr int HOST_MAX_WG = 4;
+
+struct TokBwdParams {
+    const float* dout;
+    const float* real;
+    const float* y4;
+    const float* y2; int64_t ld2;
+    const float *w4, *w2;
+    float *d_nf, *d_add;
+    float* dx4; int64_t ldx4;
+    float* d_pt;
+    float* d_token;
+    int G, N;
+    float slope4, slope2;
+    uint32_t thr_pos, thr_in;
+    float keep_pos, keep_in;
+    uint64_t seed;
+    const uint64_t* seed_dev;
+    uint32_t salt_nf, salt_tok, salt_in;
+    int n_node_blocks;
+};
+
+struct TokHost {
+    const uint16_t *t_dqkv, *t_wqt;
+    float* dx1;
+    mobgt_wgrad::WgradParams wg[HOST_MAX_WG];
+    int wg_first[HOST_MAX_WG + 1], wg_tiles[HOST_MAX_WG], wg_splits[HOST_MAX_WG];
+    int n_wg, n_chain;
+};
+
+__device__ __forceinline__ float leaky_grad(float y, float slope) { return y > 0.f ? 1.f : slope; }
+
+#ifdef TB_STAMP
+__device__ int* g_tb_dbg = nullptr;
+#define TSTAMP_DECL int st_[8] = {}
+#define TSTAMP(i) st_[i] = (int)wall_clock64()
+#define TSTAMP_DUMP() do { if (g_tb_dbg && threadIdx.x == 0) for (int q_ = 0; q_ < 8; ++q_) g_tb_dbg[blockIdx.x * 8 + q_] = st_[q_]; } while (0)
+#else
+#define TSTAMP_DECL
+#define TSTAMP(i)
+#define TSTAMP_DUMP()
+#endif
+
+template <int N> constexpr int gemm_ks() { return TNW / ((N + 63) / 64); }
+template <int K, int N, int LDA, int LDO>
+__device__ __forceinline__ void gemm_kn(const float* __restrict__ A, const float* __restrict__ W, float* __restrict__ out) {
+    constexpr int NB = (N + 63) / 64, KS = TNW / NB, NT16 = K / 16, TMAX = (NT16 + KS - 1) / KS;
+    static_assert(K % 16 == 0 && N % 32 == 0 && KS >= 1, "shape");
+    const int lane = threadIdx.x & 63, wave = threadIdx.x >> 6;
+    const int j = lane & 15, q = lane >> 4;
+    if (wave >= NB * KS) return;
+    const int blk = wave / KS, ks = wave % KS;
+    const int t_lo = ks * NT16 / KS, t_hi = (ks + 1) * NT16 / KS;
+    const int n0 = 64 * blk;
+    const bool col_ok = n0 + 4 * j < N;
+    const int cl = col_ok ? n0 + 4 * j : 0;
+    f32x4 acc[4];
+#pragma unroll
+    for (int n = 0; n < 4; ++n) acc[n] = f32x4{0.f, 0.f, 0.f, 0.f};
+    f32x4 bw[TMAX][4];
+#pragma unroll
+    for (int tt = 0; tt < TMAX; ++tt) {
+        const int t = min(t_lo + tt, t_hi - 1);
+#pragma unroll
+        for (int i = 0; i < 4; ++i) bw[tt][i] = *reinterpret_cast<const f32x4*>(W + (int64_t)(16 * t + 4 * q + i) * N + cl);
+    }
+#pragma unroll
+    for (int tt = 0; tt < TMAX; ++tt) {
+        if (t_lo + tt < t_hi) {
+            const f32x4 a = *reinterpret_cast<const f32x4*>(A + j * LDA + 16 * (t_lo + tt) + 4 * q);
+#pragma unroll
+            for (int i = 0; i < 4; ++i)
+#pragma unroll
+                for (int n = 0; n < 4; ++n) acc[n] = __builtin_amdgcn_mfma_f32_16x16x4f32(a[i], bw[tt][i][n], acc[n], 0, 0, 0);
+        }
+    }
+    if (col_ok) {
+#pragma unroll
+        for (int n = 0; n < 4; ++n)
+#pragma unroll
+            for (int v = 0; v < 4; ++v) out[(ks * TBM + 4 * q + v) * LDO + n0 + 4 * j + n] = acc[n][v];
+    }
+}
+
+template <int C, int LDA, typename ROWOF>
+__device__ __forceinline__ void host_tail(const TokHost& h, float* __restrict__ dst, uint16_t* __restrict__ tq, ROWOF&& row_of) {
+    constexpr int K = 3 * C, S = K / 32, LDQ = K + 8;
+    static_assert(C == 16 * TNW && K % 32 == 0, "one 16-column group per wave");
+    const int lane = threadIdx.x & 63, wave = threadIdx.x >> 6;
+    const int j = lane & 15, q = lane >> 4;
+    uint4 b[S];
+    const uint16_t* wp = h.t_wqt + ((int64_t)wave * S * 64 + lane) * 8;
+#pragma unroll
+    for (int s = 0; s < S; ++s) b[s] = *reinterpret_cast<const uint4*>(wp + 512 * s);
+    for (int e = threadIdx.x; e < TBM * (C / 4); e += TNT) {
+        const int r = e / (C / 4), c = (e % (C / 4)) * 4;
+        *reinterpret_cast<float4*>(dst + r * LDA + c) = *reinterpret_cast<const float4*>(h.dx1 + row_of(r) * C + c);
+    }
+    for (int e = threadIdx.x; e < TBM * (K / 8); e += TNT) {
+        const int r = e / (K / 8), c = (e % (K / 8)) * 8;
+        *reinterpret_cast<uint4*>(tq + r * LDQ + c) = *reinterpret_cast<const uint4*>(h.t_dqkv + row_of(r) * K + c);
+    }
+    __syncthreads();
+    f32x4 acc[TAIL_NW];
+#pragma unroll
+    for (int i = 0; i < TAIL_NW; ++i) acc[i] = f32x4{0.f, 0.f, 0.f, 0.f};
+    const uint16_t* a0 = tq + j * LDQ + 8 * q;
+#pragma unroll
+    for (int s = 0; s < S; ++s) {
+        const bf16x8 af = *reinterpret_cast<const bf16x8*>(a0 + 32 * s);
+        acc[s % TAIL_NW] = __builtin_amdgcn_mfma_f32_16x16x32_bf16(af, __builtin_bit_cast(bf16x8, b[s]), acc[s % TAIL_NW], 0, 0, 0);
+    }
+    f32x4 sum = acc[0];
+#pragma unroll
+    for (int i = 1; i < TAIL_NW; ++i) sum += acc[i];
+#pragma unroll
+    for (int v = 0; v < 4; ++v) {
+        float* o = dst + (4 * q + v) * LDA + 16 * wave + j;
+        *o = sum[v] + *o;
+    }
+    __syncthreads();
+}
+
+template <int C, int W2, bool HOST>
+__device__ __forceinline__ void token_bwd_body(const TokBwdParams& p, const TokHost* hp, float* __restrict__ a4, float* __restrict__ t4) {
+    constexpr int LDA = C + 4, LD2 = W2 + 4;
+    constexpr int KS4 = gemm_ks<C>(), KS2 = gemm_ks<W2>();
+    const int lane = threadIdx.x & 63, wave = threadIdx.x >> 6;
+    const int T = p.N + 1;
+    const uint64_t seed = (p.thr_pos || p.thr_in) ? p.seed + (p.seed_dev ? *p.seed_dev : 0ull) : 0ull;
+    bool tail = false;
+    if constexpr (HOST) {
+        const TokHost& h = *hp;
+        static_assert(mobgt_wgrad::wgrad_lds_floats<TAIL_NW>() <= (KS4 > KS2 ? KS4 : KS2) * TBM * LDA, "the passenger's LDS");
+        static_assert(TBM * (3 * C + 8) * 2 <= (KS4 > KS2 ? KS4 : KS2) * TBM * LDA * 4, "the rows of dqkv");
+        if ((int)blockIdx.x >= h.n_chain) {
+            const int bid = (int)blockIdx.x - h.n_chain;
+            int qn = 0;
+#pragma unroll
+            for (int t = 1; t < HOST_MAX_WG; ++t)
+                if (t < h.n_wg && bid >= h.wg_first[t]) qn = t;
+            const int local = bid - h.wg_first[qn];
+            mobgt_wgrad::wgrad_body<false, TAIL_NW, false, TNW>(h.wg[qn], local % h.wg_tiles[qn], local / h.wg_tiles[qn],
+                                                                h.wg_splits[qn], t4);
+            return;
+        }
+        tail = h.t_dqkv != nullptr;
+        if ((int)blockIdx.x >= p.n_node_blocks) {
+            const int g0 = ((int)blockIdx.x - p.n_node_blocks) * TBM;
+            if (tail)
+                host_tail<C, LDA>(h, a4, reinterpret_cast<uint16_t*>(t4), [&](int r) { return (int64_t)min(g0 + r, p.G - 1) * T; });
+            for (int e = threadIdx.x; e < TBM * C; e += TNT) {
+                const int r = e / C, c = e % C, g = min(g0 + r, p.G - 1);
+                const int64_t row = (int64_t)g * T;
+                float x;
+                if (tail) x = a4[r * LDA + c];
+                else x = p.dout[row * C + c];
+                if (tail && g0 + r < p.G) h.dx1[row * C + c] = x;
+                float scale = 1.f;
+                if (p.thr_pos) scale = dropout_bits16(seed, dropout_row_hash(seed, (uint32_t)g ^ p.salt_tok), (uint32_t)c) >= p.thr_pos ? p.keep_pos : 0.f;
+                if (p.thr_in) scale *= dropout_bits16(seed, dropout_row_hash(seed, (uint32_t)row ^ p.salt_in), (uint32_t)c) >= p.thr_in ? p.keep_in : 0.f;
+                a4[r * LDA + c] = g0 + r < p.G ? x * scale : 0.f;
+            }
+            __syncthreads();
+            if (threadIdx.x < C) {
+                double s = 0.0;
+#pragma unroll
+                for (int r = 0; r < TBM; ++r) s += (double)a4[r * LDA + threadIdx.x];
+                if (s != 0.0) atomicAdd(&p.d_token[threadIdx.x], (float)s);
+            }
+            return;
+        }
+    }
+    if (!HOST && (int)blockIdx.x >= p.n_node_blocks) {
+        const int g = ((int)blockIdx.x - p.n_node_blocks) * TNW + wave;
+        if (g >= p.G) return;
+        const int64_t row = (int64_t)g * T;
+        const uint32_t h1 = p.thr_pos ? dropout_row_hash(seed, (uint32_t)g ^ p.salt_tok) : 0u;
+        const uint32_t h2 = p.thr_in ? dropout_row_hash(seed, (uint32_t)row ^ p.salt_in) : 0u;
+        for (int c = lane; c < C; c += 64) {
+            float scale = 1.f;
+            if (p.thr_pos) scale = dropout_bits16(seed, h1, (uint32_t)c) >= p.thr_pos ? p.keep_pos : 0.f;
+            if (p.thr_in) scale *= dropout_bits16(seed, h2, (uint32_t)c) >= p.thr_in ? p.keep_in : 0.f;
+            const float d = p.dout[row * C + c] * scale;
+            if (d != 0.f) atomicAdd(&p.d_token[c], d);
+        }
+        return;
+    }
+    const int64_t R = (int64_t)p.G * p.N;
+    const int64_t j0 = (int64_t)blockIdx.x * TBM;
+    TSTAMP_DECL;
+    TSTAMP(0);
+    if constexpr (HOST) {
+        if (tail)
+            host_tail<C, LDA>(*hp, a4, reinterpret_cast<uint16_t*>(t4), [&](int r) {
+                const int64_t jc = min(j0 + r, R - 1);
+                return jc + jc / p.N + 1;
+            });
+    }
+    constexpr int EPT = TBM * C / TNT;
+    static_assert(TBM * C % TNT == 0, "flat split");
+    float dv[EPT], yv[EPT], rl[EPT];
+#pragma unroll
+    for (int k = 0; k < EPT; ++k) {
+        const int e = threadIdx.x + k * TNT, r = e / C, c = e % C;
+        const int64_t jc = min(j0 + r, R - 1);
+        const int g = (int)(jc / p.N), n = (int)(jc - (int64_t)g * p.N);
+        if (HOST && tail) dv[k] = a4[r * LDA + c];
+        else dv[k] = p.dout[((int64_t)g * T + n + 1) * C + c];
+        yv[k] = p.y4[jc * C + c];
+        rl[k] = p.real[jc];
+    }
+#pragma unroll
+    for (int k = 0; k < EPT; ++k) {
+        const int e = threadIdx.x + k * TNT, r = e / C, c = e % C;
+        const int64_t jn = j0 + r;
+        const bool on = jn < R;
+        const int64_t jc = on ? jn : R - 1;
+        const int g = (int)(jc / p.N), n = (int)(jc - (int64_t)g * p.N);
+        const int64_t row = (int64_t)g * T + n + 1;
+        float scale = 1.f;
+        if (p.thr_pos) scale = dropout_bits16(seed, dropout_row_hash(seed, (uint32_t)jc ^ p.salt_nf), (uint32_t)c) >= p.thr_pos ? p.keep_pos : 0.f;
+        if (p.thr_in) scale *= dropout_bits16(seed, dropout_row_hash(seed, (uint32_t)row ^ p.salt_in), (uint32_t)c) >= p.thr_in ? p.keep_in : 0.f;
+        const float d = on ? dv[k] * scale : 0.f;
+        const float dnf = d * rl[k];
+        a4[r * LDA + c] = dnf * leaky_grad(yv[k], p.slope4);
+        if (on) {
+            if constexpr (HOST) {
+                if (tail) hp->dx1[row * C + c] = dv[k];
+            }
+            p.d_add[jn * C + c] = d;
+            p.d_nf[jn * C + c] = dnf;
+        }
+    }
+    __syncthreads();
+    TSTAMP(1);
+    gemm_kn<C, C, LDA, LDA>(a4, p.w4, t4);
+    __syncthreads();
+    TSTAMP(2);
+    for (int e = threadIdx.x; e < TBM * C; e += TNT) {
+        const int r = e / C, c = e % C;
+        const int64_t jn = j0 + r;
+        float v = 0.f;
+#pragma unroll
+        for (int ks = 0; ks < KS4; ++ks) v += t4[(ks * TBM + r) * LDA + c];
+        if (jn < R) p.dx4[jn * p.ldx4 + c] = v;
+        if (c < W2) a4[r * LD2 + c] = jn < R ? v * leaky_grad(p.y2[jn * p.ld2 + c], p.slope2) : 0.f;
+    }
+    __syncthreads();
+    TSTAMP(3);
+    gemm_kn<W2, W2, LD2, LD2>(a4, p.w2, t4);
+    __syncthreads();
+    TSTAMP(4);
+    for (int e = threadIdx.x; e < TBM * W2; e += TNT) {
+        const int r = e / W2, c = e % W2;
+        const int64_t jn = j0 + r;
+        float v = 0.f;
+#pragma unroll
+        for (int ks = 0; ks < KS2; ++ks) v += t4[(ks * TBM + r) * LD2 + c];
+        if (jn < R) p.d_pt[jn * W2 + c] = v;
+    }
+    TSTAMP(5);
+    TSTAMP_DUMP();
+}
+
+#define TOKBWD_LDS(C, W2)                                                                                                          \
+    __shared__ __attribute__((aligned(16))) float a4[TBM * (C + 4)];                                                               \
+    __shared__ __attribute__((aligned(16))) float t4[(gemm_ks<C>() > gemm_ks<W2>() ? gemm_ks<C>() : gemm_ks<W2>()) * TBM * (C + 4)]
+
+template <int C, int W2>
+__global__ __launch_bounds__(TNT) void token_bwd_chain_kernel(const TokBwdParams p) {
+    TOKBWD_LDS(C, W2);
+    token_bwd_body<C, W2, false>(p, nullptr, a4, t4);
+}
+
+template <int C, int W2>
+__global__ __launch_bounds__(TNT) void token_bwd_chain_host_kernel(const TokBwdParams p, const TokHost h) {
+    TOKBWD_LDS(C, W2);
+    token_bwd_body<C, W2, true>(p, &h, a4, t4);
+}
+
+inline int fill_params(TokBwdParams& p, const float* dout, const float* real, const float* y4, const float* y2, int64_t ld_y2, const float* w4,
+                const float* w2, float* d_nf, float* d_add, float* dx4, int64_t ld_dx4, float* d_pt, float* d_token, int G, int N,
+                int C, int W2, float slope4, float slope2, float p_pos, float p_in, uint64_t seed, const uint64_t* seed_dev,
+                uint32_t salt_nf, uint32_t salt_tok, uint32_t salt_in) {
+    if (G <= 0 || N <= 0) return MOBGT_EBADDIM;
+    if (!(C == 192 && W2 == 160)) return MOBGT_EBADDIM;
+    if (!dout || !real || !y4 || !y2 || !w4 || !w2 || !d_nf || !d_add || !dx4 || !d_pt || !d_token || ld_y2 < W2 || ld_dx4 < C)
+        return MOBGT_EBADDIM;
+    if (((uintptr_t)w4 | (uintptr_t)w2) & 15) return MOBGT_EALIGN;
+    p = {};
+    p.dout = dout; p.real = real; p.y4 = y4; p.y2 = y2; p.ld2 = ld_y2; p.w4 = w4; p.w2 = w2; p.d_nf = d_nf; p.d_add = d_add;
+    p.dx4 = dx4; p.ldx4 = ld_dx4; p.d_pt = d_pt; p.d_token = d_token; p.G = G; p.N = N; p.slope4 = slope4; p.slope2 = slope2;
+    p.thr_pos = p_pos > 0.f ? dropout_threshold(p_pos) : 0u;
+    p.thr_in = p_in > 0.f ? dropout_threshold(p_in) : 0u;
+    p.keep_pos = p.thr_pos ? 1.f / (1.f - (float)p.thr_pos / 65536.f) : 1.f;
+    p.keep_in = p.thr_in ? 1.f / (1.f - (float)p.thr_in / 65536.f) : 1.f;
+    p.seed = seed; p.seed_dev = seed_dev; p.salt_nf = salt_nf; p.salt_tok = salt_tok; p.salt_in = salt_in;
+    p.n_node_blocks = (int)(((int64_t)G * N + TBM - 1) / TBM);
+    return 0;
+}
+
+inline int launch_plain(const TokBwdParams& p, void* stream) {
+    const dim3 grid(p.n_node_blocks + (p.G + TNW - 1) / TNW), block(TNT);
+    hipLaunchKernelGGL((token_bwd_chain_kernel<192, 160>), grid, block, 0, (hipStream_t)stream, p);
+    return (int)hipGetLastError();
+}
+
+}
+}
diff --git a/mobgt_amd/csrc/wgrad_body.h b/mobgt_amd/csrc/wgrad_body.h
--- a/mobgt_amd/csrc/wgrad_body.h
+++ b/mobgt_amd/csrc/wgrad_body.h
@@ -93,12 +93,14 @@
 
 template <int NWAVE> constexpr int wgrad_lds_floats() { return (NWAVE / 2) * TILE * TILE + NWAVE * TILE; }
 
-template <bool F32, int NWAVE, bool XF32 = F32>
+template <bool F32, int NWAVE, bool XF32 = F32, int WGW = NWAVE>
 __device__ __forceinline__ void wgrad_body(const WgradParams& p, const int tile, const int split, const int nsplit,
                                            float* __restrict__ lds) {
+    static_assert(WGW >= NWAVE, "a workgroup of at least NWAVE waves");
     float (*part)[TILE * TILE] = reinterpret_cast<float (*)[TILE * TILE]>(lds);
     float (*colpart)[TILE] = reinterpret_cast<float (*)[TILE]>(lds + (NWAVE / 2) * TILE * TILE);
     const int lane = threadIdx.x & 63, wave = threadIdx.x >> 6;
+    const bool act = WGW == NWAVE || wave < NWAVE;
     const int i = lane & 15, kq = lane >> 4;
     const int m0 = (tile / p.tiles_n) * TILE, n0 = (tile % p.tiles_n) * TILE;
     const int k0 = split * p.k_per_wg;
@@ -123,7 +125,7 @@
         if (masked) s_.template load_masked<F32>(p, gp, xp, gm, xm, r0_, k1, m_ok, n_ok, gkeep);
         else s_.template load<F32, XF32>(gp, xp, p.ldg, p.ldx, r0_, k1, m_ok, n_ok);
     };
-    int kb = k0 + wave * KSTEP;
+    int kb = act ? k0 + wave * KSTEP : k1;
     Slab cur, nxt;
     if (kb < k1) fetch(cur, kb + 8 * kq);
     for (; kb < k1; kb += NWAVE * KSTEP) {
@@ -146,7 +148,7 @@
         if (kn < k1) cur = nxt;
     }
 
-    if (wave >= NWAVE / 2) {
+    if (wave >= NWAVE / 2 && act) {
 #pragma unroll
         for (int a = 0; a < 2; ++a)
 #pragma unroll
@@ -163,13 +165,13 @@
 #pragma unroll
                 for (int v = 0; v < 4; ++v) part[wave][(2 * (4 * kq + v) + a) * TILE + 2 * i + b] += acc[a][b][v];
     }
-    if (want_db) {
+    if (want_db && act) {
         se += __shfl_xor(se, 16, 64); se += __shfl_xor(se, 32, 64);
         so += __shfl_xor(so, 16, 64); so += __shfl_xor(so, 32, 64);
         if (kq == 0) { colpart[wave][2 * i] = se; colpart[wave][2 * i + 1] = so; }
     }
     __syncthreads();
-    for (int e = threadIdx.x; e < TILE * TILE; e += NWAVE * 64) {
+    for (int e = act ? threadIdx.x : TILE * TILE; e < TILE * TILE; e += NWAVE * 64) {
         const int r = e >> 5, c = e & 31;
         float s = 0.f;
 #pragma unroll
diff --git a/mobgt_amd/csrc_tokhost/tokhost.hip b/mobgt_amd/csrc_tokhost/tokhost.hip
--- /dev/null
+++ b/mobgt_amd/csrc_tokhost/tokhost.hip
@@ -0,0 +1,46 @@
+#include "mobgt_tokhost.h"
+#include "tokbwd_body.h"
+
+using namespace mobgt_tokbwd;
+
+static_assert(MOBGT_TOKHOST_MAX_WG == HOST_MAX_WG, "the kernel's problem slots");
+static_assert(MOBGT_TOKHOST_MAX_ROWS == mobgt_wgrad::SHORT_R, "the rows of the 8-wave weight-gradient launch");
+static_assert(MOBGT_TOKHOST_EBADDIM == MOBGT_EBADDIM && MOBGT_TOKHOST_EALIGN == MOBGT_EALIGN, "the shared fill's status codes");
+
+extern "C" int mobgt_tokhost_abi_version(void) { return MOBGT_TOKHOST_ABI_VERSION; }
+
+extern "C" int mobgt_tokhost_token_bwd_chain(const float* dout, const float* real, const float* y4, const float* y2, int64_t ld_y2,
+                                             const float* w4, const float* w2, float* d_nf, float* d_add, float* dx4, int64_t ld_dx4,
+                                             float* d_pt, float* d_token, int G, int N, int C, int W2, float slope4, float slope2,
+                                             float p_pos, float p_in, uint64_t seed, const uint64_t* seed_dev, uint32_t salt_nf,
+                                             uint32_t salt_tok, uint32_t salt_in, const void* tail_dqkv, const void* tail_wqkv_t,
+                                             float* dx1, int n_wg, const void* const* wg_g, const int64_t* wg_ldg,
+                                             const void* const* wg_x, const int64_t* wg_ldx, float* const* wg_dw,
+                                             const int64_t* wg_ldw, float* const* wg_db, const int* wg_M, const int* wg_N,
+                                             void* stream) {
+    TokBwdParams p;
+    int rc = fill_params(p, dout, real, y4, y2, ld_y2, w4, w2, d_nf, d_add, dx4, ld_dx4, d_pt, d_token, G, N, C, W2, slope4, slope2,
+                         p_pos, p_in, seed, seed_dev, salt_nf, salt_tok, salt_in);
+    if (rc) return rc;
+    if ((tail_dqkv == nullptr) != (tail_wqkv_t == nullptr) || n_wg < 0 || n_wg > MOBGT_TOKHOST_MAX_WG) return MOBGT_TOKHOST_EBADDIM;
+    if (tail_dqkv && dx1 != dout) return MOBGT_TOKHOST_EBADDIM;
+    if (n_wg && (!wg_g || !wg_ldg || !wg_x || !wg_ldx || !wg_dw || !wg_ldw || !wg_M || !wg_N)) return MOBGT_TOKHOST_EBADDIM;
+    if (((uintptr_t)tail_dqkv | (uintptr_t)tail_wqkv_t | (uintptr_t)(tail_dqkv ? dx1 : nullptr)) & 15) return MOBGT_TOKHOST_EALIGN;
+    if (!tail_dqkv && n_wg == 0) return launch_plain(p, stream);
+    if ((int64_t)G * (N + 1) > MOBGT_TOKHOST_MAX_ROWS) return MOBGT_TOKHOST_EBADDIM;
+    TokHost h = {};
+    h.t_dqkv = reinterpret_cast<const uint16_t*>(tail_dqkv); h.t_wqt = reinterpret_cast<const uint16_t*>(tail_wqkv_t); h.dx1 = dx1;
+    h.n_wg = n_wg;
+    h.n_chain = p.n_node_blocks + (G + TBM - 1) / TBM;
+    int total = 0;
+    for (int i = 0; i < n_wg; ++i) {
+        rc = mobgt_wgrad::fill_problem(h.wg[i], wg_g[i], wg_ldg[i], wg_x[i], wg_ldx[i], wg_dw[i], wg_ldw[i], wg_db ? wg_db[i] : nullptr,
+                                       (int64_t)G * (N + 1), wg_M[i], wg_N[i], 256 / n_wg, &h.wg_tiles[i], &h.wg_splits[i], 0, TAIL_NW);
+        if (rc) return rc;
+        h.wg_first[i] = total;
+        total += h.wg_tiles[i] * h.wg_splits[i];
+    }
+    for (int i = n_wg; i <= MOBGT_TOKHOST_MAX_WG; ++i) h.wg_first[i] = total;
+    hipLaunchKernelGGL((token_bwd_chain_host_kernel<192, 160>), dim3(h.n_chain + total), dim3(TNT), 0, (hipStream_t)stream, p, h);
+    return (int)hipGetLastError();
+}
diff --git a/mobgt_amd/forms.py b/mobgt_amd/forms.py
--- a/mobgt_amd/forms.py
+++ b/mobgt_amd/forms.py
@@ -20,6 +20,10 @@
     Form("skinny_all", "MOBGT_SKINNY_ALL", False, "all three classifier products on csrc/skinny.hip (off: dW / db only)"),
     Form("token_fwd_chain", "MOBGT_NO_TOKEN_FWD_CHAIN", True, "the encoder input's forward as one launch (off: four)"),
     Form("token_bwd_chain", "MOBGT_NO_TOKEN_BWD_CHAIN", True, "the encoder input's backward as one launch, csrc/tokbwd.hip (off: three)"),
+    Form("l0_token_host", "MOBGT_NO_L0_TOKEN_HOST", True, "the first encoder layer leaves dx and its weight gradients to the encoder "
+         "input's one-launch backward (off: it finishes its own backward); no workgroup waits for another, so safe_forms keeps it"),
+    Form("l0_token_host_eager", "MOBGT_L0_TOKEN_HOST_EAGER", False, "l0_token_host outside a graph capture as well (off: only a step "
+         "that is being captured defers; an eager step is bound by the host, gains nothing and keeps its launch list)"),
     Form("pack_passenger", "MOBGT_NO_PACK_PASSENGER", True, "the layers' weight pack, in the next front launch"),
     Form("front_passengers", "MOBGT_NO_FRONT_PASSENGERS", True, "hop table forward and node-feature indices, in the category GCN's forward"),
     Form("bias_bwd_passenger", "MOBGT_NO_BIAS_BWD_PASSENGER", True, "short batches: the bias tables' backward, in the category GCN's backward"),
diff --git a/mobgt_amd/fused_layer.py b/mobgt_amd/fused_layer.py
--- a/mobgt_amd/fused_layer.py
+++ b/mobgt_amd/fused_layer.py
@@ -264,6 +264,7 @@
         self.pack = pack
         self.act_dtype = act_dtype
         self.from_layer = False
+        self.token_host = False
         self.next_qkv = None
         self.packed = None
         self.packed_t = None
@@ -514,6 +515,8 @@
         busy = getattr(ctx, "_mobgt_pending", None)
         if busy is not None:
             busy.done()
+        if cfg.token_host and not (STEP.wgrad_on and forms.on("l0_token_host") and forms.on("token_bwd_chain")):
+            plan = plan._replace(below_hosts=False)
         preln = plan.body == "preln_chain"
         dout = dout.contiguous().view(R, C).float()
         if preln:
diff --git a/mobgt_amd/layer_plan.py b/mobgt_amd/layer_plan.py
--- a/mobgt_amd/layer_plan.py
+++ b/mobgt_amd/layer_plan.py
@@ -1,11 +1,12 @@
 from collections import namedtuple
 
-from . import _lib
+from . import _lib, _tokhost
 
 CHAIN_SHAPES = ((128, 1024), (192, 1024), (256, 1024))
 BIG_R = _lib.CONSTANTS["MOBGT_CHAIN_BIG_ROWS"]
 TAIL_MAX_R = 1024
 DEFER_MAX_R = 4096
+TOKEN_HOST_MAX_R = _tokhost.MAX_ROWS
 
 FORWARD_FORMS = ("own_gemm", "ln_gemm", "stock_ln_qkv", "chain", "chain_big", "chain_bwd")
 BACKWARD_FORMS = ("ln_gemm_bwd", "wgrad_big", "defer_tail", "tail")
diff --git a/mobgt_amd/model.py b/mobgt_amd/model.py
--- a/mobgt_amd/model.py
+++ b/mobgt_amd/model.py
@@ -181,7 +181,11 @@
     if (p > 0 or p_att > 0) and mha.seed_dev is None:
         seed = (seed + int(torch.randint(0, 2 ** 31 - 1, (1,)).item())) & 0x7FFFFFFFFFFFFFFF
     cfg = LayerConfig(variant, mha.num_heads, mha.scale, p, p_att, seed, mha.seed_dev, mha._layer_index * 8, pack, act)
-    cfg.from_layer = bool(getattr(x, "_mobgt_from_layer", False)) and not getattr(layer, "_mobgt_cut", False)
+    cut = getattr(layer, "_mobgt_cut", False)
+    cfg.token_host = bool(variant != "stock" and getattr(x, "_mobgt_token_host", False) and not cut and forms.on("l0_token_host")
+                          and forms.on("token_bwd_chain") and G * T <= layer_plan.TOKEN_HOST_MAX_R
+                          and (torch.cuda.is_current_stream_capturing() or forms.on("l0_token_host_eager")))
+    cfg.from_layer = (bool(getattr(x, "_mobgt_from_layer", False)) and not cut) or cfg.token_host
     nxt = next_layer
     stock = variant == "stock"
     if (nxt is not None and act != torch.float32 and not amp and getattr(nxt, "fused", False)
diff --git a/mobgt_amd/ops.py b/mobgt_amd/ops.py
--- a/mobgt_amd/ops.py
+++ b/mobgt_amd/ops.py
@@ -4,7 +4,7 @@
 
 import torch
 
-from . import _lib, forms
+from . import _lib, _tokhost, forms
 from ._lib import F32, BF16, I64, I32, I16, U8, check
 from .step_state import STEP
 
@@ -1512,12 +1512,28 @@
         W2 = ent["w2"].shape[0]
         d_pt = torch.empty(G * N, W2, dtype=torch.float32, device=g.device)
         dx4 = pend["dx4"]
-        _lib.call("mobgt_token_bwd_chain", _p(pend["dout"]), _p(pend["real"]), _p(ent["nf"]), _p(ent["x4"]), ent["x4"].stride(0),
-                  _p(ent["w4"]), _p(ent["w2"]), _p(pend["d_nf"]), _p(pend["d_add"]), _p(dx4), dx4.stride(0),
-                  _p(d_pt), _p(pend["d_tok"]), G, N, C, W2, ent["slope4"], ent["slope2"], p_pos, p_in, seed,
-                  _p(seed_dev), salts[0], salts[1], salts[2], _stream())
+        args = (_p(pend["dout"]), _p(pend["real"]), _p(ent["nf"]), _p(ent["x4"]), ent["x4"].stride(0),
+                _p(ent["w4"]), _p(ent["w2"]), _p(pend["d_nf"]), _p(pend["d_add"]), _p(dx4), dx4.stride(0),
+                _p(d_pt), _p(pend["d_tok"]), G, N, C, W2, ent["slope4"], ent["slope2"], p_pos, p_in, seed,
+                _p(seed_dev), salts[0], salts[1], salts[2])
+        tail = pend.get("tail")
+        if tail is None:
+            _lib.call("mobgt_token_bwd_chain", *args, _stream())
+        else:
+            from .fused_layer import _wgrad_arrays
+            _tokhost.launch("mobgt_tokhost_token_bwd_chain", *args, _p(tail["dqkv"]), _p(tail["wqt"]), _p(tail["dx1"]),
+                      *_wgrad_arrays(tail["items"]), _stream())
         return d_pt
     return None
+
+
+def _token_can_host(tail, dout, rows, C):
+    dqkv, wqt, items = tail["dqkv"], tail["wqt"], tail["items"]
+    return (forms.on("l0_token_host") and tail["kind"] == "layer" and tail["R"] == rows and C == 192
+            and rows <= _tokhost.MAX_ROWS and 1 <= len(items) <= _tokhost.MAX_WG and tail["dx1"].data_ptr() == dout.data_ptr()
+            and dout.dtype == torch.float32 and dout.data_ptr() % 16 == 0 and dqkv.dtype == torch.bfloat16 and dqkv.is_contiguous()
+            and tuple(dqkv.shape) == (rows, 3 * C) and dqkv.data_ptr() % 16 == 0 and wqt.data_ptr() % 16 == 0
+            and all(g_.dtype == torch.bfloat16 and x_.dtype == torch.bfloat16 and g_.shape[0] == rows for g_, x_, _, _ in items))
 
 
 class _LinearSplitKFn(torch.autograd.Function):
@@ -1920,10 +1936,16 @@
             d_tok = zeros_f32((C,), dout.device)
             d_pe = d_tok.view(pshape)
         ent = STEP.token_chain
-        if (ent is not None and ent["nf_ptr"] == ctx.nf_ptr and STEP.wgrad_on and C == ent["nf"].shape[1]
-                and G * N == ent["nf"].shape[0] and forms.on("token_bwd_chain")):
+        park = (ent is not None and ent["nf_ptr"] == ctx.nf_ptr and STEP.wgrad_on and C == ent["nf"].shape[1]
+                and G * N == ent["nf"].shape[0] and forms.on("token_bwd_chain"))
+        from . import fused_layer
+        tail = fused_layer._take_tail(dout)
+        if tail is not None and not (park and _token_can_host(tail, dout, G * (N + 1), C)):
+            fused_layer._complete_pending(tail)
+            tail = None
+        if park:
             STEP.token_pending[d_nf.data_ptr()] = dict(stage=1, ent=ent, dout=dout, real=real, d_nf=d_nf, d_add=d_add, d_tok=d_tok,
-                                                       misc=(G, N, C, p_pos, p_in, seed, seed_dev, salts))
+                                                       misc=(G, N, C, p_pos, p_in, seed, seed_dev, salts), tail=tail)
         else:
             _lib.call("mobgt_assemble_tokens_bwd", _p(dout), _p(real), _p(d_nf), _p(d_add), _p(d_tok), G, N, C, p_pos, p_in, seed,
                       _p(seed_dev), salts[0], salts[1], salts[2], _stream())
@@ -1951,6 +1973,9 @@
         out._mobgt_act = side[0]
         if len(side) > 1:
             out._mobgt_qkv = side[1]
+            ent = STEP.token_chain
+            if ent is not None and ent["nf_ptr"] == nf.data_ptr() and nf.shape[-1] == 192:
+                out._mobgt_token_host = True
     return out
 
 
diff --git a/mobgt_amd/step_state.py b/mobgt_amd/step_state.py
--- a/mobgt_amd/step_state.py
+++ b/mobgt_amd/step_state.py
@@ -17,7 +17,8 @@
     Field("token_fwd", PARKED, dict, "'gather' / 'f2' / 'f4': _GatherMultiFn / _LinearSplitKFn.forward record; _AssembleTokensFn launches them as one"),
     Field("token_fwd_fused_calls", CARRIED, int, "how often mobgt_token_fwd_chain took the three records (a counter for tests)"),
     Field("token_chain", CARRIED, _none, "ops.register_token_chain: the encoder-input chain of the forward that just ran; its backward reads it"),
-    Field("token_pending", PARKED, dict, "_AssembleTokensFn.backward parks under a gradient's address; FuseEmbeddings-4 / -2's backward re-park / launch"),
+    Field("token_pending", PARKED, dict, "_AssembleTokensFn.backward parks under a gradient's address (with the first layer's tail, taken from layer_tails, "
+          "under 'tail'); FuseEmbeddings-4 / -2's backward re-park / launch"),
     Field("front_sgemm", PARKED, dict, "'job': ops.front_small_gemm parks, the bias assembly's launch takes; 'done': its result until ops.small_gemm asks"),
     Field("wgrad_on", SWITCH, bool, "ops.recording_wgrads around the trainer's backward"),
     Field("wgrad_items", PARKED, list, "leaf weight gradients (ops.linear_wgrad*, fused layers) for ops.flush_deferred_wgrads' grouped launch"),
@@ -25,7 +26,8 @@
     Field("wgrad_hop_wide", PARKED, _none, "_HopTableFn.backward past 256 edge ids; shares the flush's stock tail launch"),
     Field("wgrad_stock_tok", PARKED, _none, "_StockTokensFn.backward parks; the flush's stock tail launch takes"),
     Field("wgrad_psum", PARKED, list, "ops.defer_partial_sum: split-K partial sums for the flush's one reduction launch"),
-    Field("layer_tails", PARKED, dict, "(graph task, device, address of dx1) -> a fused layer's tail; the chain launch of the layer below takes"),
+    Field("layer_tails", PARKED, dict, "(graph task, device, address of dx1) -> a fused layer's tail; the chain launch of the layer below (first layer: "
+          "the encoder input's backward) takes"),
     Field("tail_check_task", PARKED, _none, "graph task whose end-of-backward check (fused_layer._pending_check) is queued"),
     Field("weight_pack", PARKED, list, "model.pack_layer_weights(defer=True) parks; the category GCN's / stock front's forward launch takes"),
     Field("gcn_prelaunched", PARKED, dict, "modelGNN.prelaunch_small_gcn: id(module) -> (key, result); that module's forward adopts it"),
```

New measurement: 27310, median of 6. 1.3% higher.
